# kvarq/kvarq

Measured on AMD Instinct MI355X. Metric: fastq_reads_per_sec_scanned, higher is better.
Workload: dtype u8

## Files before the change

include/kvarq_hip.h:

```cpp
#ifndef KVARQ_HIP_H
#define KVARQ_HIP_H

#include <stddef.h>
#include <stdint.h>

#ifdef __cplusplus
extern "C" {
#endif

#define KVQ_MAX_READLENGTH 1024
#define KVQ_SCANBUFSIZE    (1024*1024)
#define KVQ_MUT_CLASSES    6

enum {
    KVQ_OK          = 0,
    KVQ_ERR_FORMAT  = 1,
    KVQ_ERR_IO      = 2,
    KVQ_ERR_MEMORY  = 3,
    KVQ_ERR_RUNTIME = 4,
    KVQ_ERR_TYPE    = 5,
    KVQ_ERR_DEVICE  = 6,
    KVQ_ERR_RESCAN  = 7
};

typedef struct kvq_config {
    int32_t maxerrors;
    int32_t minoverlap;
    int32_t minreadlength;
    int32_t nthreads;
    int8_t  Amin;
    int8_t  Azero;
} kvq_config;

void kvq_config_set(const kvq_config *cfg);
void kvq_config_get(kvq_config *cfg);

int32_t kvq_last_error(char *msg, size_t cap);

typedef struct kvq_table kvq_table;

kvq_table *kvq_table_create(const uint8_t *const *seqs, const int32_t *seqlens, int32_t nseq,
                            const kvq_config *cfg);
void    kvq_table_destroy(kvq_table *t);
int32_t kvq_table_nseq(const kvq_table *t);
int64_t kvq_table_bases(const kvq_table *t);
int32_t kvq_table_seq_is_seeded(const kvq_table *t, int32_t s);
int32_t kvq_table_seed_k(const kvq_table *t);

enum { KVQ_CTR_RECORDS = 0, KVQ_CTR_LONGEST = 1, KVQ_CTR_HITS = 2, KVQ_CTR_READLENGTHS = 4 };
int64_t kvq_counters_len(const kvq_table *t);
int64_t kvq_counters_off_nseqhits(const kvq_table *t);
int64_t kvq_counters_off_nseqbasehits(const kvq_table *t);
int64_t kvq_counters_off_coverage(const kvq_table *t);
int64_t kvq_counters_off_mutations(const kvq_table *t);
int64_t kvq_table_seq_offset(const kvq_table *t, int32_t s);

typedef struct kvq_scan kvq_scan;

kvq_scan *kvq_scan_create(const kvq_table *t, void *d_counters);
void      kvq_scan_destroy(kvq_scan *s);

int64_t kvq_chunk_offsets(const uint8_t *data, int64_t nbytes, int64_t *offsets, int64_t cap);

int32_t kvq_scan_device(kvq_scan *s, const void *d_data, int64_t nbytes,
                        const int64_t *chunk_off, int64_t nchunks, int64_t fpos_base);

int32_t kvq_scan_host(kvq_scan *s, const void *h_data, int64_t nbytes,
                      const int64_t *chunk_off, int64_t nchunks, int64_t fpos_base);

int32_t kvq_scan_host_async(kvq_scan *s, const void *h_data, int64_t nbytes,
                            const int64_t *chunk_off, int64_t nchunks, int64_t fpos_base);
int32_t kvq_scan_host_copied(kvq_scan *s);
int32_t kvq_scan_host_drain(kvq_scan *s);

int32_t kvq_scan_finish(kvq_scan *s);
int32_t kvq_scan_finish_begin(kvq_scan *s);

int64_t        kvq_scan_n_hits(const kvq_scan *s);
const int32_t *kvq_scan_hit_seq_nr(const kvq_scan *s);
const int64_t *kvq_scan_hit_file_pos(const kvq_scan *s);
const int32_t *kvq_scan_hit_seq_pos(const kvq_scan *s);
const int32_t *kvq_scan_hit_length(const kvq_scan *s);
const int32_t *kvq_scan_hit_readlength(const kvq_scan *s);
const uint8_t *kvq_scan_hitseq_blob(const kvq_scan *s);
const int64_t *kvq_scan_hitseq_offsets(const kvq_scan *s);
const int64_t *kvq_scan_counters(const kvq_scan *s);
void          *kvq_scan_device_counters(const kvq_scan *s);
void          *kvq_scan_device_counters_own(const kvq_scan *s);
int64_t        kvq_scan_parsed(const kvq_scan *s);
int64_t        kvq_scan_total(const kvq_scan *s);

int32_t        kvq_scan_set_records(kvq_scan *s, int32_t on);
const uint8_t *kvq_scan_record_blob(const kvq_scan *s);
const int64_t *kvq_scan_hit_record_off(const kvq_scan *s);
const int32_t *kvq_scan_hit_record_len(const kvq_scan *s);
int64_t        kvq_scan_record_bytes(const kvq_scan *s);

double  kvq_scan_kernel_ms(const kvq_scan *s);
double  kvq_scan_main_kernel_ms(const kvq_scan *s);
double  kvq_scan_gap_ms(const kvq_scan *a, const kvq_scan *b);
int64_t kvq_scan_main_kernel_launches(const kvq_scan *s);
int32_t kvq_scan_reset(kvq_scan *s);
int32_t kvq_scan_path(const kvq_scan *s);
void    kvq_scan_force_exhaustive(kvq_scan *s, int32_t on);

#define KVQ_CELL_DENSE  0x1000
#define KVQ_CELL_DIAG   0x2000
#define KVQ_CELL_STAMPS 0x4000
int32_t kvq_scan_kernel_pick(int32_t k, int32_t stride, int32_t dense, uint32_t rec_bytes, uint32_t tile_bytes, uint32_t dbg);
int32_t kvq_scan_kernel(const kvq_scan *s);
uint32_t kvq_tile_for_text(const uint8_t *text, size_t n, uint32_t *rec_bytes_out);

typedef struct kvq_comm kvq_comm;
int32_t   kvq_comm_unique_id(void *id128);
kvq_comm *kvq_comm_create(int32_t nranks, int32_t rank, const void *id128);
void      kvq_comm_destroy(kvq_comm *c);
int32_t   kvq_comm_nranks(const kvq_comm *c);
int32_t   kvq_comm_rank(const kvq_comm *c);
int32_t   kvq_scan_set_comm(kvq_scan *s, kvq_comm *c);
int32_t   kvq_scan_gather_hits(kvq_scan *s, kvq_comm *c);
int32_t   kvq_comm_allreduce_counters(kvq_comm *c, void *d_counters, int64_t ctr_len, void *d_scratch16);
kvq_comm *kvq_comm_create_local(int32_t nranks, int32_t rank, uint64_t world_key);
int32_t   kvq_gather_plan(int32_t nranks, const uint64_t *counts, uint64_t *parts, uint64_t *blob_base, uint64_t *totals);
int32_t   kvq_gather_host(int32_t nranks, const uint64_t *counts, const uint8_t *const *rank_bufs, uint8_t *out);
void      kvq_result_layout_words(uint64_t n, uint64_t blob_bytes, uint64_t *out8);

kvq_scan *kvq_findseqs(const char *const *files, int32_t nfiles,
                       const uint8_t *const *seqs, const int32_t *seqlens, int32_t nseq);

#define KVQ_FIND_DEVICE_INFLATE 1u
#define KVQ_FIND_DEVICE_GZIP 2u
#define KVQ_FIND_RECORDS 4u
kvq_scan *kvq_findseqs_ex(const char *const *files, int32_t nfiles,
                          const uint8_t *const *seqs, const int32_t *seqlens, int32_t nseq, uint32_t flags);

void kvq_findseqs_free(kvq_scan *s);

int64_t kvq_host_chunk_plan(const char *const *files, int32_t nfiles, int64_t *chunk_fpos, int64_t *chunk_len,
                            int64_t cap, int64_t *parsed, int64_t *total, int64_t batch_bytes);

typedef struct kvq_live_stats {
    int64_t records_parsed;
    int64_t parsed;
    int64_t total;
    int64_t rls_longest;
    int32_t nseq;
    int32_t running;
    int32_t sigints;
    int32_t stop_requested;
} kvq_live_stats;

void kvq_poll_stats(kvq_live_stats *out, int64_t *readlengths ,
                    int64_t *nseqhits, int64_t *nseqbasehits, int32_t nseq_cap);
void kvq_request_stop(void);
void kvq_count_sigint(void);
int  kvq_sigint_counter_install(void);
void kvq_sigint_counter_remove(void);

int32_t kvq_device_count(void);
int32_t kvq_set_device(int32_t ordinal);
void   *kvq_device_alloc(int64_t nbytes);
void    kvq_device_free(void *p);
int32_t kvq_memcpy_h2d(void *d, const void *h, int64_t nbytes);
int32_t kvq_memcpy_d2h(void *h, const void *d, int64_t nbytes);
int32_t kvq_memset_d(void *d, int32_t value, int64_t nbytes);
int32_t kvq_device_synchronize(void);
void    kvq_release_cached(void);

int32_t kvq_synth_reads_device(void *d_out, int64_t first, int64_t n, int32_t L,
                               uint64_t seed, const void *d_genome, int64_t genome_size);
void    kvq_synth_reads_host(uint8_t *out, int64_t first, int64_t n, int32_t L,
                             uint64_t seed, const uint8_t *genome, int64_t genome_size);
void    kvq_synth_genome_host(uint8_t *out, int64_t size, uint64_t seed);

int32_t kvq_inflate_raw_host(const uint8_t *in, int64_t n, uint8_t *out, int64_t isize);

int64_t kvq_bgzf_index(const uint8_t *file_bytes, int64_t n, int64_t *block_off, uint32_t *csize, uint32_t *isize, int64_t cap);

typedef struct kvq_bgzf_block {
    int64_t  in_off;
    int64_t  out_off;
    uint32_t in_len;
    uint32_t isize;
} kvq_bgzf_block;

int32_t kvq_inflate_bgzf_device(const void *d_in, int64_t in_bytes, const kvq_bgzf_block *d_blocks, int64_t nblocks,
                                void *d_out, int64_t out_bytes, int32_t *d_status);

int64_t kvq_chunk_offsets_device(const void *d_data, int64_t nbytes, int64_t *offsets, int64_t cap);

typedef struct kvq_gzip_report {
    int64_t runs;
    int64_t chunks;
    int64_t candidates_tested;
    int64_t refuted;
    int64_t redecodes;
    int64_t slot_overflows;
    int64_t marker_symbols;
    int64_t input_retries;
    double  ms_find, ms_decode, ms_resolve, ms_replace;
} kvq_gzip_report;

int64_t kvq_inflate_gzip_host(const uint8_t *file, int64_t n, int64_t chunk_bytes, uint8_t *out, int64_t out_cap,
                              int32_t *status, int64_t *err_fpos, kvq_gzip_report *rep);
int64_t kvq_inflate_gzip_device(const void *d_file, int64_t n, int64_t chunk_bytes, void *d_out, int64_t out_cap,
                                int32_t *status, int64_t *err_fpos, kvq_gzip_report *rep);
void    kvq_gzip_last_report(kvq_gzip_report *rep);
int64_t kvq_gzip_slot_canaries(int32_t pad_symbols);
int64_t kvq_gzip_last_chunks(int64_t *cand, int64_t ncand_cap, int64_t *start_bit, int64_t *end_bit, int64_t *nsym, int64_t cap,
                             int64_t *ncand);

typedef struct kvq_bam_report {
    int64_t runs;
    int64_t segments;
    int64_t refuted;
    int64_t check_passes;
    int64_t records_seen;
    int64_t records_written;
    int64_t records_skipped;
    int64_t records_noqual;
    int64_t bam_bytes;
    int64_t text_bytes;
    double  ms_inflate, ms_find, ms_emit;
} kvq_bam_report;
void    kvq_bam_last_report(kvq_bam_report *rep);
int64_t kvq_bam_header_host(const uint8_t *inflated, int64_t n, int32_t *n_ref);
int64_t kvq_bam_to_fastq_host(const uint8_t *inflated, int64_t n, int32_t n_ref, int64_t first_record, uint8_t *out, int64_t cap,
                              int64_t *consumed);
int64_t kvq_bam_to_fastq_device(const void *d_in, int64_t n, int32_t n_ref, int64_t first_record, void *d_out, int64_t cap,
                                int64_t segment_bytes, kvq_bam_report *report);

const char *kvq_version(void);

#ifdef __cplusplus
}
#endif
#endif
```

kvarq_amd/_lib.py:

```python
import ctypes as C
import os

HERE = os.path.dirname(os.path.abspath(__file__))
PATH = os.path.join(HERE, 'libkvarq_hip.so')

MAX_READLENGTH = 1024
OK, ERR_FORMAT, ERR_IO, ERR_MEMORY, ERR_RUNTIME, ERR_TYPE, ERR_DEVICE, ERR_RESCAN = range(8)
CTR_RECORDS, CTR_LONGEST, CTR_HITS, CTR_READLENGTHS = 0, 1, 2, 4
CELL_DENSE, CELL_DIAG, CELL_STAMPS = 0x1000, 0x2000, 0x4000
FIND_RECORDS = 4


class Config(C.Structure):
    _fields_ = [('maxerrors', C.c_int32), ('minoverlap', C.c_int32), ('minreadlength', C.c_int32),
                ('nthreads', C.c_int32), ('Amin', C.c_int8), ('Azero', C.c_int8)]


class LiveStats(C.Structure):
    _fields_ = [('records_parsed', C.c_int64), ('parsed', C.c_int64), ('total', C.c_int64),
                ('rls_longest', C.c_int64), ('nseq', C.c_int32), ('running', C.c_int32),
                ('sigints', C.c_int32), ('stop_requested', C.c_int32)]


class GzipReport(C.Structure):
    _fields_ = [(n, C.c_int64) for n in ('runs', 'chunks', 'candidates_tested', 'refuted', 'redecodes',
                                         'slot_overflows', 'marker_symbols', 'input_retries')] + \
        [(n, C.c_double) for n in ('ms_find', 'ms_decode', 'ms_resolve', 'ms_replace')]

    def as_dict(self):
        return {n: getattr(self, n) for n, _ in self._fields_}


class BamReport(C.Structure):
    _fields_ = [(n, C.c_int64) for n in ('runs', 'segments', 'refuted', 'check_passes', 'records_seen', 'records_written',
                                         'records_skipped', 'records_noqual', 'bam_bytes', 'text_bytes')] + \
        [(n, C.c_double) for n in ('ms_inflate', 'ms_find', 'ms_emit')]

    def as_dict(self):
        return {n: getattr(self, n) for n, _ in self._fields_}


i32, i64, u64, vp, cp = C.c_int32, C.c_int64, C.c_uint64, C.c_void_p, C.c_char_p
P = C.POINTER

PROTOTYPES = {
    'kvq_config_set': (None, [P(Config)]),
    'kvq_config_get': (None, [P(Config)]),
    'kvq_last_error': (i32, [C.c_char_p, C.c_size_t]),
    'kvq_table_create': (vp, [P(cp), P(i32), i32, P(Config)]),
    'kvq_table_destroy': (None, [vp]),
    'kvq_table_nseq': (i32, [vp]),
    'kvq_table_bases': (i64, [vp]),
    'kvq_table_seq_is_seeded': (i32, [vp, i32]),
    'kvq_table_seed_k': (i32, [vp]),
    'kvq_counters_len': (i64, [vp]),
    'kvq_counters_off_nseqhits': (i64, [vp]),
    'kvq_counters_off_nseqbasehits': (i64, [vp]),
    'kvq_counters_off_coverage': (i64, [vp]),
    'kvq_counters_off_mutations': (i64, [vp]),
    'kvq_table_seq_offset': (i64, [vp, i32]),
    'kvq_scan_create': (vp, [vp, vp]),
    'kvq_scan_destroy': (None, [vp]),
    'kvq_chunk_offsets': (i64, [vp, i64, P(i64), i64]),
    'kvq_scan_device': (i32, [vp, vp, i64, P(i64), i64, i64]),
    'kvq_scan_host': (i32, [vp, vp, i64, P(i64), i64, i64]),
    'kvq_scan_host_async': (i32, [vp, vp, i64, P(i64), i64, i64]),
    'kvq_scan_host_copied': (i32, [vp]),
    'kvq_scan_host_drain': (i32, [vp]),
    'kvq_scan_finish': (i32, [vp]),
    'kvq_scan_finish_begin': (i32, [vp]),
    'kvq_scan_n_hits': (i64, [vp]),
    'kvq_scan_hit_seq_nr': (P(i32), [vp]),
    'kvq_scan_hit_file_pos': (P(i64), [vp]),
    'kvq_scan_hit_seq_pos': (P(i32), [vp]),
    'kvq_scan_hit_length': (P(i32), [vp]),
    'kvq_scan_hit_readlength': (P(i32), [vp]),
    'kvq_scan_hitseq_blob': (vp, [vp]),
    'kvq_scan_hitseq_offsets': (P(i64), [vp]),
    'kvq_scan_counters': (P(i64), [vp]),
    'kvq_scan_device_counters': (vp, [vp]),
    'kvq_scan_device_counters_own': (vp, [vp]),
    'kvq_scan_parsed': (i64, [vp]),
    'kvq_scan_total': (i64, [vp]),
    'kvq_scan_set_records': (i32, [vp, i32]),
    'kvq_scan_record_blob': (vp, [vp]),
    'kvq_scan_hit_record_off': (P(i64), [vp]),
    'kvq_scan_hit_record_len': (P(i32), [vp]),
    'kvq_scan_record_bytes': (i64, [vp]),
    'kvq_scan_kernel_ms': (C.c_double, [vp]),
    'kvq_scan_main_kernel_ms': (C.c_double, [vp]),
    'kvq_scan_gap_ms': (C.c_double, [vp, vp]),
    'kvq_scan_main_kernel_launches': (i64, [vp]),
    'kvq_scan_reset': (i32, [vp]),
    'kvq_scan_path': (i32, [vp]),
    'kvq_scan_force_exhaustive': (None, [vp, i32]),
    'kvq_scan_kernel_pick': (i32, [i32, i32, i32, C.c_uint32, C.c_uint32, C.c_uint32]),
    'kvq_scan_kernel': (i32, [vp]),
    'kvq_tile_for_text': (C.c_uint32, [vp, C.c_size_t, P(C.c_uint32)]),
    'kvq_comm_unique_id': (i32, [vp]),
    'kvq_comm_create': (vp, [i32, i32, vp]),
    'kvq_comm_destroy': (None, [vp]),
    'kvq_comm_nranks': (i32, [vp]),
    'kvq_comm_rank': (i32, [vp]),
    'kvq_scan_set_comm': (i32, [vp, vp]),
    'kvq_scan_gather_hits': (i32, [vp, vp]),
    'kvq_comm_allreduce_counters': (i32, [vp, vp, i64, vp]),
    'kvq_comm_create_local': (vp, [i32, i32, C.c_uint64]),
    'kvq_gather_plan': (i32, [i32, vp, vp, vp, vp]),
    'kvq_gather_host': (i32, [i32, vp, vp, vp]),
    'kvq_result_layout_words': (None, [C.c_uint64, C.c_uint64, vp]),
    'kvq_findseqs': (vp, [P(cp), i32, P(cp), P(i32), i32]),
    'kvq_findseqs_ex': (vp, [P(cp), i32, P(cp), P(i32), i32, C.c_uint32]),
    'kvq_findseqs_free': (None, [vp]),
    'kvq_host_chunk_plan': (i64, [P(cp), i32, P(i64), P(i64), i64, P(i64), P(i64), i64]),
    'kvq_poll_stats': (None, [P(LiveStats), P(i64), P(i64), P(i64), i32]),
    'kvq_request_stop': (None, []),
    'kvq_count_sigint': (None, []),
    'kvq_sigint_counter_install': (C.c_int, []),
    'kvq_sigint_counter_remove': (None, []),
    'kvq_device_count': (i32, []),
    'kvq_set_device': (i32, [i32]),
    'kvq_device_alloc': (vp, [i64]),
    'kvq_device_free': (None, [vp]),
    'kvq_memcpy_h2d': (i32, [vp, vp, i64]),
    'kvq_memcpy_d2h': (i32, [vp, vp, i64]),
    'kvq_memset_d': (i32, [vp, i32, i64]),
    'kvq_device_synchronize': (i32, []),
    'kvq_release_cached': (None, []),
    'kvq_synth_reads_device': (i32, [vp, i64, i64, i32, u64, vp, i64]),
    'kvq_synth_reads_host': (None, [vp, i64, i64, i32, u64, vp, i64]),
    'kvq_synth_genome_host': (None, [vp, i64, u64]),
    'kvq_inflate_raw_host': (i32, [vp, i64, vp, i64]),
    'kvq_bgzf_index': (i64, [vp, i64, P(i64), P(C.c_uint32), P(C.c_uint32), i64]),
    'kvq_chunk_offsets_device': (i64, [vp, i64, P(i64), i64]),
    'kvq_inflate_bgzf_device': (i32, [vp, i64, vp, i64, vp, i64, vp]),
    'kvq_inflate_gzip_host': (i64, [vp, i64, i64, vp, i64, P(i32), P(i64), P(GzipReport)]),
    'kvq_inflate_gzip_device': (i64, [vp, i64, i64, vp, i64, P(i32), P(i64), P(GzipReport)]),
    'kvq_gzip_last_report': (None, [P(GzipReport)]),
    'kvq_gzip_slot_canaries': (i64, [i32]),
    'kvq_gzip_last_chunks': (i64, [P(i64), i64, P(i64), P(i64), P(i64), i64, P(i64)]),
    'kvq_bam_last_report': (None, [P(BamReport)]),
    'kvq_bam_header_host': (i64, [vp, i64, P(i32)]),
    'kvq_bam_to_fastq_host': (i64, [vp, i64, i32, i64, vp, i64, P(i64)]),
    'kvq_bam_to_fastq_device': (i64, [vp, i64, i32, i64, vp, i64, i64, P(BamReport)]),
    'kvq_version': (cp, []),
}

_lib = None


def build():
    import subprocess
    subprocess.check_call(['make', '-s', '-C', os.path.join(HERE, 'csrc')])


def lib():
    global _lib
    if _lib is None:
        if not os.path.exists(PATH):
            raise ImportError('%s is missing: build it with `make -C kvarq_amd/csrc` '
                              '(there is no CPU fallback for the scan)' % PATH)
        L = C.CDLL(PATH)
        for name, (res, args) in PROTOTYPES.items():
            f = getattr(L, name)
            f.restype, f.argtypes = res, args
        _lib = L
    return _lib


def kernel_cell(cell):
    if cell <= 0:
        return None
    return {'k': cell & 15, 'stride': (cell >> 4) & 15, 'lg': ((cell >> 8) & 15) - 1, 'dense': bool(cell & CELL_DENSE)}


def last_error():
    buf = C.create_string_buffer(1024)
    code = lib().kvq_last_error(buf, 1024)
    return code, buf.value.decode('latin-1')
```

kvarq_amd/csrc/kernels_bp.hip:

```cpp
#include "kvq_host.h"

#ifndef KVQ_TEXT_AUX
#define KVQ_TEXT_AUX 0
#endif
#define KVQ_MARK(name) asm volatile("; KVQMARK " name)
#define BP_WIN (ST_BUF + ST_BLK)
#define BP_Q1_KIND 25
#define BP_QW 96
#define BP_Q2W 96
#define BP_NLCAP 1920
#define BP_P2_LATE 0xFFFEu
#define BP_HEAD 2048u
#define BP_QCAP (BP_QW * ST_WAVES)
#define BP_Q2CAP (BP_Q2W * ST_WAVES)

typedef unsigned int u32x4_t __attribute__((ext_vector_type(4)));

struct BpLds {
    uint32_t cdp[BP_WIN / 16 + 8];
    uint32_t gdp[BP_WIN / 32 + 8];
    uint16_t nl[BP_NLCAP];
    uint8_t  bmA[8192];
    uint32_t hist[KVQ_RL_BINS / 2];
    union {
// ... 98 lines not shown
                for (int jj = 0; jj <= me && !earlier; jj++) {
                    const int ph = jj * KK, pt = rl - (jj + 1) * KK;
                    if (ph + KK <= rl && (kind == 0u || ph < p)) earlier = seed_live_bp<KK>(P.tab2, roff, rl, ph, toff, seql, ph + d);
                    if (!earlier && pt >= 0 && (kind == 0u || pt < p)) earlier = seed_live_bp<KK>(P.tab2, roff, rl, pt, toff, seql, pt + d);
                }
                if (kind == 0u) {
                    for (int jj = 0; jj <= me && !earlier; jj++)
                        for (int sft = 0; sft < stride && !earlier; sft++) {
                            const int o = jj * P.pitch + sft;
                            if (o < q && ((o - d) & (stride - 1)) == 0) earlier = seed_live_bp<KK>(P.tab2, roff, rl, o - d, toff, seql, o);
                        }
                }
                if (!earlier) { hitAB = canAB; hitC = canC; }
            }
        }
    }
    emit_cold(P.cold, hitAB, fpos, s, sposAB, lenAB, rl, keyAB);
    emit_cold(P.cold, hitC, fpos, s, sposC, lenC, rl, keyC);
}

__device__ __forceinline__ void bp_vector(const uint4 v, uint32_t addk, uint32_t &nl16, uint32_t &g16, uint32_t &c32)
{
    const uint32_t x[4] = { v.x, v.y, v.z, v.w };
    uint32_t nf[4], gf[4], cc[4];
#pragma unroll
    for (int d = 0; d < 4; d++) {
        nf[d] = kvq_nl_flags(x[d]);
        gf[d] = good_flags(x[d], addk);
        cc[d] = __builtin_amdgcn_udot4(x[d] & 0x06060606u, 0x40100401u, 0u, false);
    }
#ifdef KVQ_ABL_JUNK
    {
        uint32_t junk = x[0];
#pragma unroll
        for (int i = 0; i < KVQ_ABL_JUNK; i++) {
#if KVQ_ABL_SLOW == 2
            { uint32_t sj = 0; asm volatile("s_add_u32 %0, %0, 1" : "+s"(sj)); asm volatile("" :: "s"(sj)); }
#elif KVQ_ABL_SLOW == 3
            { uint32_t lj; asm volatile("ds_read_b32 %0, %1" : "=v"(lj) : "v"(junk & 0x3FCu)); asm volatile("s_waitcnt lgkmcnt(0)" ::: "memory"); asm volatile("" :: "v"(lj)); }
#elif KVQ_ABL_SLOW
            asm volatile("v_lshl_or_b32 %0, %0, 1, %1" : "+v"(junk) : "v"(x[1]));
#else
            asm volatile("v_add_u32 %0, %0, %1" : "+v"(junk) : "v"(x[1]));
#endif
        }
        asm volatile("" :: "v"(junk));
    }
#endif
    nl16 = kvq_flags16(nf[0], nf[1], nf[2], nf[3]);
    g16 = kvq_flags16(gf[0], gf[1], gf[2], gf[3]);
    c32 = ((cc[0] | (cc[1] << 8)) >> 1) | ((cc[2] | (cc[3] << 8)) << 15);
}

struct BpArgs {
    KvqParams P;
    SeedTables X;
    const uint8_t *data; int64_t fpos_base;
    const uint4 *tiles; uint32_t *tile_report; unsigned int *tile_ctr;
    void *redo;
    unsigned int *fail;
    void *surv;
    uint32_t ntiles, tile_bytes, dbg, pad_, redo_cap;
    uint32_t surv_cap;
};
#define BP_SHARDS 64u
#define BP_SHARD_STRIDE 32u
__host__ __device__ static inline uint32_t bp_shard_begin(uint32_t sh, uint32_t ntiles) { return (uint32_t)(((uint64_t)sh * ntiles) / BP_SHARDS); }
__device__ __forceinline__ uint32_t bp_draw(unsigned int *ctr, uint32_t ntiles, uint32_t &sh, uint32_t &left)
{
    while (left) {
        const uint32_t t = atomicAdd(&ctr[sh * BP_SHARD_STRIDE], 1u);
        if (t < bp_shard_begin(sh + 1u, ntiles)) return t;
        sh = sh + 1u == BP_SHARDS ? 0u : sh + 1u; left--;
    }
    return ntiles;
}
static_assert(BP_SHARDS == 64u, "one counter per lane of the drawing wave");
__device__ __forceinline__ uint32_t bp_draw_wave(unsigned int *ctr, uint32_t ntiles, uint32_t &sh, uint32_t lane)
{
    const uint32_t m = (((uint32_t)blockIdx.x >> 6) * 2u + 37u) | 1u;
    for (;;) {
        const uint32_t mine = (sh + m * lane) & (BP_SHARDS - 1u);
        const uint32_t seen = __hip_atomic_load(&ctr[mine * BP_SHARD_STRIDE], __ATOMIC_RELAXED, __HIP_MEMORY_SCOPE_AGENT);
        const uint64_t open = __ballot(seen < bp_shard_begin(mine + 1u, ntiles));
        if (open == 0) return ntiles;
        const uint32_t pick = (sh + m * (uint32_t)(__ffsll((long long)open) - 1)) & (BP_SHARDS - 1u);
        uint32_t t = 0;
        if (lane == 0) t = atomicAdd(&ctr[pick * BP_SHARD_STRIDE], 1u);
        t = (uint32_t)__builtin_amdgcn_readfirstlane((int)t);
        sh = pick;
        if (t < bp_shard_begin(pick + 1u, ntiles)) return t;
    }
}
typedef const __attribute__((address_space(4))) BpArgs *BpArgsPtr;
__device__ __forceinline__ BpArgsPtr bp_args(const BpArgs *A)
{
    BpArgsPtr p = (BpArgsPtr)A;
    asm volatile("" : "+s"(p));
    return p;
}

#ifndef BP_OCC
#define BP_OCC 8
#endif

__device__ __forceinline__ void bp_runs64(uint64_t m, int n, uint32_t dbg, int &pre, int &suf, int &best, int &bstart)
{
    const uint64_t nmask = n < 64 ? (1ull << n) - 1ull : ~0ull;
    uint64_t zz = ~m & nmask;
    const int c = __popc((uint32_t)zz) + __popc((uint32_t)(zz >> 32));
    if (!__any(c > 3) && !(dbg & 4u)) {
        const uint32_t lo = (uint32_t)zz, hi = (uint32_t)(zz >> 32);
        auto ffbl = [](uint32_t x) -> uint32_t { uint32_t r; asm("v_ffbl_b32 %0, %1" : "=v"(r) : "v"(x)); return r; };
        auto ffbh = [](uint32_t x) -> uint32_t { uint32_t r; asm("v_ffbh_u32 %0, %1" : "=v"(r) : "v"(x)); return r; };
        auto ctz64 = [&](uint32_t l, uint32_t h) -> uint32_t {
            const uint32_t pl = ffbl(l), ph = ffbl(h) | 32u;
            const uint32_t r = pl < ph ? pl : ph; return r < (uint32_t)n ? r : (uint32_t)n;
        };
        const uint32_t p1 = ctz64(lo, hi);
        const uint64_t z2 = zz & (zz - 1ull);
        const uint32_t p2 = ctz64((uint32_t)z2, (uint32_t)(z2 >> 32));
        const uint32_t ch = ffbh(hi), cl = ffbh(lo) | 32u;
        uint32_t lz = ch < cl ? ch : cl; lz = lz < 64u ? lz : 64u;
        const uint32_t e = 64u - lz;
        const int g0 = (int)p1, g1 = (int)p2 - (int)p1 - 1, g2 = (int)e - (int)p2 - 2, g3 = n - (int)e;
        int bl = g0, bs = 0;
        if (g1 > bl) { bl = g1; bs = (int)p1 + 1; }
        if (g2 > bl) { bl = g2; bs = (int)p2 + 1; }
        if (g3 > bl) { bl = g3; bs = (int)e; }
        pre = g0; suf = g3; best = bl; bstart = bs;
    } else if (!__any(c > 8) && !(dbg & 4u)) {
        int prev = 0, first = n, p, bl = 0, bs = 0;
        do {
            const uint32_t plo = (uint32_t)(__ffs((int)(uint32_t)zz) - 1), ph = (uint32_t)(__ffs((int)(uint32_t)(zz >> 32)) - 1);
            const uint32_t phi = ph > 0xFFFFFFDFu ? 0xFFFFFFFFu : ph + 32u;
            uint32_t pm = plo < phi ? plo : phi; if (pm > (uint32_t)n) pm = (uint32_t)n;
            p = (int)pm;
            zz &= zz - 1ull;
            first = first < p ? first : p;
            const int gap = p - prev;
            if (gap > bl) { bl = gap; bs = prev; }
            prev = p < n ? p + 1 : prev;
        } while (__any(p < n));
        pre = first; suf = n - prev; best = bl; bstart = bs;
    } else {
        const uint64_t inv = ~m;
        pre = inv ? __ffsll((long long)inv) - 1 : 64; if (pre > n) pre = n;
        const uint64_t top = ~(m << (64 - n));
        suf = top ? __clzll((long long)top) : 64; if (suf > n) suf = n;
        longest_run64(m, n, best, bstart);
    }
}

template <int SS, int LG, bool STAMPS, bool DIAG = STAMPS, int KK = 8, bool DENSE = (KK < 8)>
__global__ void __launch_bounds__(ST_THREADS, DENSE ? 8 : BP_OCC)
kvq_scan_bp(const BpArgs *__restrict__ A_)
{
    __shared__ __align__(16) BpLds S;
    uint8_t *const lds_raw = reinterpret_cast<uint8_t *>(&S);
    int tid = threadIdx.x, lane = tid & 63;
    const uint32_t wave = rfl((uint32_t)tid >> 6);
    if ((uint32_t)(uintptr_t)((__attribute__((address_space(3))) uint8_t *)lds_raw) != 0u) __builtin_trap();
    unsigned long long stamp_acc[8] = { 0, 0, 0, 0, 0, 0, 0, 0 }, stamp_t = 0, wave_p34 = 0;
    unsigned long long rt_in = 0, rt_pro = 0, rt_first = 0;
    uint32_t tally[8] = { 0, 0, 0, 0, 0, 0, 0, 0 };
#ifdef KVQ_TALLY
#define BTALLY(i, cond) do { if constexpr (STAMPS) { if (cond) tally[i]++; } } while (0)
#else
#define BTALLY(i, cond) ((void)0)
#endif
    if constexpr (STAMPS) rt_in = __builtin_amdgcn_s_memrealtime();
#define BSTAMP(i) do { if constexpr (STAMPS) { const unsigned long long now_ = __builtin_amdgcn_s_memtime(); stamp_acc[i] += now_ - stamp_t; stamp_t = now_; } } while (0)

    uint32_t ntiles, tile_bytes, dbg, amin;
    {
        const BpArgsPtr A = bp_args(A_);
        ntiles = A->ntiles; tile_bytes = A->tile_bytes; dbg = DIAG ? A->dbg : 0u; amin = (uint32_t)A->P.amin;
        const GlbWords bm1 = (GlbWords)A->X.bm1;
        for (int i = tid; i < (1 << (2 * KK)) / 32; i += ST_THREADS) reinterpret_cast<uint32_t *>(S.bmA)[i] = bm1[i];
    }
    uint32_t my_shard = blockIdx.x % BP_SHARDS; bool no_more = false;
    if (wave == ST_WAVES - 1u) {
        unsigned int *const ctr = bp_args(A_)->tile_ctr;
        const uint32_t t0 = bp_draw_wave(ctr, ntiles, my_shard, (uint32_t)lane);
        const uint32_t t1 = t0 < ntiles ? bp_draw_wave(ctr, ntiles, my_shard, (uint32_t)lane) : ntiles;
        no_more = t1 >= ntiles;
        if (lane == 0) { S.first_tile = t0; S.next_tile = t1; }
    }
    for (int i = tid; i < KVQ_RL_BINS / 2; i += ST_THREADS) S.hist[i] = 0;
    if (tid == 0) { S.longest_p1 = 0; S.records = 0; S.fallback = 0; }
    if (tid < (int)ST_WAVES) { S.sv_at[tid] = 0; S.sv_end[tid] = 0; }
    if (tid < 8) { S.cdp[BP_WIN / 16 + tid] = 0; S.gdp[BP_WIN / 32 + tid] = 0; }

    static_assert(ST_ROUNDS * 16u == ST_BLK, "one scan block per thread");
    static_assert(ST_WAVES == 8, "eight wave totals");
    __syncthreads();

    if (const uint32_t stg = bp_args(A_)->pad_) { for (uint32_t i = 0; i < (blockIdx.x >> 8) * stg; i++) __builtin_amdgcn_s_sleep(127); }
    if constexpr (STAMPS) rt_pro = __builtin_amdgcn_s_memrealtime();
    unsigned long long *const ctr_stamps = bp_args(A_)->P.ctr + KVQ_CTR_RL_ + 924;
    const uint32_t addk = (0x80u - amin) * 0x01010101u;
    uint32_t tiles_done = 0;
    uint32_t g_done = 0xFFFFFFFFu;
    uint32_t my_longest = 0;
    for (uint32_t g = rfl(S.first_tile); ; ) {
        asm volatile("" : "+v"(tid));
        lane = tid & 63;
        const uint32_t blk = (uint32_t)tid * ST_BLK;
        const uint32_t wv = wave * (ST_BLK * 64u / 16u) + (uint32_t)lane;
        if constexpr (STAMPS) stamp_t = __builtin_amdgcn_s_memtime();
        uint32_t Ja = 0, Jb = 0, Jt = 0, g0 = 0; GlbBytes text = nullptr;
        uint4 pre[ST_ROUNDS];
#pragma unroll
        for (int r = 0; r < (int)ST_ROUNDS; r++) pre[r] = make_uint4(0, 0, 0, 0);
        if (g < ntiles) {
            const BpArgsPtr A = bp_args(A_);
            const u32x4_t q = ((const __attribute__((address_space(4))) u32x4_t *)A->tiles)[(dbg & 64u) ? (g & 63u) : g];
            Ja = q.x; Jb = q.y; Jt = q.z;
            g0 = (Ja & ~15u) + Jt * tile_bytes;
            const uint8_t *const data = A->data;
            text = (GlbBytes)data + g0 - ST_PRE;
            const uint32_t load_hi = g0 + ST_TILE + ST_OV < Jb ? g0 + ST_TILE + ST_OV : Jb;
            const uint32_t vo = 16u * wv - ST_PRE, vo0 = wv >= ST_PRE / 16u ? vo : ST_NO_BLOCK;
            const __amdgpu_buffer_rsrc_t rs = __builtin_amdgcn_make_buffer_rsrc((void *)(data + g0), 0, (int)(((load_hi + 15u) & ~15u) - g0), 0x00020000);
#pragma unroll
            for (int r = 0; r < (int)ST_ROUNDS; r++) {
                const u32x4_t v = __builtin_amdgcn_raw_buffer_load_b128(rs, (int)(r ? vo + 1024u * r : vo0), 0, KVQ_TEXT_AUX);
                pre[r] = make_uint4(v.x, v.y, v.z, v.w);
            }
        }
        __syncthreads();
        unsigned long long sub_t0 = 0, sub_t1 = 0;
        if constexpr (STAMPS) sub_t0 = __builtin_amdgcn_s_memtime();
        if (g_done != 0xFFFFFFFFu) {
            if (tid == 0 && S.fallback) { atomicOr(&bp_args(A_)->tile_report[g_done], TR_FLAG_FALLBACK); S.fallback = 0; }
        }
        if (g >= ntiles) break;
        const uint32_t gn = rfl(S.next_tile);
        const uint32_t own_end = g0 + tile_bytes < Jb ? g0 + tile_bytes : Jb;
        const uint32_t load_hi = g0 + ST_TILE + ST_OV < Jb ? g0 + ST_TILE + ST_OV : Jb;
        const uint32_t own_begin_l = (Jt == 0 ? Ja : g0) - g0 + ST_PRE;
        const uint32_t own_end_l = own_end - g0 + ST_PRE;
        const uint32_t end_l = load_hi - g0 + ST_PRE;

        {
            const uint32_t w_lo = wave * (ST_BLK * 64u), w_hi = w_lo + ST_BLK * 64u;
            const bool cut = ((own_begin_l & 15u) && own_begin_l > w_lo && own_begin_l < w_hi) || ((end_l & 15u) && end_l > w_lo && end_l < w_hi);
            if (cut) {
                uint32_t wv_ = wv;
                asm volatile("" : "+v"(wv_));
#pragma unroll
                for (int r = 0; r < (int)ST_ROUNDS; r++) {
                    const uint32_t o = 16u * (wv_ + 64u * r);
                    uint32_t x[4] = { pre[r].x, pre[r].y, pre[r].z, pre[r].w };
#pragma unroll
                    for (int d = 0; d < 4; d++) x[d] &= (kvq_range_flags(o + 4u * d, own_begin_l, end_l) >> 7) * 0xFFu;
                    pre[r] = make_uint4(x[0], x[1], x[2], x[3]);
                }
            }
        }
        if constexpr (STAMPS) { asm volatile("s_waitcnt vmcnt(0)" ::: "memory"); sub_t1 = __builtin_amdgcn_s_memtime(); }
        KVQ_MARK("P0 vectors");
        {
            const uint32_t pa = 2u * wv, ca = 4u * wv;
#pragma unroll
            for (int r = 0; r < (int)ST_ROUNDS; r++) {
                uint32_t n16, g16, c32;
                bp_vector(pre[r], addk, n16, g16, c32);
                *reinterpret_cast<__attribute__((address_space(3))) uint16_t *>((uintptr_t)(BP_LDS_NLP + pa + 128u * r)) = (uint16_t)n16;
                *reinterpret_cast<__attribute__((address_space(3))) uint16_t *>((uintptr_t)(BP_LDS_GDP + pa + 128u * r)) = (uint16_t)g16;
                *reinterpret_cast<__attribute__((address_space(3))) uint32_t *>((uintptr_t)(ca + 256u * r)) = c32;
            }
            if (wave == 0u) {
#pragma unroll
                for (int r = 0; r < (int)(BP_HEAD / 1024u); r++)
                    *reinterpret_cast<__attribute__((address_space(3))) u32x4_t *>((uintptr_t)(BP_LDS_HEAD + 16u * (uint32_t)lane + 1024u * r)) = u32x4_t{ pre[r].x, pre[r].y, pre[r].z, pre[r].w };
            }
        }
        KVQ_MARK("P0 vectors end");
        uint32_t m0, m1, m2;
        {
            const uint32_t a = BP_LDS_NLP + ((10u * (uint32_t)tid) & ~3u), sh = ((uint32_t)tid & 1u) * 16u;
            const uint32_t d0 = lds_u32_at(a), d1 = lds_u32_at(a + 4u), d2 = lds_u32_at(a + 8u);
            m0 = __builtin_amdgcn_alignbit(d1, d0, sh); m1 = __builtin_amdgcn_alignbit(d2, d1, sh); m2 = (d2 >> sh) & 0xFFFFu;
        }
        static_assert(ST_BLK == 80u, "five vectors per block");
        const uint32_t cnt = (uint32_t)(__popc(m0) + __popc(m1) + __popc(m2));
        const uint32_t incl = kvq_wave_incl_scan(cnt);
        if (lane == 63) S.wtot[wave] = incl;
        KVQ_MARK("P0 scan end");
        if constexpr (STAMPS) { if (tid == 0) { atomicAdd(&ctr_stamps[0], sub_t0 - stamp_t); atomicAdd(&ctr_stamps[1], sub_t1 - sub_t0); } }
        BSTAMP(0);
        __syncthreads();
        KVQ_MARK("P1b");
        BSTAMP(1);
        uint32_t n_all = 0;
        {
            uint32_t run = S.wtot[lane & 7];
            run += (uint32_t)__builtin_amdgcn_update_dpp(0, (int)run, 0x111, 0xf, 0xf, false);
            run += (uint32_t)__builtin_amdgcn_update_dpp(0, (int)run, 0x112, 0xf, 0xf, false);
            run += (uint32_t)__builtin_amdgcn_update_dpp(0, (int)run, 0x114, 0xf, 0xf, false);
            n_all = (uint32_t)__builtin_amdgcn_readlane((int)run, 7);
            const uint32_t upto = (uint32_t)__builtin_amdgcn_readlane((int)run, (int)wave);
            uint32_t n = upto - (uint32_t)__builtin_amdgcn_readlane((int)incl, 63) + incl - cnt;
            if (blk < own_end_l && blk + ST_BLK >= own_end_l) S.n_owned = n + cnt;
            if (__any(cnt != 0u)) {
                if (n_all <= BP_NLCAP && !__any(cnt > 2u)) {
// ... 264 lines not shown
                }
                }
        KVQ_MARK("filter end / P4a");
                BSTAMP(5);
                KVQ_SETPRIO(3);

                if constexpr (!DENSE) {
                const bool over = qn > BP_QW;
                const uint32_t qn_ok = (over || (dbg & 1u)) ? 0u : qn;
                if (over && step > 1u) { step >>= 1; continue; }
                if (over) {
                    if (mine && gl == 0) {
                        const BpArgsPtr A = bp_args(A_);
                        const KvqRedo Rd(A->redo);
                        const uint32_t boff = g0 - ST_PRE + roff;
                        bool put = false;
                        if (A->redo) {
                            if (rl >= KVQ_LONG_READ) {
                                const unsigned int i = atomicAdd(Rd.count + 1, 1u);
                                if (i < KVQ_LONG_CAP) { Rd.read_off[KVQ_REDO_CAP - 1u - i] = boff; Rd.read_len[KVQ_REDO_CAP - 1u - i] = rl; put = true; }
                            }
                            if (!put) {
                                const unsigned int i = atomicAdd(Rd.count, 1u);
                                if (i < A->redo_cap) { Rd.rec_start[i] = KVQ_REDO_TRIMMED; Rd.read_off[i] = boff; Rd.read_len[i] = rl; }
                                put = true;
                            }
                        }
                        if (!put) S.fallback = 1u;
                        else atomicOr(A->fail, 2u);
                    }
                }
#include "kernels_bp_p4.inc"
                } else {
                    uint32_t hA = 0, hpos = 0, tpos = 0; bool hh = false, th = false;
                    int ee = e0, xt = (int)G;
                    int ee_of_hA = e0;
                    bool done = false;
                    while (!done) {
                        bool full = false;
                        while (!full) {
                            if (!__any(hA != 0u || hh || th)) {
                                ee_of_hA = ee;
                                if (__any(ee < e1)) {
                                    const bool act = ee < e1;
                                    uint32_t hA_;
                                    {
#include "kernels_bp_lookup.inc"
                                        hA_ = hA;
                                    }
                                    const int nv = act ? (e1 - ee < NR ? e1 - ee : NR) : 0;
                                    hA = hA_ & ((1u << nv) - 1u);
                                    if (first) { hh = hhit; th = thit; hpos = gl * KK; tpos = (uint32_t)(rl - ((int)gl + 1) * KK); first = false; }
                                    ee += NR;
                                } else if (xt <= me_) {
                                    const int jj = xt + (int)gl;
                                    hpos = (uint32_t)(jj * KK); tpos = (uint32_t)(rl - (jj + 1) * KK);
                                    hh = fixed_block((int)hpos, head_ok(jj)); th = fixed_block((int)tpos, tail_ok(jj));
                                    xt += (int)G;
                                } else { done = true; break; }
                                continue;
                            }
                            const uint32_t c = (uint32_t)__popc(hA) + (hh ? 1u : 0u) + (th ? 1u : 0u);
                            const uint32_t inc = kvq_wave_incl_scan(c);
                            const uint32_t tot = (uint32_t)__builtin_amdgcn_readlane((int)inc, 63);
                            uint32_t idx = qn + inc - c;
                            while (hA && idx < BP_QW) {
                                const int j = __ffs((int)hA) - 1; hA &= hA - 1u;
                                q1[idx++] = k | ((uint32_t)(SS * (ee_of_hA + j)) << 9);
                            }
                            if (hh && idx < BP_QW) { q1[idx++] = k | (hpos << 9) | (1u << BP_Q1_KIND); hh = false; }
                            if (th && idx < BP_QW) { q1[idx++] = k | (tpos << 9) | (1u << BP_Q1_KIND); th = false; }
                            full = qn + tot >= BP_QW;
                            qn = qn + tot < BP_QW ? qn + tot : BP_QW;
                        }
                        {
                            const uint32_t qn_ok = (dbg & 1u) ? 0u : qn;
#include "kernels_bp_p4.inc"
                        }
                        qn = 0;
                    }
                }
                KVQ_SETPRIO(2);
                sub += step;
            }
            KVQ_SETPRIO(0);
            if (have && gl == 0 && (c0 != '@' || cp != '+')) {
                const BpArgsPtr A = bp_args(A_);
                const uint32_t m = jn + 4u * k;
                const uint32_t rstart = m == 0 ? ST_PRE + (Ja & 15u) : (uint32_t)S.nl[m - 1] + 1u, plus = (uint32_t)S.nl[m + 1] + 1u;
                const int64_t tf = A->fpos_base + (int64_t)g0;
                if (c0 != '@') atomicMin(A->P.err, ((unsigned long long)(tf + rstart - ST_PRE) << 16) | (0ull << 8) | c0);
                else atomicMin(A->P.err, ((unsigned long long)(tf + plus - ST_PRE) << 16) | (1ull << 8) | cp);
            }
        KVQ_MARK("P4 end");
            BSTAMP(6);
        }
        if constexpr (STAMPS) wave_p34 += __builtin_amdgcn_s_memtime() - wave_t3;
        if (wave == ST_WAVES - 1u) {
            uint32_t d = no_more ? ntiles : rfl(drawn);
            if (!no_more && d >= bp_shard_begin(my_shard + 1u, ntiles)) {
                d = bp_draw_wave(bp_args(A_)->tile_ctr, ntiles, my_shard, (uint32_t)tid & 63u);
                no_more = d >= ntiles;
            }
            if ((tid & 63) == 0) S.next_tile = d;
        }
        KVQ_MARK("tile end");
        BSTAMP(7);
        if constexpr (STAMPS) { if (rt_first == 0) rt_first = __builtin_amdgcn_s_memrealtime(); }
        g_done = g; g = gn;
    }

    unsigned long long rt_loop = 0;
    if constexpr (STAMPS) rt_loop = __builtin_amdgcn_s_memrealtime();
    {
        const uint32_t at = S.sv_at[wave], end = S.sv_end[wave];
        if (at + (uint32_t)lane < end) KvqSurvivors(bp_args(A_)->surv).item[at + (uint32_t)lane].rl = 0;
    }
    atomicMax(&S.longest_p1, my_longest);
    __syncthreads();
    unsigned long long *const ctr = (bp_args(A_)->P.ctr + (size_t)(blockIdx.x % KVQ_STAGE_COPIES) * KVQ_STAGE_SLOTS);
    if constexpr (STAMPS) {
        if (tid == 0) for (int i = 0; i < 8; i++) atomicAdd(&ctr[KVQ_CTR_RL_ + 900 + i], stamp_acc[i]);
        for (int i = 0; i < 8; i++) if (tally[i]) atomicAdd(&ctr[KVQ_CTR_RL_ + 930 + i], (unsigned long long)tally[i]);
        if (lane == 0) atomicAdd(&ctr[KVQ_CTR_RL_ + 908 + wave], wave_p34);
        if (tid == 0) {
            const unsigned long long rt_out = __builtin_amdgcn_s_memrealtime();
            atomicAdd(&ctr[KVQ_CTR_RL_ + 916], rt_pro - rt_in); atomicAdd(&ctr[KVQ_CTR_RL_ + 917], rt_first ? rt_first - rt_pro : 0ull);
            atomicAdd(&ctr[KVQ_CTR_RL_ + 918], rt_loop - rt_in); atomicAdd(&ctr[KVQ_CTR_RL_ + 919], 1ull);
            atomicMax(&ctr[KVQ_CTR_RL_ + 920], rt_out); atomicMax(&ctr[KVQ_CTR_RL_ + 921], rt_in);
            atomicMax(&ctr[KVQ_CTR_RL_ + 922], ~rt_in);
            atomicAdd(&ctr[KVQ_CTR_RL_ + 923], rt_out - rt_loop);
        }
    }
    for (int i = tid; i < KVQ_RL_BINS / 2; i += ST_THREADS) {
        const uint32_t w = S.hist[i];
        if (w & 0xFFFFu) atomicAdd(&ctr[KVQ_CTR_RL_ + 2 * i], (unsigned long long)(w & 0xFFFFu));
        if (w >> 16) atomicAdd(&ctr[KVQ_CTR_RL_ + 2 * i + 1], (unsigned long long)(w >> 16));
    }
    if (tid == 0) {
        if (S.longest_p1) atomicMax(&ctr[KVQ_CTR_LONGEST_], (unsigned long long)S.longest_p1);
        if (S.records) atomicAdd(&ctr[KVQ_CTR_RECORDS_], (unsigned long long)S.records);
    }
}

__device__ __forceinline__ bool seed_same_text(GlbBytes x, GlbBytes y, int K)
{
    const uint32_t x0 = glb_u32(x), y0 = glb_u32(y), x1 = glb_u32(x + 4), y1 = glb_u32(y + 4);
    const uint32_t m0 = K >= 4 ? 0x06060606u : (0x06060606u & ((1u << (8 * K)) - 1u));
    const uint32_t m1 = K >= 8 ? 0x06060606u : K > 4 ? (0x06060606u & ((1u << (8 * (K - 4))) - 1u)) : 0u;
    return (((x0 ^ y0) & m0) | ((x1 ^ y1) & m1)) == 0u;
}
extern "C" __global__ void __launch_bounds__(1024)
kvq_verify_survivors(KvqParams P, const uint8_t *__restrict__ data, int64_t fpos_base, const void *surv_, const unsigned int *__restrict__ fail,
                     int K, int stride, int pitch)
{
    const KvqSurvivors Sv(const_cast<void *>(surv_));
    if (fail && (*fail & 1u)) return;
    const uint32_t n = Sv.count[0] < Sv.count[1] ? Sv.count[0] : Sv.count[1];
    const int me = P.maxerrors, mo = P.minoverlap;
    const uint32_t step = gridDim.x * blockDim.x;
    __shared__ uint32_t n_round, arena_at;
    const uint32_t lane = threadIdx.x & 63u;
    for (uint32_t base = blockIdx.x * blockDim.x; base < n; base += step) {
        if (threadIdx.x == 0) n_round = 0;
        __syncthreads();
        const uint32_t i = base + threadIdx.x;
        bool hitAB = false, hitC = false;
        int s = 0, rl = 0, lenAB = 0, lenC = 0, sposAB = 0, sposC = 0; uint32_t keyAB = 0, keyC = 0; int64_t fpos = 0;
        if (i < n) {
            const KvqSurvivor v = Sv.item[i];
            rl = (int)v.rl; const int p = (int)v.p; const uint32_t kind = v.kind;
            fpos = fpos_base + (int64_t)v.boff;
            const int q = (int)(v.en & 4095u);
            s = (int)((v.en >> 12) & 0xFFFFFu);
            const uint32_t toff = (uint32_t)((v.en >> 32) & 0xFFFFFu);
            const int seql = (int)(v.en >> 52);
            const GlbBytes read = (GlbBytes)data + v.boff, seq = (GlbBytes)P.tab + toff;
            const int d = q - p;
            const int a = d < 0 ? -d : 0;
            const int L = (rl < seql - d ? rl : seql - d) - a;
            bool canAB = false, canC = false;
            const bool guard = rl > mo && seql > mo;
            if (d < 0) {
                const int ii = -d;
                if (ii <= rl - seql) { canC = true; lenC = seql; sposC = -ii; keyC = (2u << 30) | (uint32_t)ii; }
                else if (guard && ii <= rl - mo) { canAB = true; lenAB = rl - ii; sposAB = -ii; keyAB = (0u << 30) | (uint32_t)(rl - mo - ii); }
            } else if (d == 0) {
                canC = true; lenC = rl > seql ? seql : rl; sposC = 0; keyC = 2u << 30;
            } else {
                const int ii = d;
                if (guard && ii <= seql - mo && ii >= seql - rl) { canAB = true; lenAB = seql - ii; sposAB = ii; keyAB = (1u << 30) | (uint32_t)(seql - mo - ii); }
                if (rl <= seql && ii <= seql - rl) { canC = true; lenC = rl; sposC = ii; keyC = (2u << 30) | (uint32_t)ii; }
            }
            if ((canAB || canC) && L > 0 && rl > 0) {
                bool earlier = false;
                auto live = [&](bool want, int rp, int sq) -> bool {
                    const bool ok = want && rp >= 0 && rp + K <= rl && sq >= 0 && sq + K <= seql;
                    return seed_same_text(read + (ok ? rp : 0), seq + (ok ? sq : 0), K) && ok;
                };
                const int sft = d & (stride - 1);
                constexpr int JJ = 4;
#pragma unroll
                for (int jj = 0; jj < JJ; jj++) {
                    const int ph = jj * K, pt = rl - (jj + 1) * K, o = jj * pitch + sft;
                    const bool in = jj <= me;
                    const bool e0 = live(in && (kind == 0u || ph < p), ph, ph + d);
                    const bool e1 = live(in && (kind == 0u || pt < p), pt, pt + d);
                    const bool e2 = live(in && kind == 0u && o < q, o - d, o);
                    earlier = earlier || e0 || e1 || e2;
                }
                for (int jj = JJ; jj <= me && !earlier; jj++) {
                    const int ph = jj * K, pt = rl - (jj + 1) * K, o = jj * pitch + sft;
                    earlier = live(kind == 0u || ph < p, ph, ph + d) || live(kind == 0u || pt < p, pt, pt + d) || live(kind == 0u && o < q, o - d, o);
                }
                if (!earlier) {
                    int mism = 0, j = 0;
                    const GlbBytes x = read + a, y = seq + (a + d);
                    typedef u32x4_t __attribute__((aligned(1))) u32x4_any;
                    typedef const __attribute__((address_space(1))) u32x4_any *GlbVec;
                    auto diff16 = [](const u32x4_t xv, const u32x4_t yv) { return diff_bytes(xv.x, yv.x) + diff_bytes(xv.y, yv.y) + diff_bytes(xv.z, yv.z) + diff_bytes(xv.w, yv.w); };
                    for (; j + 128 <= L && mism <= me; j += 128) {
                        u32x4_t xv[8], yv[8];
#pragma unroll
                        for (int t = 0; t < 8; t++) { xv[t] = *(GlbVec)(x + j + 16 * t); yv[t] = *(GlbVec)(y + j + 16 * t); }
#pragma unroll
                        for (int t = 0; t < 8; t++) mism += diff16(xv[t], yv[t]);
                    }
                    if (j + 64 <= L && mism <= me) {
                        u32x4_t xv[4], yv[4];
#pragma unroll
                        for (int t = 0; t < 4; t++) { xv[t] = *(GlbVec)(x + j + 16 * t); yv[t] = *(GlbVec)(y + j + 16 * t); }
#pragma unroll
                        for (int t = 0; t < 4; t++) mism += diff16(xv[t], yv[t]);
                        j += 64;
                    }
                    for (; j + 16 <= L && mism <= me; j += 16) mism += diff16(*(GlbVec)(x + j), *(GlbVec)(y + j));
                    if (j < L && mism <= me) {
                        if (L >= 16) {
                            const u32x4_t xv = *(GlbVec)(x + L - 16), yv = *(GlbVec)(y + L - 16);
                            const int keep = L - j;
                            uint32_t dx[4] = { xv.x ^ yv.x, xv.y ^ yv.y, xv.z ^ yv.z, xv.w ^ yv.w };
#pragma unroll
                            for (int t = 0; t < 4; t++) {
                                const int first_new = 16 - keep - 4 * t;
                                const uint32_t m = first_new <= 0 ? 0xFFFFFFFFu : first_new >= 4 ? 0u : 0xFFFFFFFFu << (8 * first_new);
                                mism += diff_bytes(dx[t] & m, 0u);
                            }
                        } else {
                            for (; j + 4 <= L && mism <= me; j += 4) mism += diff_bytes(glb_u32(x + j), glb_u32(y + j));
                            for (; j < L && mism <= me; j++) mism += (x[j] != y[j]);
                        }
                    }
                    if (mism <= me) { hitAB = canAB; hitC = canC; }
                }
            }
        }
        const uint64_t mAB = __ballot(hitAB), mC = __ballot(hitC);
        const uint32_t nAB = (uint32_t)__popcll(mAB), nC = (uint32_t)__popcll(mC);
        uint32_t at = 0;
        if (nAB + nC) {
            if (lane == 0u) at = atomicAdd(&n_round, nAB + nC);
            at = (uint32_t)__builtin_amdgcn_readfirstlane((int)at);
        }
        __syncthreads();
        const uint32_t total = n_round;
        if (total) {
            if (threadIdx.x == 0) arena_at = atomicAdd(P.arena_n, total);
            __syncthreads();
            const uint32_t o = arena_at + at;
            KvqHit h;
            h.fpos = fpos; h.seq_nr = s; h.readlength = rl; h.blob_off = 0;
            if (hitAB) {
                const uint32_t idx = o + (uint32_t)__popcll(mAB & kvq_lanemask_lt());
                h.seq_pos = sposAB; h.length = lenAB; h.key = keyAB;
                if (idx < P.arena_cap) P.arena[idx] = h;
            }
            if (hitC) {
                const uint32_t idx = o + nAB + (uint32_t)__popcll(mC & kvq_lanemask_lt());
                h.seq_pos = sposC; h.length = lenC; h.key = keyC;
                if (idx < P.arena_cap) P.arena[idx] = h;
            }
        }
    }
}

__device__ void kvq_long_line_run(const uint8_t *line, uint32_t Q, int amin, int lane, int &best, uint32_t &best_start)
{
    Seg all; all.beg = 0; all.len = 0; all.pre = 0; all.suf = 0; all.best = 0; all.bstart = 0;
    for (uint32_t r0 = 0; r0 < Q; r0 += 4096u) {
        uint32_t w[4][4];
#pragma unroll
        for (int r = 0; r < 4; r++) {
            const uint32_t o = r0 + 1024u * (uint32_t)r + 16u * (uint32_t)lane;
            const uint32_t oo = o + 16u <= Q + 1u ? o : (Q + 1u >= 16u ? Q + 1u - 16u : 0u);
#pragma unroll
            for (int d = 0; d < 4; d++) __builtin_memcpy(&w[r][d], line + oo + 4u * d, 4);
        }
#pragma unroll
        for (int r = 0; r < 4; r++) {
            const uint32_t row = r0 + 1024u * (uint32_t)r;
            if (row >= Q) break;
            const uint32_t o = row + 16u * (uint32_t)lane;
            const uint32_t oo = o + 16u <= Q + 1u ? o : (Q + 1u >= 16u ? Q + 1u - 16u : 0u);
            const int n = o < Q ? (Q - o < 16u ? (int)(Q - o) : 16) : 0;
            uint32_t m = 0;
#pragma unroll
            for (int d = 0; d < 4; d++)
#pragma unroll
                for (int b = 0; b < 4; b++) m |= (uint32_t)((int)(int8_t)(w[r][d] >> (8 * b)) >= amin) << (4 * d + b);
            const uint32_t shift = o - oo;
// ... 21 lines not shown
```

kvarq_amd/csrc/kernels_bp_p4.inc:

```
                if (qn_ok) {
                    typedef const __attribute__((address_space(1))) u32x4_t *GlbEntries;
                    typedef unsigned int u32x2_t __attribute__((ext_vector_type(2)));
                    typedef const __attribute__((address_space(1))) u32x2_t __attribute__((aligned(4))) *GlbPairs;
                    GlbWords start; GlbEntries ent; int need;
                    {
                        const BpArgsPtr A = bp_args(A_);
                        start = (GlbWords)A->X.start; ent = (GlbEntries)A->X.ent;
                        need = (me_ + 1) * KK;
                    }
                    BTALLY(5, lane == 0);
                    for (uint32_t w0 = 0; ; w0 += BP_Q2W) {
                        uint32_t run = 0;
                        for (uint32_t q0 = 0; q0 < qn_ok; q0 += 64u) {
                            const uint32_t qi = q0 + lane;
                            uint32_t en0 = 0, ne = 0;
                            if (qi < qn_ok) {
                                const uint32_t cd = q1[qi];
                                BTALLY(0, w0 == 0u && (cd >> BP_Q1_KIND) == 0u); BTALLY(1, w0 == 0u && (cd >> BP_Q1_KIND) != 0u);
                                const uint32_t code = cdp_code<KK>((S.rinfo[cd & 511u] & 0xFFFFu) + ((cd >> 9) & 0xFFFFu));
                                const u32x2_t st = *(GlbPairs)(start + (code | ((cd >> BP_Q1_KIND) << (2 * KK))));
                                en0 = st.x; ne = st.y - st.x;
                            }
                            const uint32_t inc = kvq_wave_incl_scan(ne);
                            const uint32_t base = run + inc - ne - w0;
                            for (uint32_t j = 0; j < ne; j++)
                                if (base + j < BP_Q2W) q2[base + j] = (qi << 22) | (en0 + j);
                            run += (uint32_t)__builtin_amdgcn_readlane((int)inc, 63);
                        }
        KVQ_MARK("P4b");
                        const uint32_t n_items = run - w0 < BP_Q2W ? run - w0 : BP_Q2W;
                        for (uint32_t i0 = 0; i0 < n_items; i0 += 64u) {
                            BTALLY(4, lane == 0);
                            const uint32_t ii = i0 + lane;
                            bool alive = false;
                            uint32_t kind = 0, croff = 0, en_lo = 0, en_hi = 0; int p = 0, crl = 0;
                            BTALLY(2, ii < n_items);
                            if (ii < n_items) {
                                const uint32_t it = q2[ii];
                                const u32x4_t E = ent[it & 0x3FFFFFu];
                                const uint32_t cd = q1[it >> 22];
                                p = (int)((cd >> 9) & 0xFFFFu); kind = cd >> BP_Q1_KIND;
                                const uint32_t ri = S.rinfo[cd & 511u];
                                croff = ri & 0xFFFFu; crl = (int)(ri >> 16);
                                en_lo = E.x; en_hi = E.y;
                                const int q = (int)(E.x & 4095u), seql = (int)(E.y >> 20);
                                const int d = q - p;
                                const int a = d < 0 ? -d : 0;
                                const int L = (crl < seql - d ? crl : seql - d) - a;
                                if (L >= need) {
                                    const int wn = L < 16 ? L : 16;
                                    const int w = p < a + L - wn ? p : a + L - wn;
                                    const uint32_t sh = 2u * (uint32_t)(w - p + 16);
                                    const uint32_t seqw = (uint32_t)((((uint64_t)E.w << 32) | E.z) >> sh);
                                    const uint32_t v = cdp32(croff + (uint32_t)w) ^ seqw;
                                    uint32_t dm = (v | (v >> 1)) & 0x55555555u;
                                    if (wn < 16) dm &= (1u << (2 * wn)) - 1u;
                                    alive = __popc(dm) <= me_;
                                }
                            }
                            const bool any_alive = __any(alive);
                            BTALLY(3, alive); BTALLY(7, lane == 0 && any_alive);
                            if (any_alive) {
                                const KvqSurvivors Sv(bp_args(A_)->surv);
                                if (Sv.count) {
                                    const uint64_t am = __ballot(alive);
                                    const uint32_t na = (uint32_t)__popcll(am);
                                    uint32_t at = rfl(S.sv_at[wave]), end = rfl(S.sv_end[wave]);
                                    if (at + na > end) {
                                        if (at + lane < end) Sv.item[at + lane].rl = 0;
                                        const uint32_t want = na > KVQ_SURV_CHUNK ? na : KVQ_SURV_CHUNK;
                                        uint32_t base = 0;
                                        if (lane == 0) base = atomicAdd(Sv.count, want);
                                        base = rfl(base);
                                        const uint32_t cap = bp_args(A_)->surv_cap;
                                        if (base + want <= cap) { at = base; end = base + want; }
                                        else {
                                            if (lane < want && base + lane < cap) Sv.item[base + lane].rl = 0;
                                            at = end = 0;
                                        }
                                    }
                                    if (at + na <= end && end != 0u) {
                                        if (alive) {
                                            KvqSurvivor v;
                                            v.boff = g0 - ST_PRE + croff; v.rl = (uint16_t)crl; v.p = (uint16_t)p; v.en = ((uint64_t)en_hi << 32) | en_lo; v.kind = kind; v.pad = 0;
                                            Sv.item[at + (uint32_t)__popcll(am & kvq_lanemask_lt())] = v;
                                            alive = false;
                                        }
                                        at += na;
                                    }
                                    if (lane == 0) { S.sv_at[wave] = at; S.sv_end[wave] = end; }
                                }
                                if (__any(alive)) {
                                    BpHot H; int64_t tile_fpos;
                                    {
                                        const BpArgsPtr A = bp_args(A_);
                                        H.cold = &A_->P; H.tab = (GlbBytes)A->P.tab; H.tab2 = (GlbWords)A->X.tab2; H.maxerrors = me_; H.minoverlap = A->P.minoverlap; H.pitch = A->X.pitch;
                                        tile_fpos = A->fpos_base + (int64_t)g0;
                                    }
                                    bp_verify_rest<KK>(H, text, alive, croff, crl, p, kind, en_lo, en_hi, tile_fpos, SS);
                                }
                            }
                        }
                        if (run <= w0 + BP_Q2W) break;
                    }
                }
```

kvarq_amd/csrc/kvq_findseqs.hip:

```cpp
#include "kvq_host.h"

#include <atomic>
#include <condition_variable>
#include <deque>
#include <memory>
#include <mutex>
#include <signal.h>
#include <string.h>
#include <zlib.h>
#include <thread>
#include <sys/mman.h>
#include <unistd.h>

int64_t kvq_tail_record(const uint8_t *buf, int64_t n);
int kvq_scan_finish_internal(kvq_scan *s);


static std::atomic<int> g_running{0}, g_stop{0}, g_sigints{0};
static struct { kvq_table *t = nullptr; kvq_scan *s = nullptr; int dev = -1; } g_kept;
static std::mutex g_kept_lock;
void kvq_drop_kept_scan()
{
    std::lock_guard<std::mutex> l(g_kept_lock);
    if (g_kept.s) { kvq_table *kt = g_kept.t; kvq_scan_destroy(g_kept.s); kvq_table_destroy(kt); g_kept.t = nullptr; g_kept.s = nullptr; }
// ... 1139 lines not shown
            uint8_t *text = g_dev.d_text[tb].as<uint8_t>();
            const uint8_t *carry_at = g_dev.d_text[cb].as<uint8_t>() + carry_src;
            if (carry && carry_at != text) KVQ_HIP(hipMemcpyAsync(text, carry_at, (size_t)carry, hipMemcpyDeviceToDevice, st));
            KVQ_HIP(hipEventRecord(ev[2], st));
            if ((rc = bam_run_emit(bam, s0, seg_bytes, ro, text, carry, (int64_t)g_dev.d_text[tb].cap, st))) return rc;
            KVQ_HIP(hipEventRecord(ev[3], st));
            rep.text_bytes += ro.text;
            bcarry = n - ro.end; bcarry_src = ro.end; run_base += ro.end; bb ^= 1;
            int64_t *cut = (int64_t *)g_dev.pcut;
            int64_t *d_cut = g_dev.d_cut.as<int64_t>();
            std::vector<int64_t> off;
            int64_t cs = 0, cfill = fill;
            for (;;) {
                if ((rc = kvq_cut_chunks_launch(text, have, cs, cfill, d_cut + 8, KVQ_CUT_CAP, d_cut, st))) return rc;
                KVQ_HIP(hipMemcpyAsync(cut, d_cut, (8 + KVQ_CUT_CAP) * 8, hipMemcpyDeviceToHost, st));
                KVQ_HIP(hipStreamSynchronize(st));
                if (cut[3]) {
                    kvq_set_error(KVQ_ERR_RUNTIME, "could find beginning of record; read %ld bytes up to %ld", (long)cut[4], (long)(text_fpos + cut[5]));
                    return KVQ_ERR_RUNTIME;
                }
                off.insert(off.end(), cut + 8, cut + 8 + cut[0]);
                cs = cut[1]; cfill = cut[2];
                if (cut[0] < KVQ_CUT_CAP) break;
            }
            ms = 0; if (hipEventElapsedTime(&ms, ev[2], ev[3]) == hipSuccess) rep.ms_emit += ms;
            fill = cfill;
            fpos += ro.text;
            if (ftell0 + consumed > 0)
                total = (int64_t)(size_t)((float)size_all * fpos / (ftell0 + consumed));
            if (eof) { if (have > cs) off.push_back(cs); cs = have; }
            const bool handed = !off.empty();
            if (handed) {
                off.push_back(cs);
                if ((rc = sink.batch(text, cs, off.data(), (int64_t)off.size() - 1, text_fpos, fpos, total))) return rc;
            }
            if (eof) { ftell0 += consumed; }
            else { carry = have - cs; carry_src = cs; cb = tb; fill -= cs; text_fpos += cs; }
            if (handed) tb ^= 1;
        }
    }
    s->path_bits |= 64;
    *parsed = fpos; *total_out = total;
    return KVQ_OK;
}

static int findseqs_pass(kvq_scan *s, const char *const *files, int nfiles, uint8_t *pin, uint8_t *pin2, int64_t pin_cap,
                         const std::vector<BgzfFile> *bz = nullptr, const std::vector<GzFile> *gz = nullptr,
                         const std::vector<BamFile> *bam = nullptr)
{
    ScanSink sink; sink.s = s; sink.staged = bz != nullptr || gz != nullptr || bam != nullptr;
    int64_t parsed = 0, total = 0;
    const double tp0 = now_ms();
    int rc = bz ? stream_device(sink, s, *bz, &parsed, &total)
           : gz ? stream_gzip_device(sink, s, *gz, &parsed, &total)
           : bam ? stream_bam_device(sink, s, *bam, &parsed, &total)
                : stream_batches(sink, files, nfiles, pin, pin_cap, &parsed, &total, pin2);
    if (g_timing) fprintf(stderr, "findseqs pass: stream %.1f ms\n", now_ms() - tp0);
    if (rc) return rc;
    s->parsed = parsed; s->total = total;
    {
        std::lock_guard<std::mutex> l(g_live_lock);
        g_live.parsed = parsed; g_live.total = total;
    }
    rc = kvq_scan_finish_internal(s);
    if (rc == KVQ_OK) live_from_counters(s->t, s->h_ctr.data(), parsed, total);
    return rc;
}

struct PlanSink {
    int64_t *fpos, *len; int64_t cap, n = 0;
    void begin(int64_t) {}
    int batch(const uint8_t *, int64_t, const int64_t *off, int64_t nchunks, int64_t base, int64_t, int64_t)
    {
        for (int64_t c = 0; c < nchunks; c++, n++)
            if (n < cap) { fpos[n] = base + off[c]; len[n] = off[c + 1] - off[c]; }
        return KVQ_OK;
    }
};

extern "C" int64_t kvq_host_chunk_plan(const char *const *files, int32_t nfiles, int64_t *chunk_fpos, int64_t *chunk_len,
                                       int64_t cap, int64_t *parsed, int64_t *total, int64_t batch_bytes)
{
    kvq_clear_error();
    const int64_t pin_cap = (batch_bytes > 0 ? batch_bytes : BATCH_BYTES) + 2 * KVQ_SCANBUFSIZE;
    uint8_t *buf = (uint8_t *)malloc((size_t)pin_cap);
    if (!buf) { kvq_set_error(KVQ_ERR_MEMORY, "cannot allocate memory for scanning"); return -1; }
    PlanSink sink; sink.fpos = chunk_fpos; sink.len = chunk_len; sink.cap = cap;
    const int rc = stream_batches(sink, files, nfiles, buf, pin_cap, parsed, total);
    free(buf);
    return rc ? -1 : sink.n;
}

static kvq_scan *findseqs_impl(const char *const *files, int32_t nfiles,
                               const uint8_t *const *seqs, const int32_t *seqlens, int32_t nseq, uint32_t flags)
{
    kvq_clear_error();
    int expected = 0;
    if (!g_running.compare_exchange_strong(expected, 1)) {
        kvq_set_error(KVQ_ERR_RUNTIME, "findseqs() already running!");
        return nullptr;
    }
    g_stop = 0; g_sigints = 0;
    const double tf0 = now_ms();
    kvq_table *t = nullptr; kvq_scan *s = nullptr;
    {
        kvq_config cfg; kvq_config_get(&cfg);
        std::lock_guard<std::mutex> l(g_kept_lock);
        int dev_now = 0; (void)hipGetDevice(&dev_now);
        if (g_kept.s && g_kept.dev == dev_now && nseq == g_kept.t->nseq && memcmp(&cfg, &g_kept.t->cfg, sizeof(cfg)) == 0) {
            bool same = true;
            for (int32_t i = 0; i < nseq && same; i++) {
                const int32_t len = g_kept.t->h_off[i + 1] - g_kept.t->h_off[i];
                same = seqlens[i] == len && memcmp(seqs[i], g_kept.t->h_tab.data() + g_kept.t->h_off[i], (size_t)len) == 0;
            }
            if (same && kvq_scan_reset(g_kept.s) == KVQ_OK) {
                t = g_kept.t; s = g_kept.s; g_kept.t = nullptr; g_kept.s = nullptr;
                s->tile_bytes = 0; s->rec_bytes = 0;
            }
        }
        if (!s && g_kept.s) { kvq_table *kt = g_kept.t; kvq_scan_destroy(g_kept.s); kvq_table_destroy(kt); g_kept.t = nullptr; g_kept.s = nullptr; }
        kvq_clear_error();
    }
    if (!s) {
        t = kvq_table_create(seqs, seqlens, nseq, nullptr);
        s = t ? kvq_scan_create(t, nullptr) : nullptr;
    }
    if (s && kvq_scan_set_records(s, (flags & KVQ_FIND_RECORDS) ? 1 : 0)) { kvq_scan_destroy(s); kvq_table_destroy(t); s = nullptr; t = nullptr; }
    const double tf1 = now_ms();
    static uint8_t *g_pin = nullptr;
    const int64_t pin_cap = BATCH_BYTES + 2 * KVQ_SCANBUFSIZE;
    std::vector<BamFile> bamf;
    bool bam = false, bam_failed = false;
    if (s) {
        int nbam = 0; bool unreadable = false;
        for (int32_t i = 0; i < nfiles; i++) { const int v = bam_peek(files[i]); unreadable |= v < 0; nbam += v > 0; }
        if (!unreadable && nbam > 0 && nbam < nfiles) { kvq_set_error(KVQ_ERR_IO, "cannot scan BAM and FastQ files in one call"); bam_failed = true; }
        else if (!unreadable && nbam > 0) { bam = true; bam_failed = bam_files(files, nfiles, bamf) != KVQ_OK; }
    }
    std::vector<BgzfFile> bz;
    const bool dev = s && !bam && !bam_failed && (flags & (KVQ_FIND_DEVICE_INFLATE | KVQ_FIND_DEVICE_GZIP)) && bgzf_files(files, nfiles, bz);
    std::vector<GzFile> gzf;
    const bool dev_any = s && !bam && !bam_failed && !dev && (flags & KVQ_FIND_DEVICE_GZIP) && gz_files(files, nfiles, gzf);
    if (s && !bam && !bam_failed && !dev && !dev_any && !g_pin && hipHostMalloc((void **)&g_pin, (size_t)pin_cap * 2, hipHostMallocDefault) != hipSuccess) {
        kvq_set_error(KVQ_ERR_MEMORY, "cannot allocate memory for scanning"); g_pin = nullptr;
    }
    uint8_t *const pin = g_pin;
    int64_t use_cap = pin_cap;
    if (const char *mb = getenv("KVQ_BATCH_MB")) {
        const long v = atol(mb);
        if (v >= 2 && (v << 20) < BATCH_BYTES) use_cap = ((int64_t)v << 20) + 2 * KVQ_SCANBUFSIZE;
    }
    const double tf2 = now_ms();
    if (s && !bam_failed && (pin || dev || dev_any || bam)) {
        for (int attempt = 0; attempt < 4; attempt++) {
            const int rc = bam ? findseqs_pass(s, files, nfiles, nullptr, nullptr, 0, nullptr, nullptr, &bamf)
                         : dev ? findseqs_pass(s, files, nfiles, nullptr, nullptr, 0, &bz)
                         : dev_any ? findseqs_pass(s, files, nfiles, nullptr, nullptr, 0, nullptr, &gzf)
                               : findseqs_pass(s, files, nfiles, pin, pin + pin_cap, use_cap);
            if (rc != KVQ_NEED_RESCAN) break;
            if (kvq_scan_reset(s)) break;
            if (attempt == 3) kvq_set_error(KVQ_ERR_MEMORY, "cannot allocate memory for results");
        }
    }
    const double tf3 = now_ms();
    if (s && s->stream) (void)hipStreamSynchronize(s->stream);
    if (g_timing) fprintf(stderr, "findseqs: table+scan %.1f  pinned alloc %.1f  passes %.1f  free %.1f ms\n", tf1 - tf0, tf2 - tf1, tf3 - tf2, now_ms() - tf3);
    if (s && (dev || dev_any)) s->path_bits |= 16;
    g_running = 0;
    if (s) s->t = t;
    else if (t) kvq_table_destroy(t);
    return s;
}

extern "C" kvq_scan *kvq_findseqs(const char *const *files, int32_t nfiles,
                                  const uint8_t *const *seqs, const int32_t *seqlens, int32_t nseq)
{
    return findseqs_impl(files, nfiles, seqs, seqlens, nseq, 0);
}

extern "C" kvq_scan *kvq_findseqs_ex(const char *const *files, int32_t nfiles,
                                     const uint8_t *const *seqs, const int32_t *seqlens, int32_t nseq, uint32_t flags)
{
    return findseqs_impl(files, nfiles, seqs, seqlens, nseq, flags);
}

extern "C" void kvq_findseqs_free(kvq_scan *s)
{
    if (!s) return;
    kvq_table *t = const_cast<kvq_table *>(s->t);
    {
        static const bool keep = !(getenv("KVQ_KEEP_SCAN") && getenv("KVQ_KEEP_SCAN")[0] == '0');
        std::lock_guard<std::mutex> l(g_kept_lock);
        if (keep && t && !g_kept.s && s->finished) { g_kept.t = t; g_kept.s = s; (void)hipGetDevice(&g_kept.dev); return; }
    }
    kvq_scan_destroy(s);
    kvq_table_destroy(t);
}
```

kvarq_amd/csrc/kvq_host.h:

```cpp
#pragma once

#include <hip/hip_runtime.h>
#include <stdint.h>
#include <stdio.h>
#include <string>
#include <vector>

#include "../../include/kvarq_hip.h"
#include "kvq_device.h"

void kvq_set_error(int code, const char *fmt, ...);
void kvq_clear_error();
int  kvq_error_code();

#define KVQ_HIP(call)                                                                         \
    do {                                                                                      \
        hipError_t e_ = (call);                                                               \
        if (e_ != hipSuccess) {                                                               \
            kvq_set_error(KVQ_ERR_DEVICE, "%s failed: %s (%s:%d)", #call, hipGetErrorString(e_), __FILE__, __LINE__); \
            return KVQ_ERR_DEVICE;                                                            \
        }                                                                                     \
    } while (0)

struct DevBuf {
    void *p = nullptr; size_t cap = 0;
    int ensure(size_t n);
    void release();
    template <class T> T *as() const { return (T *)p; }
};

struct TablePool {
    uint8_t *h = nullptr, *d = nullptr; size_t cap = 0, used = 0, h_cap = 0, d_cap = 0;
    int reserve(size_t bytes, hipStream_t stream);
    size_t take(size_t bytes) { const size_t at = used; used += (bytes + 255) & ~(size_t)255; return at; }
    void release();
};

struct kvq_table {
    kvq_config cfg;
    int32_t nseq = 0;
    int64_t bases = 0;
    std::vector<uint8_t> h_tab;
    std::vector<int32_t> h_off;
    std::vector<int32_t> exhaustive;
    std::vector<int32_t> seeded;
    std::vector<uint8_t> is_seeded;
    int32_t seed_k = 0;
    int device = 0;
    DevBuf d_tab, d_off, d_exh, d_all, d_seeded;
    struct SeedIndex *index = nullptr;
    int64_t ctr_len, off_nseqhits, off_nseqbasehits, off_cov, off_mut;
};

struct KvqResultLayout {
    size_t file_pos = 0, hitseq_off = 0, seq_nr = 0, seq_pos = 0, length = 0, readlength = 0, blob = 0, total = 0;
};

struct Batch {
    const uint8_t *d_data; int64_t nbytes; int64_t fpos_base;
    std::vector<int64_t> chunk_off;
    bool redone = false;
    bool is_redo = false;
    bool skips_done = false;
    size_t skip_at = 0;
    uint32_t tile_bytes = 0;
    const uint8_t *staged = nullptr;
};

struct kvq_comm;
#define KVQ_REDO_CAP 16384u
struct KvqSurvivor { uint32_t boff; uint16_t rl, p; uint64_t en; uint32_t kind, pad; };
#define KVQ_SURV_CAP (1u << 22)
#define KVQ_SURV_CHUNK 16u
struct KvqSurvivors {
    unsigned int *count; KvqSurvivor *item;
    static size_t bytes() { return 256 + (size_t)KVQ_SURV_CAP * sizeof(KvqSurvivor); }
    __host__ __device__ explicit KvqSurvivors(void *p) { count = (unsigned int *)p; item = (KvqSurvivor *)((char *)p + 256); }
};
struct KvqRedo {
    unsigned int *count; uint32_t *nl4, *rec_start, *read_off; int32_t *read_len;
    static size_t bytes() { return 256 + (size_t)KVQ_REDO_CAP * (16 + 4 + 4 + 4); }
    __host__ __device__ explicit KvqRedo(void *p) { char *c = (char *)p; count = (unsigned int *)c; nl4 = (uint32_t *)(c + 256); rec_start = nl4 + 4 * (size_t)KVQ_REDO_CAP; read_off = rec_start + KVQ_REDO_CAP; read_len = (int32_t *)(read_off + KVQ_REDO_CAP); }
};
int kvq_live_scans();
int kvq_chain_wait(struct kvq_scan *s, bool *behind_a_running_scan = nullptr);
bool kvq_chain_busy(const struct kvq_scan *s);
int kvq_chain_publish(struct kvq_scan *s);
uint32_t kvq_device_cu_count();
int kvq_comm_reduce_counters(kvq_comm *c, const unsigned long long *d_in, unsigned long long *d_out, int64_t ctr_len, unsigned long long *d_scratch, hipStream_t stream);
int kvq_comm_max_status(kvq_comm *c, unsigned long long mine, unsigned long long *d_scratch, hipStream_t stream, unsigned long long *out);

struct kvq_scan {
    const kvq_table *t = nullptr;
    kvq_comm *comm = nullptr;
    hipStream_t stream = nullptr;
    bool force_exhaustive = false;
    unsigned long long *d_ctr = nullptr; bool own_ctr = false; DevBuf d_ctr_own;
    std::vector<int64_t> h_ctr;
    uint32_t cus = 0;
    bool seen_skips = false;
    bool tail_pending = false; size_t tail_nb0 = 0, tail_spec = 0;
    uint32_t surv_cap = 0;
    DevBuf d_surv;
    DevBuf d_redo;
    DevBuf d_skipped, d_chunk_off, d_seg_base, d_seg_cnt, d_chunk_nrec, d_rec_base, d_nl4, d_rec_start, d_read_off, d_read_len;
    DevBuf d_covdiff;
    uint32_t tile_bytes = 0;
    uint32_t rec_bytes = 0;
    DevBuf d_arena, d_blob, d_small;
    uint32_t arena_cap = 0; uint64_t blob_cap = 0;
    unsigned int *d_arena_n = nullptr, *d_range = nullptr, *d_fail = nullptr, *cur_fail = nullptr;
    unsigned long long *d_blob_n = nullptr, *d_err = nullptr, *d_err_stage = nullptr, *d_stage_ctr = nullptr;
    int path_bits = 0;
    int32_t kernel_cell = 0;
    std::vector<int64_t> cur_chunk_off;
    size_t cur_co_at = 0;
    size_t cur_skip_at = 0, cur_first_at = 0; uint32_t cur_ntiles = 0;
    TablePool pool;
    DevBuf d_stage, d_stage_b;
    int run_slot = 1;
    hipStream_t copy_stream = nullptr;
    hipEvent_t ev_copy[2] = { nullptr, nullptr };
    bool copied_pending = false; int copied_slot = 0; Batch copied;
    std::vector<Batch> batches;
    bool host_batches = false;
    int64_t host_pending = -1;
    hipEvent_t ev_chain = nullptr;
    int64_t records = 0;
    int64_t parsed = 0, total = 0;
    std::vector<std::pair<hipEvent_t, hipEvent_t>> ev_all, ev_main, ev_free;
    double ms_all = 0, ms_main = 0; int64_t main_launches = 0;
    DevBuf d_sort_tmp, d_sorted, d_result, d_order, d_finish;
    uint32_t order_nb_max = 0;
    uint8_t *pin_res = nullptr;
    size_t spec_bytes = 1u << 20;
    uint8_t *pin = nullptr; size_t pin_cap = 0;
    uint8_t *pin_small = nullptr; size_t pin_small_cap = 0;
    KvqResultLayout res;
    uint64_t n_hits = 0;
    bool finished = false;
    DevBuf d_ctr_all;
    DevBuf d_gather_cnt, d_gather_res;
    bool reduced = false, gathered = false;
    bool records_on = false;
    DevBuf d_rkey, d_roff, d_rlen, d_rdir, d_rstore, d_rsmall, d_rres;
    uint32_t rslots = 0;
    unsigned long long rstore_cap = 0;
    uint8_t *pin_rec = nullptr; size_t pin_rec_cap = 0;
    uint64_t rec_hcap = 0, rec_scap = 0;
    uint64_t rec_tail_n = 0, rec_tail_b = 0;
    uint64_t rec_spec_n = 4096, rec_spec_b = 1u << 20;
    int64_t rec_store_bytes = 0;
};

struct SeedIndex;
SeedIndex *kvq_seed_index_build(kvq_table *t);
void       kvq_seed_index_destroy(SeedIndex *ix);
int kvq_seeded_launch(kvq_scan *s, const KvqParams &P, const uint8_t *d_data, int64_t nbytes,
                      const uint32_t *d_chunk_off, int64_t nchunks, int64_t fpos_base, uint32_t max_chunk_bytes);

uint32_t kvq_choose_tile(uint32_t maxline, uint32_t rec_bytes);
uint32_t kvq_min_tile();
int32_t  kvq_scan_pick(int k, int stride, bool ix_dense, uint32_t rec_bytes, uint32_t tile_bytes, uint32_t dbg, int lg_env, int dense_env);


int kvq_scan_staged(kvq_scan *s, const uint8_t *d_text, int64_t nbytes, const int64_t *chunk_off, int64_t nchunks, int64_t fpos_base);

struct kvq_bgzf_entry_ { int64_t off; uint32_t size, hdr, isize; };
int kvq_inflate_bgzf_launch(const uint8_t *d_in, int64_t in_bytes, const kvq_bgzf_block *d_tab, int64_t nblocks,
                            uint8_t *d_out, int64_t out_bytes, int32_t *d_status, hipStream_t stream);
int kvq_cut_chunks_launch(const uint8_t *d_text, int64_t have, int64_t cs, int64_t fill, int64_t *d_offs, int64_t cap, int64_t *d_res, hipStream_t stream);
```

kvarq_amd/csrc/kvq_launch.hip:

```cpp
#include "kvq_host.h"


int32_t kvq_scan_pick(int k, int stride, bool ix_dense, uint32_t rec_bytes, uint32_t tile_bytes, uint32_t dbg, int lg_env, int dense_env)
{
    if (k < 5 || k > 8 || (stride != 2 && stride != 4 && stride != 8)) return -1;
    const bool st = (dbg & 16u) != 0;
    int lg = -1;
    if (rec_bytes >= 40u) {
        const uint32_t n_full = tile_bytes / rec_bytes + 1u;
        if (n_full <= 128u && n_full > 64u) lg = 2;
        else if (n_full <= 64u && n_full > 32u) lg = 3;
        else if (n_full <= 256u && n_full > 128u) lg = 1;
    }
    if (lg_env >= -1) lg = lg_env >= 1 && lg_env <= 3 ? lg_env : -1;
    if ((lg == 3 || lg == 1) && st) lg = -1;
    const bool dense = k == 8 && !st && (dense_env >= 0 ? dense_env != 0 : ix_dense);
    const bool diag = ((dbg & ~16u) && !st) || k != 8 || dense;
    if (diag && lg != 2) lg = -1;
    return (int32_t)k | (int32_t)stride << 4 | (int32_t)(lg + 1) << 8 | (k < 8 || dense ? KVQ_CELL_DENSE : 0) |
           (diag ? KVQ_CELL_DIAG : 0) | (st && !diag ? KVQ_CELL_STAMPS : 0);
}

extern "C" int32_t kvq_scan_kernel_pick(int32_t k, int32_t stride, int32_t dense, uint32_t rec_bytes, uint32_t tile_bytes, uint32_t dbg)
{
    return kvq_scan_pick(k, stride, dense != 0, rec_bytes, tile_bytes, dbg, -2, -1);
}

extern "C" int32_t kvq_scan_kernel(const kvq_scan *s) { return s->kernel_cell; }

int kvq_seeded_launch(kvq_scan *s, const KvqParams &P, const uint8_t *d_data, int64_t nbytes,
                      const uint32_t *d_chunk_off, int64_t nchunks, int64_t fpos_base, uint32_t max_chunk_bytes)
{
    (void)nbytes; (void)max_chunk_bytes;
    SeedIndex *ix = s->t->index;
    const std::vector<int64_t> &co = s->cur_chunk_off;
    if (s->tile_bytes == 0) {
        const size_t n = (size_t)std::min<int64_t>(nbytes, 128 << 10);
        std::vector<uint8_t> head(n);
        KVQ_HIP(hipStreamSynchronize(s->stream));
        KVQ_HIP(hipMemcpy(head.data(), d_data, n, hipMemcpyDeviceToHost));
        s->tile_bytes = kvq_tile_for_text(head.data(), n, &s->rec_bytes);
    }
    const uint32_t TILE = s->tile_bytes;
    uint64_t nt = 0;
    for (int64_t c = 0; c < nchunks; c++) {
        const uint32_t a = (uint32_t)co[c], b = (uint32_t)co[c + 1];
        nt += b > a ? (uint32_t)(((uint64_t)b - (a & ~15u) + TILE - 1) / TILE) : 0u;
    }
    s->cur_ntiles = 0;
    if (nt == 0) {
        if (!s->ev_main.empty()) { KVQ_HIP(hipEventRecord(s->ev_main.back().first, s->stream)); KVQ_HIP(hipEventRecord(s->ev_main.back().second, s->stream)); }
        return KVQ_OK;
    }
    static const uint32_t grid_env = (uint32_t)(getenv("KVQ_GRID") ? atoi(getenv("KVQ_GRID")) : 0);
    const uint32_t cus = s->cus ? s->cus : (s->cus = kvq_device_cu_count());
    const uint32_t per_cu = 4u;
    const uint32_t grid_full = cus * per_cu, grid_shared = grid_full - cus / 4u;
    const uint32_t grid_cap = grid_env ? grid_env : (kvq_live_scans() > 1 && kvq_chain_busy(s)) ? grid_shared : grid_full;
    if (s->pool.used + ((size_t)nchunks + 1) * 4 + (size_t)nt * 24 + 24576 + KVQ_SKIP_CAP * sizeof(KvqSkippedTile) > s->pool.cap) {
        kvq_set_error(KVQ_ERR_RUNTIME, "batch tables outgrew their reservation"); return KVQ_ERR_RUNTIME;
    }
    const size_t first_b = (((size_t)nchunks + 1) * 4 + 255) & ~(size_t)255;
    const size_t ctr_b = 256 + 4 * BP_SHARDS * BP_SHARD_STRIDE;
    const size_t first_at = s->pool.take(first_b + sizeof(BpArgs) + ctr_b);
    const size_t chunk_at = s->pool.take((size_t)nt * 16), report_at = s->pool.take((size_t)nt * 8), skip_at = s->pool.take(KVQ_SKIP_CAP * sizeof(KvqSkippedTile));
    s->cur_skip_at = skip_at; s->cur_first_at = first_at; s->cur_ntiles = (uint32_t)nt;
    uint32_t *first = reinterpret_cast<uint32_t *>(s->pool.h + first_at);
    uint64_t acc = 0;
    for (int64_t c = 0; c < nchunks; c++) {
        const uint32_t a = (uint32_t)co[c], b = (uint32_t)co[c + 1];
        first[c] = (uint32_t)acc;
        acc += b > a ? (uint32_t)(((uint64_t)b - (a & ~15u) + TILE - 1) / TILE) : 0u;
    }
    first[nchunks] = (uint32_t)acc;
    static const uint32_t dbg = (uint32_t)(getenv("KVQ_DBG") ? atoi(getenv("KVQ_DBG")) : 0);
    const uint32_t grid_seeded = (uint32_t)std::min<uint64_t>(nt, grid_cap);
    uint32_t *d_first = reinterpret_cast<uint32_t *>(s->pool.d + first_at);
    const BpArgs *d_args = reinterpret_cast<const BpArgs *>(s->pool.d + first_at + first_b);
    uint32_t *d_tchunk = reinterpret_cast<uint32_t *>(s->pool.d + chunk_at);
    uint32_t *d_report = reinterpret_cast<uint32_t *>(s->pool.d + report_at);
    const size_t ctr_at = first_at + first_b + ((sizeof(BpArgs) + 127) & ~(size_t)127);
    unsigned int *d_tile_ctr = reinterpret_cast<unsigned int *>(s->pool.d + ctr_at);
    {
        BpArgs a;
        memset(&a, 0, sizeof(a));
        a.P = P; a.X = ix->dev; a.data = d_data; a.fpos_base = fpos_base;
        a.tiles = reinterpret_cast<const uint4 *>(d_tchunk); a.tile_report = d_report; a.tile_ctr = d_tile_ctr;
        static const uint32_t stagger = (uint32_t)(getenv("KVQ_STAGGER") ? atoi(getenv("KVQ_STAGGER")) : 0);
        a.ntiles = (uint32_t)nt; a.tile_bytes = TILE; a.dbg = dbg; a.pad_ = stagger;
        a.redo = s->d_redo.p; a.redo_cap = KVQ_REDO_CAP - KVQ_LONG_CAP; a.fail = s->cur_fail;
        static const bool surv_off = getenv("KVQ_SURVIVORS") && getenv("KVQ_SURVIVORS")[0] == '0';
        a.surv = surv_off ? nullptr : s->d_surv.p; a.surv_cap = s->surv_cap;
        memcpy(s->pool.h + first_at + first_b, &a, sizeof(a));
    }
    {
        unsigned int *hc = reinterpret_cast<unsigned int *>(s->pool.h + ctr_at);
        memset(hc, 0, 4 * BP_SHARDS * BP_SHARD_STRIDE);
        for (uint32_t sh = 0; sh < BP_SHARDS; sh++) hc[sh * BP_SHARD_STRIDE] = bp_shard_begin(sh, (uint32_t)nt);
    }
    KVQ_HIP(hipMemcpyAsync(s->pool.d + s->cur_co_at, s->pool.h + s->cur_co_at, ctr_at + 4 * BP_SHARDS * BP_SHARD_STRIDE - s->cur_co_at,
                           hipMemcpyHostToDevice, s->stream));
    hipLaunchKernelGGL(kvq_expand_tiles, dim3((uint32_t)((nchunks + 255) / 256)), dim3(256), 0, s->stream, (uint32_t)nchunks, d_chunk_off, d_first, reinterpret_cast<uint4 *>(d_tchunk),
                       s->d_redo.p ? KvqRedo(s->d_redo.p).count : (unsigned int *)nullptr, s->d_surv.p ? KvqSurvivors(s->d_surv.p).count : (unsigned int *)nullptr);

    bool pipelined = false;
    { const int rcw = kvq_chain_wait(s, &pipelined); if (rcw) return rcw; }
    const bool timed = !s->ev_main.empty();
    if (timed) KVQ_HIP(hipEventRecord(s->ev_main.back().first, s->stream));
    typedef void (*BpKernel)(const BpArgs *);
    {
        static const BpKernel kernels_diag[6] = { kvq_scan_bp<2, -1, false, true>, kvq_scan_bp<4, -1, false, true>, kvq_scan_bp<8, -1, false, true>,
                                                  kvq_scan_bp<2, 2, false, true>, kvq_scan_bp<4, 2, false, true>, kvq_scan_bp<8, 2, false, true> };
        static const BpKernel kernels_bp[18] = { kvq_scan_bp<2, -1, false>, kvq_scan_bp<4, -1, false>, kvq_scan_bp<8, -1, false>,
                                                 kvq_scan_bp<2, -1, true>, kvq_scan_bp<4, -1, true>, kvq_scan_bp<8, -1, true>,
                                                 kvq_scan_bp<2, 2, false>, kvq_scan_bp<4, 2, false>, kvq_scan_bp<8, 2, false>,
                                                 kvq_scan_bp<2, 2, true>, kvq_scan_bp<4, 2, true>, kvq_scan_bp<8, 2, true>,
                                                 kvq_scan_bp<2, 3, false>, kvq_scan_bp<4, 3, false>, kvq_scan_bp<8, 3, false>,
                                                 kvq_scan_bp<2, 1, false>, kvq_scan_bp<4, 1, false>, kvq_scan_bp<8, 1, false> };
        static const BpKernel kernels_k5[6] = { kvq_scan_bp<2, -1, false, true, 5>, kvq_scan_bp<4, -1, false, true, 5>, kvq_scan_bp<8, -1, false, true, 5>,
                                                kvq_scan_bp<2, 2, false, true, 5>, kvq_scan_bp<4, 2, false, true, 5>, kvq_scan_bp<8, 2, false, true, 5> };
        static const BpKernel kernels_k6[6] = { kvq_scan_bp<2, -1, false, true, 6>, kvq_scan_bp<4, -1, false, true, 6>, kvq_scan_bp<8, -1, false, true, 6>,
                                                kvq_scan_bp<2, 2, false, true, 6>, kvq_scan_bp<4, 2, false, true, 6>, kvq_scan_bp<8, 2, false, true, 6> };
        static const BpKernel kernels_k7[6] = { kvq_scan_bp<2, -1, false, true, 7>, kvq_scan_bp<4, -1, false, true, 7>, kvq_scan_bp<8, -1, false, true, 7>,
                                                kvq_scan_bp<2, 2, false, true, 7>, kvq_scan_bp<4, 2, false, true, 7>, kvq_scan_bp<8, 2, false, true, 7> };
        static const BpKernel kernels_dense[6] = { kvq_scan_bp<2, -1, false, true, 8, true>, kvq_scan_bp<4, -1, false, true, 8, true>, kvq_scan_bp<8, -1, false, true, 8, true>,
                                                   kvq_scan_bp<2, 2, false, true, 8, true>, kvq_scan_bp<4, 2, false, true, 8, true>, kvq_scan_bp<8, 2, false, true, 8, true> };
        static const int lg_env = getenv("KVQ_LG") ? atoi(getenv("KVQ_LG")) : -2;
        static const int dense_env = getenv("KVQ_DENSE") ? atoi(getenv("KVQ_DENSE")) : -1;
        const int32_t cell = kvq_scan_pick(ix->k, ix->stride, ix->dense, s->rec_bytes, TILE, dbg, lg_env, dense_env);
        if (cell < 0) { kvq_set_error(KVQ_ERR_RUNTIME, "no scan kernel for seeds of %d bases at stride %d", ix->k, ix->stride); return KVQ_ERR_RUNTIME; }
        const int si = ix->stride == 8 ? 2 : ix->stride == 4 ? 1 : 0, lg = ((cell >> 8) & 15) - 1;
        const int k = cell & 15;
        const bool dense = (cell & KVQ_CELL_DENSE) != 0, diag = (cell & KVQ_CELL_DIAG) != 0, stamps = (cell & KVQ_CELL_STAMPS) != 0;
        const BpKernel *const dk = k == 5 ? kernels_k5 : k == 6 ? kernels_k6 : k == 7 ? kernels_k7 : dense ? kernels_dense : kernels_diag;
        const BpKernel kern = diag ? dk[(lg == 2 ? 3 : 0) + si] : kernels_bp[lg == 3 ? 12 + si : lg == 1 ? 15 + si : (lg == 2 ? 6 : 0) + si + (stamps ? 3 : 0)];
        s->kernel_cell = cell;
        hipLaunchKernelGGL(kern, dim3(grid_seeded), dim3(ST_THREADS), 0, s->stream, d_args);
    }
    if (timed) KVQ_HIP(hipEventRecord(s->ev_main.back().second, s->stream));
    static const int sv_env = getenv("KVQ_SV_MODE") ? atoi(getenv("KVQ_SV_MODE")) : -1;
    const bool beside = sv_env >= 0 ? sv_env != 0 : pipelined;
    if (beside) { const int rcp = kvq_chain_publish(s); if (rcp) return rcp; }
    static const int sv_grid = getenv("KVQ_SV_GRID") ? atoi(getenv("KVQ_SV_GRID")) : 64;
    if (s->d_surv.p)
        hipLaunchKernelGGL(kvq_verify_survivors, dim3(beside ? sv_grid : 256), dim3(beside ? 256 : 1024), 0, s->stream, P, d_data, fpos_base, (const void *)s->d_surv.p,
                           (const unsigned int *)s->cur_fail, ix->k, ix->stride, ix->pitch);
    if (!beside) { const int rcp = kvq_chain_publish(s); if (rcp) return rcp; }
    if (!(dbg & 64u))
    hipLaunchKernelGGL(kvq_validate_tiles, dim3((uint32_t)((nchunks + 255) / 256)), dim3(256), 0, s->stream, (uint32_t)nchunks,
                       d_first, d_report, s->cur_fail, reinterpret_cast<KvqSkippedTile *>(s->pool.d + skip_at), d_chunk_off, TILE);
    KVQ_HIP(hipGetLastError());
    if (getenv("KVQ_DBG_REPORT")) {
        KVQ_HIP(hipStreamSynchronize(s->stream));
        std::vector<uint32_t> rep((size_t)nt);
        KVQ_HIP(hipMemcpy(rep.data(), d_report, (size_t)nt * 4, hipMemcpyDeviceToHost));
        for (int64_t c = 0; c < nchunks; c++) {
            uint32_t seen = 0, total = 0;
            for (uint32_t g = first[c]; g < first[c + 1]; g++) total += rep[g] & 0xFFFFu;
            for (uint32_t g = first[c]; g < first[c + 1]; g++) {
                if (kvq_tile_report_bad(rep[g], g == first[c], seen, total))
                    fprintf(stderr, "tile %u (chunk %lld [%lld, %lld), tile %u of it): report %08x n_owned %u jn %u seen %u of %u\n",
                            g, (long long)c, (long long)co[c], (long long)co[c + 1], g - first[c], rep[g], rep[g] & 0xFFFFu, (rep[g] >> 16) & 0xFFu, seen, total);
                seen += rep[g] & 0xFFFFu;
            }
        }
    }
    return KVQ_OK;
}
```

kvarq_amd/csrc/kvq_runtime.hip:

```cpp
#include "kvq_host.h"

#include <algorithm>
#include <atomic>
#include <mutex>
#include <stdarg.h>
#include <string.h>
#include <chrono>

static double now_ms() { return std::chrono::duration<double, std::milli>(std::chrono::steady_clock::now().time_since_epoch()).count(); }
static const bool g_timing = getenv("KVQ_TIMING") != nullptr;

#define KVQ_NEED_RESCAN (-2)


static thread_local int  tl_err_code = 0;
static thread_local char tl_err_msg[1024] = "";

void kvq_set_error(int code, const char *fmt, ...)
{
    tl_err_code = code;
    va_list ap; va_start(ap, fmt);
    vsnprintf(tl_err_msg, sizeof(tl_err_msg), fmt, ap);
    va_end(ap);
}
// ... 166 lines not shown

    std::vector<int32_t> all((size_t)nseq);
    for (int i = 0; i < nseq; i++) all[i] = i;
    bool ok = t->d_tab.ensure(t->h_tab.size()) == KVQ_OK && t->d_off.ensure((size_t)(nseq + 1) * 4) == KVQ_OK &&
              t->d_exh.ensure((size_t)(nseq + 1) * 4) == KVQ_OK && t->d_all.ensure((size_t)(nseq + 1) * 4) == KVQ_OK &&
              t->d_seeded.ensure((size_t)(nseq + 1) * 4) == KVQ_OK;
    if (ok) {
        ok = hipMemcpy(t->d_tab.p, t->h_tab.data(), t->h_tab.size(), hipMemcpyHostToDevice) == hipSuccess &&
             hipMemcpy(t->d_off.p, t->h_off.data(), (size_t)(nseq + 1) * 4, hipMemcpyHostToDevice) == hipSuccess &&
             (t->exhaustive.empty() || hipMemcpy(t->d_exh.p, t->exhaustive.data(), t->exhaustive.size() * 4, hipMemcpyHostToDevice) == hipSuccess) &&
             (t->seeded.empty() || hipMemcpy(t->d_seeded.p, t->seeded.data(), t->seeded.size() * 4, hipMemcpyHostToDevice) == hipSuccess) &&
             (nseq == 0 || hipMemcpy(t->d_all.p, all.data(), (size_t)nseq * 4, hipMemcpyHostToDevice) == hipSuccess);
        if (!ok) kvq_set_error(KVQ_ERR_DEVICE, "uploading the sequence table failed");
    }
    if (!ok) { kvq_table_destroy(t); return nullptr; }
    return t;
}

extern "C" void kvq_table_destroy(kvq_table *t)
{
    if (!t) return;
    {
        int cur = 0; (void)hipGetDevice(&cur);
        if (t->device != cur) (void)hipSetDevice(t->device);
        (void)hipDeviceSynchronize();
        if (t->device != cur) (void)hipSetDevice(cur);
    }
    if (t->index) kvq_seed_index_destroy(t->index);
    t->d_tab.release(); t->d_off.release(); t->d_exh.release(); t->d_all.release(); t->d_seeded.release();
    delete t;
}
extern "C" int32_t kvq_table_nseq(const kvq_table *t) { return t->nseq; }
extern "C" int64_t kvq_table_bases(const kvq_table *t) { return t->bases; }
extern "C" int32_t kvq_table_seq_is_seeded(const kvq_table *t, int32_t s) { return (s >= 0 && s < t->nseq) ? t->is_seeded[s] : 0; }
extern "C" int32_t kvq_table_seed_k(const kvq_table *t) { return t->seed_k; }
extern "C" int64_t kvq_counters_len(const kvq_table *t) { return t->ctr_len; }
extern "C" int64_t kvq_counters_off_nseqhits(const kvq_table *t) { return t->off_nseqhits; }
extern "C" int64_t kvq_counters_off_nseqbasehits(const kvq_table *t) { return t->off_nseqbasehits; }
extern "C" int64_t kvq_counters_off_coverage(const kvq_table *t) { return t->off_cov; }
extern "C" int64_t kvq_counters_off_mutations(const kvq_table *t) { return t->off_mut; }
extern "C" int64_t kvq_table_seq_offset(const kvq_table *t, int32_t s) { return (s >= 0 && s <= t->nseq) ? t->h_off[s] : -1; }


#define KVQ_MAX_BATCHES 65536
static const size_t SMALL_RANGE = 64, SMALL_FAIL = SMALL_RANGE + 4 * (KVQ_MAX_BATCHES + 1),
                    SMALL_STAGE = (SMALL_FAIL + 4 * KVQ_MAX_BATCHES + 255) & ~(size_t)255,
                    SMALL_BYTES = SMALL_STAGE + 8 * KVQ_STAGE_SLOTS * KVQ_STAGE_COPIES;

extern "C" __global__ void __launch_bounds__(256)
kvq_commit_batch(unsigned long long *stage, unsigned long long *ctr, unsigned long long *err_stage, unsigned long long *err,
                 const unsigned int *fail, unsigned int *arena_n, unsigned int *range)
{
    KVQ_BESIDE_SCAN();
    const bool bad = (*fail & 1u) != 0u;
    for (int i = threadIdx.x; i < KVQ_STAGE_SLOTS; i += blockDim.x) {
        unsigned long long v = 0;
        for (int c = 0; c < KVQ_STAGE_COPIES; c++) {
            const unsigned long long w = stage[(size_t)c * KVQ_STAGE_SLOTS + i];
            v = i == KVQ_CTR_LONGEST_ ? (v > w ? v : w) : v + w;
            stage[(size_t)c * KVQ_STAGE_SLOTS + i] = 0;
        }
        if (v && !bad) { if (i == KVQ_CTR_LONGEST_) atomicMax(&ctr[i], v); else atomicAdd(&ctr[i], v); }
    }
    if (threadIdx.x == 0) {
        if (bad) *arena_n = range[0];
        else if (*err_stage != ~0ull) atomicMin(err, *err_stage);
        *err_stage = ~0ull;
        range[1] = *arena_n;
    }
}

extern "C" __global__ void __launch_bounds__(256)
kvq_reset_state(unsigned long long *small, size_t small_words, unsigned long long *ctr, size_t ctr_words,
                unsigned long long *cov, size_t cov_words)
{
    KVQ_BESIDE_SCAN();
    const size_t i0 = (size_t)blockIdx.x * blockDim.x + threadIdx.x, step = (size_t)gridDim.x * blockDim.x;
    for (size_t i = i0; i < small_words; i += step) small[i] = (i == 2 || i == 3) ? ~0ull : 0ull;
    for (size_t i = i0; i < ctr_words; i += step) ctr[i] = 0ull;
    for (size_t i = i0; i < cov_words; i += step) cov[i] = 0ull;
}

extern "C" __global__ void __launch_bounds__(256)
kvq_publish_small(const unsigned int *__restrict__ small, const unsigned int *__restrict__ fail, unsigned int nbatches,
                  const unsigned int *__restrict__ state, unsigned int state_words,
                  unsigned int *host_small, unsigned int *host_fail, unsigned int *host_state)
{
    KVQ_BESIDE_SCAN();
    if (threadIdx.x < 8) host_small[threadIdx.x] = small[threadIdx.x];
    for (unsigned int i = threadIdx.x; i < nbatches; i += blockDim.x) host_fail[i] = fail[i];
    for (unsigned int i = threadIdx.x; i < state_words; i += blockDim.x) host_state[i] = state[i];
    __threadfence_system();
}

static KvqRecTable rec_table(const kvq_scan *s)
{
    KvqRecTable T;
    T.key = s->d_rkey.as<unsigned long long>(); T.off = s->d_roff.as<unsigned long long>(); T.len = s->d_rlen.as<unsigned int>();
    T.dir = s->d_rdir.as<unsigned int>(); T.ctr = s->d_rsmall.as<unsigned long long>();
    T.store = s->d_rstore.as<uint8_t>(); T.store_cap = s->rstore_cap; T.mask = s->rslots - 1u;
    return T;
}

static int records_prepare(kvq_scan *s)
{
    int rc;
    uint64_t slots = 1024; while (slots < 2ull * s->arena_cap) slots <<= 1;
    if (s->rstore_cap == 0) {
        unsigned long long cap = 32ull << 20;
        if (const char *e = getenv("KVQ_RECORD_CAP")) { const long long v = atoll(e); if (v >= 0 && (unsigned long long)v < cap) cap = (unsigned long long)v; }
        if ((rc = s->d_rstore.ensure((size_t)std::max<unsigned long long>(cap, 256) + 64))) return rc;
        s->rstore_cap = cap;
    }
    if ((rc = s->d_rsmall.ensure(256))) return rc;
    if (slots > s->rslots) {
        if ((rc = s->d_rkey.ensure((size_t)slots * 8)) || (rc = s->d_roff.ensure((size_t)slots * 8)) ||
            (rc = s->d_rlen.ensure((size_t)slots * 4)) || (rc = s->d_rdir.ensure((size_t)slots * 4))) return rc;
        KVQ_HIP(hipMemsetAsync(s->d_rkey.p, 0, (size_t)slots * 8, s->stream));
        s->rslots = (uint32_t)slots;
    } else {
        hipLaunchKernelGGL(kvq_records_clear, dim3(256), dim3(256), 0, s->stream, rec_table(s));
    }
    KVQ_HIP(hipMemsetAsync(s->d_rsmall.p, 0, 256, s->stream));
    KVQ_HIP(hipGetLastError());
    return KVQ_OK;
}

static int reset_device_state(kvq_scan *s)
{
    static_assert(SMALL_BYTES % 8 == 0, "kvq_reset_state writes 8-byte words");
    hipLaunchKernelGGL(kvq_reset_state, dim3(256), dim3(256), 0, s->stream, (unsigned long long *)s->d_small.p, SMALL_BYTES / 8,
                       s->d_ctr, (size_t)s->t->ctr_len, s->d_covdiff.as<unsigned long long>(), (size_t)s->t->bases + (size_t)s->t->nseq + 1);
    KVQ_HIP(hipGetLastError());
    if (s->records_on) return records_prepare(s);
    return KVQ_OK;
}

static int ensure_arena(kvq_scan *s, uint64_t hits, uint64_t blob)
{
    if (hits > 0xFFFFFFF0ull) { kvq_set_error(KVQ_ERR_MEMORY, "cannot allocate memory for results"); return KVQ_ERR_MEMORY; }
    if (hits > s->arena_cap) {
        int rc = s->d_arena.ensure((size_t)hits * sizeof(KvqHit)); if (rc) return rc;
        s->arena_cap = (uint32_t)hits;
    }
    if (blob > s->blob_cap) {
        if (blob > 0xFFFFFFF0ull) { kvq_set_error(KVQ_ERR_MEMORY, "cannot allocate memory for results"); return KVQ_ERR_MEMORY; }
        int rc = s->d_blob.ensure((size_t)blob); if (rc) return rc;
        s->blob_cap = blob;
    }
    return KVQ_OK;
}

static std::atomic<int> g_live_scans{0};
int kvq_live_scans() { return g_live_scans.load(); }
uint32_t kvq_device_cu_count()
{
    int dev = 0; hipDeviceProp_t pr;
    if (hipGetDevice(&dev) != hipSuccess || hipGetDeviceProperties(&pr, dev) != hipSuccess || pr.multiProcessorCount <= 0) return 256u;
    return (uint32_t)pr.multiProcessorCount;
}

extern "C" kvq_scan *kvq_scan_create(const kvq_table *t, void *d_counters)
{
    kvq_clear_error();
    kvq_scan *s = new kvq_scan();
    g_live_scans++;
    s->t = t;
    if (hipStreamCreateWithFlags(&s->stream, hipStreamNonBlocking) != hipSuccess) {
        kvq_set_error(KVQ_ERR_DEVICE, "hipStreamCreate failed"); delete s; return nullptr;
    }
    if (d_counters) { s->d_ctr = (unsigned long long *)d_counters; s->own_ctr = false; }
    else {
        if (s->d_ctr_own.ensure((size_t)t->ctr_len * 8) != KVQ_OK) { kvq_scan_destroy(s); return nullptr; }
        s->d_ctr = s->d_ctr_own.as<unsigned long long>(); s->own_ctr = true;
    }
    if (s->d_small.ensure(SMALL_BYTES) != KVQ_OK) { kvq_scan_destroy(s); return nullptr; }
    if (s->d_covdiff.ensure(((size_t)t->bases + (size_t)t->nseq + 1) * 8) != KVQ_OK) { kvq_scan_destroy(s); return nullptr; }
    s->d_arena_n = (unsigned int *)s->d_small.p;
    s->d_blob_n = (unsigned long long *)((char *)s->d_small.p + 8);
    s->d_err = (unsigned long long *)((char *)s->d_small.p + 16);
    s->d_err_stage = (unsigned long long *)((char *)s->d_small.p + 24);
    s->d_range = (unsigned int *)((char *)s->d_small.p + SMALL_RANGE);
    s->d_fail = (unsigned int *)((char *)s->d_small.p + SMALL_FAIL);
    s->d_stage_ctr = (unsigned long long *)((char *)s->d_small.p + SMALL_STAGE);
    if (ensure_arena(s, 1u << 20, 64ull << 20) != KVQ_OK) { kvq_scan_destroy(s); return nullptr; }
    if (s->d_surv.ensure(KvqSurvivors::bytes()) != KVQ_OK) { kvq_scan_destroy(s); return nullptr; }
    {
        unsigned int hdr[64] = { 0 };
        hdr[1] = KVQ_SURV_CAP;
        if (const char *e = getenv("KVQ_SURV_CAP")) { const long v = atol(e); if (v >= 0 && v < (long)KVQ_SURV_CAP) hdr[1] = (unsigned int)v; }
        s->surv_cap = hdr[1];
        if (hipMemcpyAsync(s->d_surv.p, hdr, 256, hipMemcpyHostToDevice, s->stream) != hipSuccess || hipStreamSynchronize(s->stream) != hipSuccess) { kvq_scan_destroy(s); return nullptr; }
    }
    if (s->d_redo.ensure(KvqRedo::bytes()) != KVQ_OK) { kvq_scan_destroy(s); return nullptr; }
    if (hipMemsetAsync(s->d_redo.p, 0, 256, s->stream) != hipSuccess) { kvq_scan_destroy(s); return nullptr; }
    s->pin_cap = (size_t)t->ctr_len * 8 + (4u << 20);
    {
        const size_t small_b = 64 + 4 * (size_t)KVQ_MAX_BATCHES + 512;
        size_t c = 0;
        s->pin_small = (uint8_t *)pinned_take(small_b, &c); s->pin_small_cap = c;
        s->pin = (uint8_t *)pinned_take(s->pin_cap, &c);
        if (s->pin) s->pin_cap = c;
        if (!s->pin_small || !s->pin) { kvq_set_error(KVQ_ERR_MEMORY, "cannot allocate memory for results"); kvq_scan_destroy(s); return nullptr; }
        memset(s->pin_small, 0, small_b);
    }
    memset(s->pin, 0, s->pin_cap < (1u << 20) ? s->pin_cap : (1u << 20));
    s->res = kvq_result_layout(0, 0);
    s->pin_res = s->pin + ((((size_t)t->ctr_len * 8) + 255) & ~(size_t)255);
    if (reset_device_state(s) != KVQ_OK) { kvq_scan_destroy(s); return nullptr; }
    s->h_ctr.assign((size_t)t->ctr_len, 0);
    return s;
}

static std::mutex g_chain_lock;
static hipEvent_t g_chain_done = nullptr;
static const kvq_scan *g_chain_owner = nullptr;

bool kvq_chain_busy(const kvq_scan *s)
{
    std::lock_guard<std::mutex> l(g_chain_lock);
    if (!g_chain_done || g_chain_owner == s) return false;
    const bool busy = hipEventQuery(g_chain_done) == hipErrorNotReady;
    (void)hipGetLastError();
    return busy;
}
int kvq_chain_wait(kvq_scan *s, bool *behind_a_running_scan)
{
    std::lock_guard<std::mutex> l(g_chain_lock);
    if (behind_a_running_scan) *behind_a_running_scan = false;
    if (g_chain_done && g_chain_owner != s) {
        if (behind_a_running_scan) { *behind_a_running_scan = hipEventQuery(g_chain_done) == hipErrorNotReady; (void)hipGetLastError(); }
        KVQ_HIP(hipStreamWaitEvent(s->stream, g_chain_done, 0));
    }
    return KVQ_OK;
}
int kvq_chain_publish(kvq_scan *s)
{
    if (!s->ev_chain) KVQ_HIP(hipEventCreateWithFlags(&s->ev_chain, hipEventDisableTiming));
    KVQ_HIP(hipEventRecord(s->ev_chain, s->stream));
    std::lock_guard<std::mutex> l(g_chain_lock);
    g_chain_done = s->ev_chain; g_chain_owner = s;
    return KVQ_OK;
}
static void chain_forget(const kvq_scan *s)
{
    std::lock_guard<std::mutex> l(g_chain_lock);
    if (g_chain_owner == s) { g_chain_done = nullptr; g_chain_owner = nullptr; }
}

static void drop_events(kvq_scan *s, bool destroy = false)
{
    for (auto *v : { &s->ev_all, &s->ev_main }) { s->ev_free.insert(s->ev_free.end(), v->begin(), v->end()); v->clear(); }
    if (destroy) {
        chain_forget(s);
        for (auto &e : s->ev_free) { (void)hipEventDestroy(e.first); (void)hipEventDestroy(e.second); }
        s->ev_free.clear();
    }
}

extern "C" void kvq_scan_destroy(kvq_scan *s)
{
    if (!s) return;
    g_live_scans--;
    if (s->stream) (void)hipStreamSynchronize(s->stream);
    drop_events(s, true);
    s->d_ctr_own.release();
    if (s->copy_stream) (void)hipStreamSynchronize(s->copy_stream);
    if (s->pin) pinned_give(s->pin, s->pin_cap);
    if (s->pin_small) pinned_give(s->pin_small, s->pin_small_cap);
    for (int i = 0; i < 2; i++) if (s->ev_copy[i]) (void)hipEventDestroy(s->ev_copy[i]);
    if (s->copy_stream) (void)hipStreamDestroy(s->copy_stream);
    if (s->ev_chain) (void)hipEventDestroy(s->ev_chain);
    if (s->pin_rec) pinned_give(s->pin_rec, s->pin_rec_cap);
    DevBuf *bufs[] = { &s->d_rkey, &s->d_roff, &s->d_rlen, &s->d_rdir, &s->d_rstore, &s->d_rsmall, &s->d_rres, &s->d_surv, &s->d_redo, &s->d_ctr_all, &s->d_gather_cnt, &s->d_gather_res, &s->d_sort_tmp, &s->d_sorted, &s->d_result, &s->d_order, &s->d_finish, &s->d_covdiff, &s->d_skipped, &s->d_chunk_off, &s->d_seg_base, &s->d_seg_cnt, &s->d_chunk_nrec, &s->d_rec_base, &s->d_nl4,
                       &s->d_rec_start, &s->d_read_off, &s->d_read_len, &s->d_arena, &s->d_blob, &s->d_small, &s->d_stage, &s->d_stage_b };
    for (DevBuf *b : bufs) b->release();
    s->pool.release();
    if (s->stream) (void)hipStreamDestroy(s->stream);
    delete s;
}

extern "C" int32_t kvq_scan_path(const kvq_scan *s) { return s->path_bits; }
extern "C" void kvq_scan_force_exhaustive(kvq_scan *s, int32_t on) { s->force_exhaustive = on != 0; }

extern "C" int32_t kvq_scan_set_records(kvq_scan *s, int32_t on)
{
    kvq_clear_error();
    if (!s->batches.empty() || s->copied_pending || s->host_pending >= 0) {
        kvq_set_error(KVQ_ERR_RUNTIME, "kvq_scan_set_records: only before the first batch or after kvq_scan_reset");
        return KVQ_ERR_RUNTIME;
    }
    if (on && s->comm) {
        kvq_set_error(KVQ_ERR_RUNTIME, "records are not gathered across ranks: a scan with a communicator cannot keep them");
        return KVQ_ERR_RUNTIME;
    }
    const bool was = s->records_on;
    s->records_on = on != 0;
    s->rec_store_bytes = 0;
    return s->records_on && !was ? records_prepare(s) : KVQ_OK;
}
extern "C" const uint8_t *kvq_scan_record_blob(const kvq_scan *s)
{
    return s->records_on && s->finished ? s->pin_rec + 256 + ((s->rec_hcap * 8 + 255) & ~255ull) + ((s->rec_hcap * 4 + 255) & ~255ull) : nullptr;
}
extern "C" const int64_t *kvq_scan_hit_record_off(const kvq_scan *s) { return s->records_on && s->finished ? reinterpret_cast<const int64_t *>(s->pin_rec + 256) : nullptr; }
extern "C" const int32_t *kvq_scan_hit_record_len(const kvq_scan *s)
{
    return s->records_on && s->finished ? reinterpret_cast<const int32_t *>(s->pin_rec + 256 + ((s->rec_hcap * 8 + 255) & ~255ull)) : nullptr;
}
extern "C" int64_t kvq_scan_record_bytes(const kvq_scan *s) { return s->records_on && s->finished ? s->rec_store_bytes : 0; }

extern "C" int32_t kvq_scan_reset(kvq_scan *s)
{
    kvq_clear_error();
    const double tr0 = now_ms();
    KVQ_HIP(hipStreamSynchronize(s->stream));
    drop_events(s);
    if (s->copy_stream) (void)hipStreamSynchronize(s->copy_stream);
    s->batches.clear(); s->host_batches = false; s->host_pending = -1; s->copied_pending = false; s->records = 0; s->parsed = 0; s->total = 0;
    s->ms_all = s->ms_main = 0; s->main_launches = 0; s->finished = false; s->reduced = false; s->gathered = false; s->path_bits = 0; s->kernel_cell = 0; s->n_hits = 0;
    s->tail_pending = false;
    s->pool.used = 0;
    const int rr = reset_device_state(s);
    if (g_timing) fprintf(stderr, "reset host %.3f ms\n", now_ms() - tr0);
    return rr;
}

static KvqParams make_params(const kvq_scan *s)
{
    const kvq_table *t = s->t;
    KvqParams P;
    P.maxerrors = t->cfg.maxerrors; P.minoverlap = t->cfg.minoverlap; P.minreadlength = t->cfg.minreadlength;
    P.amin = (int32_t)t->cfg.Amin; P.nseq = t->nseq;
    P.tab = t->d_tab.as<uint8_t>(); P.tab_off = t->d_off.as<int32_t>();
    P.ctr = s->d_ctr; P.covdiff = s->d_covdiff.as<unsigned long long>();
    P.off_nseqhits = t->off_nseqhits; P.off_nseqbasehits = t->off_nseqbasehits; P.off_cov = t->off_cov; P.off_mut = t->off_mut;
    P.arena = s->d_arena.as<KvqHit>(); P.arena_cap = s->arena_cap; P.arena_n = s->d_arena_n;
    P.blob = s->d_blob.as<uint8_t>(); P.blob_cap = s->blob_cap; P.blob_n = s->d_blob_n;
    P.err = s->d_err;
    return P;
}

static int new_event_pair(kvq_scan *s, std::vector<std::pair<hipEvent_t, hipEvent_t>> &v)
{
    if (!s->ev_free.empty()) { v.push_back(s->ev_free.back()); s->ev_free.pop_back(); return KVQ_OK; }
    hipEvent_t a, b;
    KVQ_HIP(hipEventCreate(&a)); KVQ_HIP(hipEventCreate(&b));
    v.emplace_back(a, b);
    return KVQ_OK;
}

static int run_batch(kvq_scan *s, const uint8_t *d_data, int64_t nbytes, const int64_t *chunk_off, int64_t nchunks,
                     int64_t fpos_base, size_t batch_no, bool exhaustive_only)
{
    const kvq_table *t = s->t;
    const double tb0 = now_ms();
    if (nbytes <= 0 || nchunks <= 0) return KVQ_OK;
    if (nbytes > 0xFFF00000ll) { kvq_set_error(KVQ_ERR_RUNTIME, "batch of %lld bytes is too large (< 4 GiB - 1 MiB)", (long long)nbytes); return KVQ_ERR_RUNTIME; }
    if (batch_no >= KVQ_MAX_BATCHES) { kvq_set_error(KVQ_ERR_RUNTIME, "too many batches in one scan"); return KVQ_ERR_RUNTIME; }
    if (((uintptr_t)d_data & 15u) != 0) { kvq_set_error(KVQ_ERR_RUNTIME, "device buffer must be 16-byte aligned"); return KVQ_ERR_RUNTIME; }

    KvqParams P = make_params(s);
    const bool use_seeded = t->index && !t->seeded.empty() && !s->force_exhaustive && !exhaustive_only;
    s->cur_chunk_off.assign(chunk_off, chunk_off + nchunks + 1);
    const std::vector<int32_t> *exh = &t->exhaustive;
    const int32_t *d_exh = t->d_exh.as<int32_t>();
    std::vector<int32_t> all;
    if (!use_seeded) { d_exh = t->d_all.as<int32_t>(); }
    const int32_t n_exh = use_seeded ? (int32_t)exh->size() : t->nseq;

    int rc;
    const size_t tiles_bound = (size_t)(nbytes / kvq_min_tile()) + (size_t)nchunks + 2;
    if ((rc = s->pool.reserve(((size_t)nchunks + 1) * 8 + tiles_bound * 24 + 65536, s->stream))) return rc;
    const size_t co_at = s->pool.take(((size_t)nchunks + 1) * 4);
    s->cur_co_at = co_at;
    uint32_t *co = reinterpret_cast<uint32_t *>(s->pool.h + co_at);
    const uint32_t *d_co = reinterpret_cast<const uint32_t *>(s->pool.d + co_at);
    std::vector<uint32_t> sb((size_t)nchunks + 1);
    uint32_t maxseg = 0, maxchunk = 0; uint64_t segs = 0;
    for (int64_t c = 0; c <= nchunks; c++) {
        if (chunk_off[c] < 0 || chunk_off[c] > nbytes || (c && chunk_off[c] < chunk_off[c - 1])) {
            kvq_set_error(KVQ_ERR_RUNTIME, "bad chunk offsets"); return KVQ_ERR_RUNTIME;
        }
        co[c] = (uint32_t)chunk_off[c];
    }
    for (int64_t c = 0; c < nchunks; c++) {
        const uint32_t a = co[c], b = co[c + 1];
        const uint32_t n = b > a ? (uint32_t)(((uint64_t)b - (a & ~15u) + KVQ_SEG_BYTES - 1) / KVQ_SEG_BYTES) : 0u;
        sb[c] = (uint32_t)segs; segs += n;
        maxseg = std::max(maxseg, n); maxchunk = std::max(maxchunk, b - a);
    }
    sb[nchunks] = (uint32_t)segs;
    if (!use_seeded) KVQ_HIP(hipMemcpyAsync(s->pool.d + co_at, co, ((size_t)nchunks + 1) * 4, hipMemcpyHostToDevice, s->stream));

    if ((rc = new_event_pair(s, s->ev_all))) return rc;
    KVQ_HIP(hipEventRecord(s->ev_all.back().first, s->stream));

    bool hist_done = false;
    if (use_seeded) {
        if ((rc = new_event_pair(s, s->ev_main))) return rc;
        KvqParams PS = P;
        PS.ctr = s->d_stage_ctr; PS.err = s->d_err_stage;
        s->cur_fail = s->d_fail + batch_no;
        if ((rc = kvq_seeded_launch(s, PS, d_data, nbytes, d_co, nchunks, fpos_base, maxchunk))) return rc;
        s->batches[batch_no].skip_at = s->cur_skip_at; s->batches[batch_no].tile_bytes = s->tile_bytes;
        s->main_launches++; s->path_bits |= 1;
        hist_done = true;
    }

    if (!hist_done || n_exh > 0) {
        if (n_exh > 0) s->path_bits |= 2;
        if ((rc = s->d_seg_base.ensure(sb.size() * 4))) return rc;
        if ((rc = s->d_seg_cnt.ensure((size_t)(segs + 1) * 4))) return rc;
        if ((rc = s->d_chunk_nrec.ensure((size_t)(nchunks + 1) * 4))) return rc;
        if ((rc = s->d_rec_base.ensure((size_t)(nchunks + 1) * 4))) return rc;
        KVQ_HIP(hipMemcpyAsync(s->d_seg_base.p, sb.data(), sb.size() * 4, hipMemcpyHostToDevice, s->stream));
        const uint32_t gx = std::max(1u, std::min(65u, (maxseg + 3) / 4));
        for (int64_t c0 = 0; c0 < nchunks; c0 += 32768) {
            const uint32_t ny = (uint32_t)std::min<int64_t>(32768, nchunks - c0);
            hipLaunchKernelGGL(kvq_count_lines, dim3(gx, ny), dim3(256), 0, s->stream, d_data,
                               d_co + c0, s->d_seg_base.as<uint32_t>() + c0, s->d_seg_cnt.as<uint32_t>());
        }
        hipLaunchKernelGGL(kvq_scan_segments, dim3((uint32_t)((nchunks + 3) / 4)), dim3(256), 0, s->stream, (uint32_t)nchunks,
                           s->d_seg_base.as<uint32_t>(), s->d_seg_cnt.as<uint32_t>(), s->d_chunk_nrec.as<uint32_t>());
        std::vector<uint32_t> nrec((size_t)nchunks), rbase((size_t)nchunks + 1);
        KVQ_HIP(hipMemcpyAsync(nrec.data(), s->d_chunk_nrec.p, (size_t)nchunks * 4, hipMemcpyDeviceToHost, s->stream));
        KVQ_HIP(hipStreamSynchronize(s->stream));
        uint64_t R = 0;
        for (int64_t c = 0; c < nchunks; c++) { rbase[c] = (uint32_t)R; R += nrec[c]; }
        rbase[nchunks] = (uint32_t)R;
        if (R > 0) {
            if ((rc = s->d_nl4.ensure((size_t)R * 16))) return rc;
            if ((rc = s->d_rec_start.ensure((size_t)R * 4))) return rc;
            if ((rc = s->d_read_off.ensure((size_t)R * 4))) return rc;
            if ((rc = s->d_read_len.ensure((size_t)R * 4))) return rc;
            KVQ_HIP(hipMemcpyAsync(s->d_rec_base.p, rbase.data(), rbase.size() * 4, hipMemcpyHostToDevice, s->stream));
            KVQ_HIP(hipStreamSynchronize(s->stream));
            for (int64_t c0 = 0; c0 < nchunks; c0 += 32768) {
                const uint32_t ny = (uint32_t)std::min<int64_t>(32768, nchunks - c0);
                hipLaunchKernelGGL(kvq_index_records, dim3(gx, ny), dim3(256), 0, s->stream, d_data,
                                   d_co + c0, s->d_seg_base.as<uint32_t>() + c0, s->d_seg_cnt.as<uint32_t>(),
                                   s->d_chunk_nrec.as<uint32_t>() + c0, s->d_rec_base.as<uint32_t>() + c0,
                                   s->d_nl4.as<uint32_t>(), s->d_rec_start.as<uint32_t>());
            }
            const uint32_t per_block = 4 * 16;
            hipLaunchKernelGGL(kvq_trim_records, dim3((uint32_t)((R + per_block - 1) / per_block)), dim3(256), 0, s->stream, P, d_data,
                               fpos_base, (uint32_t)R, KvqDevCount{ nullptr, 0, 0, nullptr }, s->d_nl4.as<uint32_t>(), s->d_rec_start.as<uint32_t>(),
                               s->d_read_off.as<uint32_t>(), s->d_read_len.as<int32_t>(), hist_done ? 0 : 1, 16u, (unsigned int *)nullptr, 0u);
            if (n_exh > 0) {
                const bool main_here = !use_seeded;
                if (main_here) { if ((rc = new_event_pair(s, s->ev_main))) return rc; KVQ_HIP(hipEventRecord(s->ev_main.back().first, s->stream)); }
                hipLaunchKernelGGL(kvq_match_all, dim3((uint32_t)((R + 3) / 4)), dim3(256), 0, s->stream, P, d_data, fpos_base, (uint32_t)R, KvqDevCount{ nullptr, 0, 0, nullptr },
                                   s->d_read_off.as<uint32_t>(), s->d_read_len.as<int32_t>(), d_exh, n_exh);
                if (main_here) { KVQ_HIP(hipEventRecord(s->ev_main.back().second, s->stream)); s->main_launches++; }
            }
        }
    }
    if (use_seeded && s->cur_ntiles) {
        const KvqRedo Rd(s->d_redo.p);
        unsigned int *const failw = s->d_fail + batch_no;
        const KvqSkippedTile *tiles = reinterpret_cast<const KvqSkippedTile *>(s->pool.d + s->cur_skip_at);
        const KvqDevCount ntile{ failw, 8, KVQ_SKIP_CAP, failw }, nrec{ Rd.count, 0, KVQ_REDO_CAP - KVQ_LONG_CAP, failw }, nlong{ Rd.count + 1, 0, 0xFFFFFFFFu, failw };
        hipLaunchKernelGGL(kvq_collect_skipped, dim3(16), dim3(256), 0, s->stream, d_data, tiles, 0u, ntile, Rd.nl4, Rd.rec_start, Rd.count, KVQ_REDO_CAP - KVQ_LONG_CAP);
        hipLaunchKernelGGL(kvq_trim_records, dim3(32), dim3(256), 0, s->stream, P, d_data, fpos_base, 0u, nrec, Rd.nl4, Rd.rec_start, Rd.read_off, Rd.read_len, 1, 1u, Rd.count + 1, KVQ_REDO_CAP - 1u);
        static const char *mg = getenv("KVQ_MGRID");
        const uint32_t lgrid = mg && atoi(mg) > 0 ? (uint32_t)atoi(mg) : 1536u;
        const dim3 ogrid = s->seen_skips ? dim3(128, (uint32_t)std::min<size_t>(s->t->seeded.size(), 4), 1) : dim3(16, (uint32_t)std::min<size_t>(s->t->seeded.size(), 4), 1);
        if (!s->t->seeded.empty()) {
            hipLaunchKernelGGL(kvq_match_all, ogrid, dim3(256), 0, s->stream, P, d_data, fpos_base, 0u, nrec,
                               Rd.read_off, Rd.read_len, s->t->d_seeded.as<int32_t>(), (int32_t)s->t->seeded.size());
            hipLaunchKernelGGL(kvq_match_long, dim3(s->seen_skips ? lgrid : 256u), dim3(256), 0, s->stream, P, d_data, fpos_base, nlong,
                               Rd.read_off, Rd.read_len, s->t->d_seeded.as<int32_t>(), (int32_t)s->t->seeded.size(), KVQ_REDO_CAP - 1u);
        }
// ... 152 lines not shown
}

extern "C" int32_t kvq_scan_host(kvq_scan *s, const void *h_data, int64_t nbytes, const int64_t *chunk_off, int64_t nchunks, int64_t fpos_base)
{
    const int rc = kvq_scan_host_async(s, h_data, nbytes, chunk_off, nchunks, fpos_base);
    return rc ? rc : kvq_scan_host_copied(s);
}

static int records_tail(kvq_scan *s, const KvqFinishState *d_st)
{
    int rc;
    const size_t hoff = ((size_t)s->arena_cap * 8 + 255) & ~(size_t)255;
    if ((rc = s->d_rres.ensure(hoff + (size_t)s->arena_cap * 4 + 256))) return rc;
    long long *d_off = s->d_rres.as<long long>();
    int32_t *d_len = reinterpret_cast<int32_t *>(s->d_rres.as<uint8_t>() + hoff);
    hipLaunchKernelGGL(kvq_record_lookup, dim3(256), dim3(256), 0, s->stream, rec_table(s), d_st, (const uint8_t *)s->d_result.p, d_off, d_len);
    KVQ_HIP(hipGetLastError());
    s->rec_tail_n = s->rec_tail_b = 0;
    if (!s->pin_rec) return KVQ_OK;
    const uint64_t n = std::min<uint64_t>(std::min<uint64_t>(s->rec_spec_n, s->rec_hcap), s->arena_cap);
    const uint64_t b = std::min<uint64_t>(std::min<uint64_t>(s->rec_spec_b, s->rec_scap), s->rstore_cap);
    uint8_t *h_len = s->pin_rec + 256 + ((s->rec_hcap * 8 + 255) & ~255ull), *h_blob = h_len + ((s->rec_hcap * 4 + 255) & ~255ull);
    if (n) {
        KVQ_HIP(hipMemcpyAsync(s->pin_rec + 256, d_off, n * 8, hipMemcpyDeviceToHost, s->stream));
        KVQ_HIP(hipMemcpyAsync(h_len, d_len, n * 4, hipMemcpyDeviceToHost, s->stream));
    }
    if (b) KVQ_HIP(hipMemcpyAsync(h_blob, s->d_rstore.p, b, hipMemcpyDeviceToHost, s->stream));
    s->rec_tail_n = n; s->rec_tail_b = b;
    return KVQ_OK;
}

static int records_check(kvq_scan *s, uint64_t n_hits, unsigned long long *used, bool *grow)
{
    *grow = false;
    unsigned long long w[4] = { 0, 0, 0, 0 };
    KVQ_HIP(hipMemcpyAsync(w, s->d_rsmall.p, 32, hipMemcpyDeviceToHost, s->stream));
    KVQ_HIP(hipStreamSynchronize(s->stream));
    *used = w[0];
    if (w[0] <= s->rstore_cap && !w[2]) return KVQ_OK;
    unsigned long long want = w[0];
    if (n_hits > s->arena_cap && s->arena_cap) want = (unsigned long long)((double)w[0] * ((double)n_hits / s->arena_cap) * 1.25) + (1 << 20);
    want = std::max<unsigned long long>(want + want / 8, s->rstore_cap);
    if (want > 0xFFFFFFF0ull) { kvq_set_error(KVQ_ERR_MEMORY, "cannot allocate memory for results"); return KVQ_ERR_MEMORY; }
    int rc; if ((rc = s->d_rstore.ensure((size_t)want + 64))) return rc;
    s->rstore_cap = want;
    *grow = true;
    return KVQ_OK;
}

static int records_fetch(kvq_scan *s, uint64_t n_hits, unsigned long long used)
{
    const size_t hoff = ((size_t)s->arena_cap * 8 + 255) & ~(size_t)255;
    bool all = false;
    if (!s->pin_rec || n_hits > s->rec_hcap || used > s->rec_scap) {
        const uint64_t hc = std::max<uint64_t>(n_hits + n_hits / 4 + 4096, s->rec_hcap), sc = std::max<uint64_t>(used + used / 4 + (1 << 20), s->rec_scap);
        const size_t want = 256 + ((hc * 8 + 255) & ~255ull) + ((hc * 4 + 255) & ~255ull) + sc;
        size_t got = 0; uint8_t *np = (uint8_t *)pinned_take(want, &got);
        if (!np) { kvq_set_error(KVQ_ERR_MEMORY, "cannot allocate memory for results"); return KVQ_ERR_MEMORY; }
        if (s->pin_rec) pinned_give(s->pin_rec, s->pin_rec_cap);
        s->pin_rec = np; s->pin_rec_cap = got; s->rec_hcap = hc; s->rec_scap = sc;
        all = true;
    }
    uint8_t *h_len = s->pin_rec + 256 + ((s->rec_hcap * 8 + 255) & ~255ull), *h_blob = h_len + ((s->rec_hcap * 4 + 255) & ~255ull);
    bool copied = false;
    if (n_hits && (all || n_hits > s->rec_tail_n)) {
        KVQ_HIP(hipMemcpyAsync(s->pin_rec + 256, s->d_rres.p, n_hits * 8, hipMemcpyDeviceToHost, s->stream));
        KVQ_HIP(hipMemcpyAsync(h_len, s->d_rres.as<uint8_t>() + hoff, n_hits * 4, hipMemcpyDeviceToHost, s->stream));
        copied = true;
    }
    if (used && (all || used > s->rec_tail_b)) {
        KVQ_HIP(hipMemcpyAsync(h_blob, s->d_rstore.p, used, hipMemcpyDeviceToHost, s->stream));
        copied = true;
    }
    if (copied) KVQ_HIP(hipStreamSynchronize(s->stream));
    s->rec_store_bytes = (int64_t)used;
    s->rec_spec_n = n_hits + n_hits / 8 + 4096; s->rec_spec_b = used + used / 8 + 65536;
    return KVQ_OK;
}

static int enqueue_tail(kvq_scan *s)
{
    int rc;
    const kvq_table *t = s->t;
    const size_t ctr_b = ((size_t)t->ctr_len * 8 + 255) & ~(size_t)255;
    unsigned char *small = s->pin_small; unsigned int *fail = reinterpret_cast<unsigned int *>(s->pin_small + 64);
    static const bool no_buckets = getenv("KVQ_ORDER") && !strcmp(getenv("KVQ_ORDER"), "mergesort");
    uint32_t nb_max = 256; while ((uint64_t)nb_max < 4ull * s->arena_cap && nb_max < KVQ_BUCKETS_MAX) nb_max <<= 1;
    const size_t order_b = kvq_order_scratch_zero_bytes(nb_max) + (size_t)s->arena_cap * 4;
    if (order_b > s->d_order.cap || nb_max != s->order_nb_max) {
        if ((rc = s->d_order.ensure(order_b))) return rc;
        KVQ_HIP(hipMemsetAsync(s->d_order.p, 0, kvq_order_scratch_zero_bytes(nb_max), s->stream));
        s->order_nb_max = nb_max;
    }
    const KvqOrderScratch W = kvq_order_scratch(s->d_order.p, nb_max);
    if ((rc = s->d_finish.ensure(sizeof(KvqFinishState) + 256))) return rc;
    KvqFinishState *d_st = s->d_finish.as<KvqFinishState>();
    const size_t res_cap = kvq_result_layout(s->arena_cap, s->blob_cap).total + 256;
    if ((rc = s->d_result.ensure(res_cap))) return rc;
    int64_t lo = 0, hi = 1;
    for (size_t b = 0; b < s->batches.size(); b++) {
        const int64_t a = s->batches[b].fpos_base, e = a + s->batches[b].nbytes;
        if (b == 0 || a < lo) lo = a;
        if (b == 0 || e > hi) hi = e;
    }
    const size_t nb0 = s->batches.size();
    hipLaunchKernelGGL(kvq_finish_plan, dim3(1), dim3(64), 0, s->stream, (const unsigned int *)s->d_arena_n, s->arena_cap,
                       (const unsigned long long *)s->d_blob_n, (unsigned long long)s->blob_cap, (const unsigned long long *)s->d_err,
                       (long long)lo, (long long)hi, nb_max, d_st);
    if (t->nseq > 0)
        hipLaunchKernelGGL(kvq_cov_apply, dim3((uint32_t)((t->nseq + 3) / 4)), dim3(256), 0, s->stream, make_params(s));
    if (!no_buckets &&
        (rc = kvq_order_by_buckets(s->stream, s->d_arena.as<KvqHit>(), s->d_blob.as<uint8_t>(), s->blob_cap, d_st, W, s->d_result.as<uint8_t>()))) return rc;
    if (s->records_on && (rc = records_tail(s, d_st))) return rc;
    hipLaunchKernelGGL(kvq_publish_small, dim3(1), dim3(256), 0, s->stream, (const unsigned int *)s->d_small.p,
                       (const unsigned int *)s->d_fail, (unsigned int)nb0, (const unsigned int *)d_st, (unsigned int)(sizeof(KvqFinishState) / 4),
                       (unsigned int *)small, fail, (unsigned int *)(s->pin_small + 64 + 4 * (size_t)KVQ_MAX_BATCHES));
    KVQ_HIP(hipGetLastError());
    size_t spec = std::min(s->spec_bytes, res_cap);
    if (ctr_b + spec > s->pin_cap) spec = s->pin_cap > ctr_b ? s->pin_cap - ctr_b : 0;
    KVQ_HIP(hipMemcpyAsync(s->pin, s->d_ctr, (size_t)t->ctr_len * 8, hipMemcpyDeviceToHost, s->stream));
    if (spec) KVQ_HIP(hipMemcpyAsync(s->pin + ctr_b, s->d_result.p, spec, hipMemcpyDeviceToHost, s->stream));
    s->tail_nb0 = nb0; s->tail_spec = spec; s->tail_pending = true;
    return KVQ_OK;
}

extern "C" int32_t kvq_scan_finish_begin(kvq_scan *s)
{
    kvq_clear_error();
    if (!s || s->finished) return KVQ_OK;
    if (s->host_pending >= 0 || s->copied_pending) { const int rc0 = kvq_scan_host_drain(s); if (rc0) return rc0; }
    return enqueue_tail(s);
}

static int finish_once(kvq_scan *s)
{
    const double t0 = now_ms();
    { const int rc0 = kvq_scan_host_drain(s); if (rc0) return rc0; }
    int rc;
    const kvq_table *t = s->t;
    const size_t ctr_b = ((size_t)t->ctr_len * 8 + 255) & ~(size_t)255;
    unsigned int *fail = reinterpret_cast<unsigned int *>(s->pin_small + 64);
    const KvqFinishState *h_st = reinterpret_cast<const KvqFinishState *>(s->pin_small + 64 + 4 * (size_t)KVQ_MAX_BATCHES);
    static const bool no_buckets = getenv("KVQ_ORDER") && !strcmp(getenv("KVQ_ORDER"), "mergesort");

    for (int round = 0; round < 3; round++) {
        if (!(s->tail_pending && s->tail_nb0 == s->batches.size()) && (rc = enqueue_tail(s))) return rc;
        s->tail_pending = false;
        const size_t nb0 = s->tail_nb0;
        size_t spec = s->tail_spec;
        KvqFinishState *d_st = s->d_finish.as<KvqFinishState>();
        KVQ_HIP(hipStreamSynchronize(s->stream));
        const double t1 = now_ms();

        if (nb0 && (s->path_bits & 1)) {
            bool any = false;
            for (size_t b = 0; b < nb0; b++) {
                if (!fail[b] || s->batches[b].redone || s->batches[b].is_redo || !s->batches[b].d_data) continue;
                if (!(fail[b] & 1u)) { s->path_bits |= 8 | 2; s->seen_skips = true; continue; }
                s->batches[b].redone = true;
                s->tile_bytes = kvq_choose_tile(1u << 20, 0); s->rec_bytes = 0;
                Batch again = s->batches[b]; again.is_redo = true;
                s->batches.push_back(again);
                s->path_bits |= 4; any = true;
                rc = run_batch(s, again.d_data, again.nbytes, again.chunk_off.data(), (int64_t)again.chunk_off.size() - 1,
                               again.fpos_base, s->batches.size() - 1, true);
                if (rc) return rc;
            }
            if (any) continue;
        }
        const KvqFinishState st = *h_st;
        const uint32_t n_hits = st.n_raw; const unsigned long long blob_n = st.blob_n, err = st.err;
        if (err != ~0ull) {
            const long fpos = (long)(err >> 16); const int kind = (int)((err >> 8) & 0xFF); const int ch = (int)(err & 0xFF);
            if (kind == 0) kvq_set_error(KVQ_ERR_FORMAT, "record must start with '@' (and not '%c') fpos=%ld", ch, fpos);
            else kvq_set_error(KVQ_ERR_FORMAT, "3rd line of record must start with '+' fpos=%ld", fpos);
            return KVQ_ERR_FORMAT;
        }
        unsigned long long rec_used = 0; bool rec_grow = false;
        if (s->records_on && (rc = records_check(s, n_hits, &rec_used, &rec_grow))) return rc;
        if (n_hits > s->arena_cap || blob_n > s->blob_cap) {
            const uint64_t want_hits = std::max<uint64_t>(n_hits + n_hits / 8 + 1024, s->arena_cap);
            uint64_t want_blob = blob_n;
            if (n_hits > s->arena_cap && s->arena_cap) want_blob = (uint64_t)((double)blob_n * ((double)n_hits / s->arena_cap) * 1.25) + (1 << 20);
            want_blob = std::max<uint64_t>(want_blob + want_blob / 8, s->blob_cap);
            rc = ensure_arena(s, want_hits, want_blob); if (rc) return rc;
            return KVQ_NEED_RESCAN;
        }
        if (rec_grow) return KVQ_NEED_RESCAN;
        const KvqResultLayout L = st.L;
        if (ctr_b + L.total > s->pin_cap) {
            const size_t want = (ctr_b + L.total) * 5 / 4 + (1 << 20);
            size_t got = 0; uint8_t *np = (uint8_t *)pinned_take(want, &got);
            if (!np) { kvq_set_error(KVQ_ERR_MEMORY, "cannot allocate memory for results"); return KVQ_ERR_MEMORY; }
            memcpy(np, s->pin, ctr_b);
            pinned_give(s->pin, s->pin_cap);
            s->pin = np; s->pin_cap = got; spec = 0;
        }
        bool refetch = L.total > spec;
        if (n_hits && (no_buckets || st.crowded)) {
            if ((rc = kvq_order_by_mergesort(s->stream, s->d_arena.as<KvqHit>(), n_hits, s->d_blob.as<uint8_t>(), s->blob_cap, d_st,
                                             s->d_sort_tmp, s->d_sorted, s->d_result.as<uint8_t>()))) return rc;
            refetch = true;
            if (s->records_on && (rc = records_tail(s, d_st))) return rc;
            s->rec_tail_n = 0;
        }
        if (n_hits && refetch) {
            KVQ_HIP(hipMemcpyAsync(s->pin + ctr_b, s->d_result.p, L.total, hipMemcpyDeviceToHost, s->stream));
            KVQ_HIP(hipStreamSynchronize(s->stream));
        }
        if (s->records_on && (rc = records_fetch(s, n_hits, rec_used))) return rc;
        memcpy(s->h_ctr.data(), s->pin, (size_t)t->ctr_len * 8);
        s->pin_res = s->pin + ctr_b;
        if (!n_hits) memset(s->pin_res + L.hitseq_off, 0, 8);
        s->res = L; s->n_hits = n_hits;
        s->spec_bytes = L.total + L.total / 8 + 65536;

        s->ms_all = s->ms_main = 0;
        for (auto &e : s->ev_all) { float ms = 0; if (hipEventElapsedTime(&ms, e.first, e.second) == hipSuccess) s->ms_all += ms; }
        for (auto &e : s->ev_main) { float ms = 0; if (hipEventElapsedTime(&ms, e.first, e.second) == hipSuccess) s->ms_main += ms; }
        (void)hipGetLastError();
        s->finished = true;
        if (g_timing) {
            unsigned int rc2[2] = { 0, 0 };
            if (s->d_redo.p) (void)hipMemcpy(rc2, s->d_redo.p, 8, hipMemcpyDeviceToHost);
            fprintf(stderr, "finish: enqueue + wait %.3f  rest %.3f ms (%u hits; the last launch's skipped tiles left %u records, %u of them long)\n", t1 - t0, now_ms() - t1, n_hits, rc2[0], rc2[1]);
        }
        return KVQ_OK;
    }
    kvq_set_error(KVQ_ERR_RUNTIME, "a redone batch failed validation again");
    return KVQ_ERR_RUNTIME;
}

int kvq_scan_finish_internal(kvq_scan *s)
{
    for (int attempt = 0; attempt < 4; attempt++) {
        int rc = finish_once(s);
        if (rc != KVQ_NEED_RESCAN) return rc;
        if (s->host_batches) return KVQ_NEED_RESCAN;
        std::vector<Batch> again; again.swap(s->batches);
        drop_events(s); s->main_launches = 0; s->path_bits = 0; s->tail_pending = false;
        if ((rc = reset_device_state(s))) return rc;
        s->pool.used = 0;
        for (size_t b = 0; b < again.size(); b++) {
            if (again[b].is_redo) continue;
            Batch nb = again[b]; nb.redone = false; nb.skips_done = false;
            s->batches.push_back(nb);
            rc = run_batch(s, nb.d_data, nb.nbytes, nb.chunk_off.data(), (int64_t)nb.chunk_off.size() - 1, nb.fpos_base, s->batches.size() - 1, false);
            if (rc) return rc;
        }
    }
    kvq_set_error(KVQ_ERR_MEMORY, "cannot allocate memory for results");
    return KVQ_ERR_MEMORY;
}

static int finish_over_ranks(kvq_scan *s, int rc_own)
{
    int rc;
    if ((rc = s->d_finish.ensure(sizeof(KvqFinishState) + 256))) return rc;
    unsigned long long *scratch = (unsigned long long *)((char *)s->d_finish.p + ((sizeof(KvqFinishState) + 15) & ~(size_t)15));
    unsigned long long worst = 0;
    const unsigned long long mine = rc_own == KVQ_OK ? 0ull : rc_own == KVQ_ERR_RESCAN ? 1ull : 2ull;
    if ((rc = kvq_comm_max_status(s->comm, mine, scratch, s->stream, &worst))) return rc;
    if (worst == 2) {
        if (rc_own != KVQ_OK && rc_own != KVQ_ERR_RESCAN) return rc_own;
        kvq_set_error(KVQ_ERR_RUNTIME, "the scan of another rank has failed");
        return KVQ_ERR_RUNTIME;
    }
    if (worst == 1) {
        if (rc_own != KVQ_ERR_RESCAN) kvq_set_error(KVQ_ERR_RESCAN, "the hit arena of another rank overflowed on host batches: every rank resets its scan and feeds its batches again");
        s->finished = false;
        return KVQ_ERR_RESCAN;
    }
    if ((rc = s->d_ctr_all.ensure((size_t)s->t->ctr_len * 8))) return rc;
    if ((rc = kvq_comm_reduce_counters(s->comm, s->d_ctr, s->d_ctr_all.as<unsigned long long>(), s->t->ctr_len, scratch, s->stream))) return rc;
    KVQ_HIP(hipMemcpyAsync(s->pin, s->d_ctr_all.p, (size_t)s->t->ctr_len * 8, hipMemcpyDeviceToHost, s->stream));
    KVQ_HIP(hipStreamSynchronize(s->stream));
    memcpy(s->h_ctr.data(), s->pin, (size_t)s->t->ctr_len * 8);
    s->reduced = true;
    return KVQ_OK;
}

extern "C" int32_t kvq_scan_finish(kvq_scan *s)
{
    kvq_clear_error();
    int rc = kvq_scan_finish_internal(s);
    if (rc == KVQ_NEED_RESCAN) { kvq_set_error(KVQ_ERR_RESCAN, "hit arena overflow on host batches: the arena has been enlarged, reset the scan and feed the batches again"); rc = KVQ_ERR_RESCAN; }
    if (s->comm) {
        const int saved = kvq_error_code(); char msg[1024]; kvq_last_error(msg, sizeof(msg));
        const int rc2 = finish_over_ranks(s, rc);
        if (rc && rc2 == rc) kvq_set_error(saved, "%s", msg);
        rc = rc2;
    }
    return rc;
}

extern "C" int64_t kvq_scan_n_hits(const kvq_scan *s) { return (int64_t)s->n_hits; }
extern "C" const int32_t *kvq_scan_hit_seq_nr(const kvq_scan *s) { return reinterpret_cast<const int32_t *>(s->pin_res + s->res.seq_nr); }
extern "C" const int64_t *kvq_scan_hit_file_pos(const kvq_scan *s) { return reinterpret_cast<const int64_t *>(s->pin_res + s->res.file_pos); }
extern "C" const int32_t *kvq_scan_hit_seq_pos(const kvq_scan *s) { return reinterpret_cast<const int32_t *>(s->pin_res + s->res.seq_pos); }
extern "C" const int32_t *kvq_scan_hit_length(const kvq_scan *s) { return reinterpret_cast<const int32_t *>(s->pin_res + s->res.length); }
extern "C" const int32_t *kvq_scan_hit_readlength(const kvq_scan *s) { return reinterpret_cast<const int32_t *>(s->pin_res + s->res.readlength); }
extern "C" const uint8_t *kvq_scan_hitseq_blob(const kvq_scan *s) { return s->pin_res + s->res.blob; }
extern "C" const int64_t *kvq_scan_hitseq_offsets(const kvq_scan *s) { return reinterpret_cast<const int64_t *>(s->pin_res + s->res.hitseq_off); }
extern "C" const int64_t *kvq_scan_counters(const kvq_scan *s) { return s->h_ctr.data(); }
extern "C" void *kvq_scan_device_counters(const kvq_scan *s) { return s->reduced ? s->d_ctr_all.p : (void *)s->d_ctr; }
extern "C" void *kvq_scan_device_counters_own(const kvq_scan *s) { return s->d_ctr; }
extern "C" int64_t kvq_scan_parsed(const kvq_scan *s) { return s->parsed; }
extern "C" int64_t kvq_scan_total(const kvq_scan *s) { return s->total; }
extern "C" double kvq_scan_kernel_ms(const kvq_scan *s) { return s->ms_all; }
extern "C" double kvq_scan_main_kernel_ms(const kvq_scan *s) { return s->ms_main; }
extern "C" double kvq_scan_gap_ms(const kvq_scan *a, const kvq_scan *b)
{
    if (!a || !b || a->ev_main.empty() || b->ev_main.empty()) return -1.0;
    float ms = 0;
    if (hipEventElapsedTime(&ms, a->ev_main.back().second, b->ev_main.front().first) != hipSuccess) { (void)hipGetLastError(); return -1.0; }
    return (double)ms;
}
extern "C" int64_t kvq_scan_main_kernel_launches(const kvq_scan *s) { return s->main_launches; }


int64_t kvq_tail_record(const uint8_t *buf, int64_t n)
{
    bool plus_seen = false;
    for (int64_t k = n - 1; k >= 2; k--) {
        const uint8_t prev = buf[k - 1];
        if (prev != '\n' && prev != '\r') continue;
        if (buf[k] == '+') plus_seen = true;
        else if (buf[k] == '@' && plus_seen) return n - k;
    }
    return -1;
}

extern "C" int64_t kvq_chunk_offsets(const uint8_t *data, int64_t nbytes, int64_t *offsets, int64_t cap)
{
    int64_t n = 0, cs = 0, fill = 0;
    for (;;) {
        const int64_t want = KVQ_SCANBUFSIZE - (fill - cs);
        const int64_t have = nbytes - fill;
        if (have >= want) {
            const int64_t end = fill + want;
            const int64_t keep = kvq_tail_record(data + cs, end - cs);
            if (keep < 0) return -1;
            if (n < cap) offsets[n] = cs;
            n++;
            cs = end - keep; fill = end;
        } else {
            if (nbytes > cs) { if (n < cap) offsets[n] = cs; n++; }
            break;
        }
    }
    if (n < cap + 1) offsets[n] = nbytes;
    return n;
}
```

kvarq_amd/engine.py:

```python
import collections
import itertools
import numpy as np
import ctypes as C

from . import _lib
from .fastq import FastqFileFormatException
from .log import lo

Hit = collections.namedtuple('Hit', 'seq_nr file_pos seq_pos length readlength')
Hit.__doc__ = (
    "seq_nr : refers to the list of sequences in call to engine.findseqs\n"
    "file_pos : beginning of read (within decompressed data)\n"
    "seq_pos : places the beginning of the read relative to the beginning of the sequence\n"
    "length : gives the number of overlapping basepairs\n"
    "readlength : length of the (quality trimmed) read containing the hit\n")

_KEYS = ('maxerrors', 'minoverlap', 'minreadlength', 'nthreads', 'Amin', 'Azero')


def _char(x, name):
    if isinstance(x, str):
        x = x.encode('latin-1')
    if not isinstance(x, (bytes, bytearray)) or len(x) != 1:
        raise TypeError('%s must be a single character' % name)
    v = x[0]
    return v - 256 if v > 127 else v


def config(**kw):
    for k in kw:
        if k not in _KEYS:
            raise TypeError("'%s' is an invalid keyword argument for this function" % k)
    L = _lib.lib()
    c = _lib.Config()
    L.kvq_config_get(C.byref(c))
    for k in _KEYS[:4]:
        if k in kw:
            if isinstance(kw[k], bool) or not isinstance(kw[k], int):
                raise TypeError('an integer is required')
            setattr(c, k, kw[k])
    for k in _KEYS[4:]:
        if k in kw:
            setattr(c, k, _char(kw[k], k))
    L.kvq_config_set(C.byref(c))


def get_config():
    L = _lib.lib()
    c = _lib.Config()
    L.kvq_config_get(C.byref(c))
    return {'maxerrors': c.maxerrors, 'minoverlap': c.minoverlap, 'minreadlength': c.minreadlength,
            'nthreads': c.nthreads, 'Amin': chr(c.Amin & 0xFF), 'Azero': chr(c.Azero & 0xFF)}


class RescanRequired(MemoryError):
    """kvq_scan_finish after host batches: the hit arena was too small; it has been enlarged, and the same
    batches have to be fed again after a reset (``scan.Scanner`` does that itself)"""


def _raise_last():
    code, msg = _lib.last_error()
    if code == _lib.ERR_FORMAT:
        raise FastqFileFormatException(msg)
    if code == _lib.ERR_IO:
        raise IOError(msg)
    if code == _lib.ERR_RESCAN:
        raise RescanRequired(msg)
    if code == _lib.ERR_MEMORY:
        raise MemoryError(msg)
    if code == _lib.ERR_TYPE:
        raise TypeError(msg)
    raise RuntimeError(msg)


def _stats_dict(readlengths, longest, nseqbasehits, nseqhits, parsed, total, sigints, records):
    progress = 0.0
    if total > 0:
        progress = C.c_float(C.c_float(min(parsed, total)).value / C.c_float(total).value).value
    return {
        'readlengths': tuple(readlengths[i] if i < _lib.MAX_READLENGTH else 0 for i in range(longest + 1)),
        'progress': progress,
        'nseqbasehits': tuple(nseqbasehits),
        'nseqhits': tuple(nseqhits),
        'parsed': parsed, 'total': total, 'sigints': sigints, 'records_parsed': records,
    }


_last_inflate = None
INFLATE_FLAGS = {'host': 0, 'device': 1, 'device_any': 2}
PATH_DEVICE_INFLATE = 0x10
PATH_DEVICE_GZIP = 0x20
PATH_DEVICE_BAM = 0x40


def findseqs(fname, sequences, *, inflate='host', records=False):
    import os, time
    global _last_inflate
    if inflate not in INFLATE_FLAGS:
        raise ValueError("inflate must be 'host', 'device' or 'device_any'")
    _last_inflate = None
    t_in = time.perf_counter()
    L = _lib.lib()
    if isinstance(fname, (str, bytes)):
        fnames = [fname]
    else:
        try:
            fnames = list(fname)
        except TypeError:
            raise TypeError('fname must be [sequence of] string[s]')
    for f in fnames:
        if not isinstance(f, (str, bytes)):
            raise TypeError('fname must be [sequence of] string[s]')
    try:
        seqs = list(sequences)
    except TypeError:
        raise TypeError('seqlist must be sequence of strings')
    as_str = any(isinstance(s, str) for s in seqs) or not seqs and isinstance(fnames[0] if fnames else '', str)
    bseqs = []
    for s in seqs:
        if isinstance(s, str):
            s = s.encode('latin-1')
        elif not isinstance(s, (bytes, bytearray)):
            raise TypeError('seqlist must be list of strings')
        bseqs.append(bytes(s))
    bfiles = [f.encode() if isinstance(f, str) else f for f in fnames]

    n = len(bseqs)
    farr = (C.c_char_p * max(1, len(bfiles)))(*bfiles)
    bufs = [C.create_string_buffer(s, len(s) + 1) for s in bseqs]
    sarr = (C.c_char_p * max(1, n))(*[C.cast(b, C.c_char_p) for b in bufs])
    lens = (C.c_int32 * max(1, n))(*[len(s) for s in bseqs])

    t_0 = time.perf_counter()
    if inflate == 'host' and not records:
        h = L.kvq_findseqs(farr, len(bfiles), sarr, lens, n)
    else:
        h = L.kvq_findseqs_ex(farr, len(bfiles), sarr, lens, n, INFLATE_FLAGS[inflate] | (_lib.FIND_RECORDS if records else 0))
    t_1 = time.perf_counter()
    try:
        if h:
            path = L.kvq_scan_path(h)
            _last_inflate = ('device_bam' if path & PATH_DEVICE_BAM else 'device_gzip' if path & PATH_DEVICE_GZIP
                             else 'device' if path & PATH_DEVICE_INFLATE else 'host')
        code, _ = _lib.last_error()
        if not h or code:
            _raise_last()
        nh = L.kvq_scan_n_hits(h)
        def col(ptr, count):
            return np.ctypeslib.as_array(ptr, shape=(count,)).tolist() if count else []
        hits = tuple(map(tuple.__new__, itertools.repeat(Hit),
                         zip(col(L.kvq_scan_hit_seq_nr(h), nh), col(L.kvq_scan_hit_file_pos(h), nh), col(L.kvq_scan_hit_seq_pos(h), nh),
                             col(L.kvq_scan_hit_length(h), nh), col(L.kvq_scan_hit_readlength(h), nh))))
        off = col(L.kvq_scan_hitseq_offsets(h), nh + 1)
        blob = C.string_at(L.kvq_scan_hitseq_blob(h), off[nh]) if nh else b''
        if as_str:
            blob = blob.decode('latin-1')
        hitseqs = [blob[a:b] for a, b in zip(off, off[1:])]
        o_hits = _lib.CTR_READLENGTHS + _lib.MAX_READLENGTH
        ctr = col(L.kvq_scan_counters(h), o_hits + 2 * n)
        st = _stats_dict(
            ctr[_lib.CTR_READLENGTHS:o_hits], ctr[_lib.CTR_LONGEST] - 1,
            ctr[o_hits + n:o_hits + 2 * n], ctr[o_hits:o_hits + n],
            L.kvq_scan_parsed(h), L.kvq_scan_total(h), _sigints(), ctr[_lib.CTR_RECORDS])
        if os.environ.get('KVQ_TIMING'):
            import sys
            sys.stderr.write('engine.findseqs: arguments %.1f ms, library %.1f ms, results as Python objects %.1f ms\n' % ((t_0 - t_in) * 1e3, (t_1 - t_0) * 1e3, (time.perf_counter() - t_1) * 1e3))
        out = {'hits': hits, 'stats': st, 'hitseqs': hitseqs}
        if _last_inflate == 'device_bam':
            noqual = last_bam_report()['records_noqual']
            if noqual:
                lo.warning('%d BAM records without qualities were written with Phred 1 (\'"\'): at the default Amin '
                           'they are trimmed to nothing' % noqual)
        if records:
            out['records'] = _records(L, h, nh, as_str)
        return out
    finally:
        if h:
            t_f = time.perf_counter()
            L.kvq_findseqs_free(h)
            if os.environ.get('KVQ_TIMING'):
                import sys
                sys.stderr.write('engine.findseqs: free %.1f ms\n' % ((time.perf_counter() - t_f) * 1e3))


def _records(L, h, nh, as_str):
    if not nh:
        return []
    off = np.ctypeslib.as_array(L.kvq_scan_hit_record_off(h), shape=(nh,)).tolist()
    ln = np.ctypeslib.as_array(L.kvq_scan_hit_record_len(h), shape=(nh,)).tolist()
    blob = C.string_at(L.kvq_scan_record_blob(h), L.kvq_scan_record_bytes(h))
    if as_str:
        blob = blob.decode('latin-1')
    return [blob[a:a + b] for a, b in zip(off, ln)]


def last_inflate():
    return _last_inflate


def last_bam_report():
    rep = _lib.BamReport()
    _lib.lib().kvq_bam_last_report(C.byref(rep))
    return rep.as_dict()


def last_inflate_report():
    rep = _lib.GzipReport()
    _lib.lib().kvq_gzip_last_report(C.byref(rep))
    return rep.as_dict()
# ... 39 lines not shown
```

kvarq_amd/scan.py:

```python
import ctypes as C

import numpy as np

from . import _lib
from .engine import Hit, _raise_last


def _check(rc):
    if rc:
        _raise_last()


class Table(object):

    def __init__(self, seqs, **config):
        L = _lib.lib()
        self.seqs = [s.encode('latin-1') if isinstance(s, str) else bytes(s) for s in seqs]
        n = len(self.seqs)
        cfg = _lib.Config()
        L.kvq_config_get(C.byref(cfg))
        for k, v in config.items():
            if k in ('Amin', 'Azero'):
                v = (v.encode('latin-1') if isinstance(v, str) else v)[0]
                v = v - 256 if v > 127 else v
            setattr(cfg, k, v)
        self.config = cfg
        bufs = [C.create_string_buffer(s, len(s) + 1) for s in self.seqs]
        arr = (C.c_char_p * max(1, n))(*[C.cast(b, C.c_char_p) for b in bufs])
        lens = (C.c_int32 * max(1, n))(*[len(s) for s in self.seqs])
        self.h = L.kvq_table_create(arr, lens, n, C.byref(cfg))
        if not self.h:
            _raise_last()
        self.nseq = n
        self.bases = L.kvq_table_bases(self.h)
        self.counters_len = L.kvq_counters_len(self.h)
        self.off_nseqhits = L.kvq_counters_off_nseqhits(self.h)
        self.off_nseqbasehits = L.kvq_counters_off_nseqbasehits(self.h)
        self.off_coverage = L.kvq_counters_off_coverage(self.h)
        self.off_mutations = L.kvq_counters_off_mutations(self.h)
        self.seq_offset = [L.kvq_table_seq_offset(self.h, i) for i in range(n + 1)]
        self.seeded = [bool(L.kvq_table_seq_is_seeded(self.h, i)) for i in range(n)]
        self.seed_k = L.kvq_table_seed_k(self.h)

    def close(self):
        if self.h:
            _lib.lib().kvq_table_destroy(self.h)
            self.h = None

    def __del__(self):
        try:
            self.close()
        except Exception:
            pass


def chunk_offsets(data):
    L = _lib.lib()
    arr = np.frombuffer(data, dtype=np.uint8) if not isinstance(data, np.ndarray) else data
    cap = arr.nbytes // (512 * 1024) + 4
    out = (C.c_int64 * (cap + 1))()
    n = L.kvq_chunk_offsets(arr.ctypes.data if arr.nbytes else None, arr.nbytes, out, cap)
    if n < 0:
        raise RuntimeError('could find beginning of record')
    return np.array(list(out)[:n + 1], dtype=np.int64)


def _view(ptr, n, ctype, dtype):
    addr = C.cast(ptr, C.c_void_p).value
    if not addr or n <= 0:
        return np.zeros(0, dtype=dtype)
    return np.frombuffer((ctype * n).from_address(addr), dtype=dtype)


class RescanRequired(RuntimeError):
    """the hit arena overflowed on host batches that the Scanner no longer holds: reset() and feed them again"""


class Scanner(object):

    def __init__(self, table, counters_ptr=None, retain_limit=1 << 30, replay=None, records=False):
        self.table = table
        self.h = _lib.lib().kvq_scan_create(table.h, counters_ptr)
        if not self.h:
            _raise_last()
        self.records = bool(records)
        if self.records:
            _check(_lib.lib().kvq_scan_set_records(self.h, 1))
        self._host_batches = []
        self._device_batches = []
        self._retained, self._retain_limit, self._replay = 0, (0 if replay is not None else retain_limit), replay
        self._comm = None

    def set_comm(self, comm):
        self._comm = comm
        _check(_lib.lib().kvq_scan_set_comm(self.h, comm.h if comm is not None else None))

    def gather_hits(self):
        _check(_lib.lib().kvq_scan_gather_hits(self.h, self._comm.h if self._comm is not None else None))
        return self._hits_dict()

    def force_exhaustive(self, on=True):
        _lib.lib().kvq_scan_force_exhaustive(self.h, 1 if on else 0)

    def scan_device(self, d_ptr, nbytes, chunk_off, fpos_base=0):
        co = np.ascontiguousarray(chunk_off, dtype=np.int64)
        self._device_batches.append((d_ptr, nbytes, co, fpos_base))
        _check(_lib.lib().kvq_scan_device(self.h, d_ptr, nbytes, co.ctypes.data_as(C.POINTER(C.c_int64)), len(co) - 1, fpos_base))

    def _feed_host(self, arr, co, fpos_base):
        _check(_lib.lib().kvq_scan_host(self.h, arr.ctypes.data if arr.nbytes else None, arr.nbytes,
                                        co.ctypes.data_as(C.POINTER(C.c_int64)), len(co) - 1, fpos_base))

    def scan_host(self, data, chunk_off=None, fpos_base=0):
        arr = np.frombuffer(data, dtype=np.uint8) if not isinstance(data, np.ndarray) else data
        co = chunk_offsets(arr) if chunk_off is None else np.ascontiguousarray(chunk_off, dtype=np.int64)
        if self._host_batches is not None:
            if self._retained + arr.nbytes <= self._retain_limit:
                self._host_batches.append((arr.copy(), co.copy(), fpos_base)); self._retained += arr.nbytes
            else:
                self._host_batches = None
        self._feed_host(arr, co, fpos_base)

    def finish_begin(self):
        _check(_lib.lib().kvq_scan_finish_begin(self.h))

    def finish(self, hits=True, stats=True):
        L = _lib.lib()
        for attempt in range(4):
            if L.kvq_scan_finish(self.h) == 0:
                break
            if _lib.last_error()[0] != _lib.ERR_RESCAN or attempt == 3:
                _raise_last()
            again, device, replay = self._host_batches, self._device_batches, self._replay
            if again is None and replay is None:
                raise RescanRequired(_lib.last_error()[1])
            if replay is None and not again and not device:
                raise RescanRequired('nothing to feed again: ' + str(_lib.last_error()[1]))
            retained = self._retained
            self.reset()
            if replay is not None:
                replay(self)
            else:
                self._host_batches, self._retained = again, retained
                for arr, co, fpos_base in again:
                    self._feed_host(arr, co, fpos_base)
                for d_ptr, nbytes, co, fpos_base in device:
                    self.scan_device(d_ptr, nbytes, co, fpos_base)
        t = self.table
        ctr = _view(L.kvq_scan_counters(self.h), t.counters_len, C.c_int64, np.int64)
        if stats:
            ctr = ctr.copy()
        out = {'counters': ctr}
        out['n_hits'] = L.kvq_scan_n_hits(self.h)
        if hits:
            out.update(self._hits_dict())
            if self.records:
                out['records'] = self._records()
        out['kernel_ms'] = L.kvq_scan_kernel_ms(self.h)
        out['main_kernel_ms'] = L.kvq_scan_main_kernel_ms(self.h)
        out['main_kernel_launches'] = L.kvq_scan_main_kernel_launches(self.h)
        if not stats:
            return out
        longest = int(ctr[_lib.CTR_LONGEST]) - 1
        parsed, total = L.kvq_scan_parsed(self.h), L.kvq_scan_total(self.h)
        rls = ctr[_lib.CTR_READLENGTHS:_lib.CTR_READLENGTHS + _lib.MAX_READLENGTH]
        out['stats'] = {
            'readlengths': tuple(int(rls[i]) if i < _lib.MAX_READLENGTH else 0 for i in range(longest + 1)),
            'progress': (C.c_float(C.c_float(min(parsed, total)).value / C.c_float(total).value).value if total > 0 else 0.0),
            'nseqbasehits': tuple(int(x) for x in ctr[t.off_nseqbasehits:t.off_nseqbasehits + t.nseq]),
            'nseqhits': tuple(int(x) for x in ctr[t.off_nseqhits:t.off_nseqhits + t.nseq]),
            'parsed': parsed, 'total': total, 'sigints': 0, 'records_parsed': int(ctr[_lib.CTR_RECORDS]),
        }
        out['coverage'] = ctr[t.off_coverage:t.off_coverage + t.bases]
        out['mutations'] = ctr[t.off_mutations:t.off_mutations + 6 * t.bases]
        path = L.kvq_scan_path(self.h)
        out['path'] = {'seeded': bool(path & 1), 'exhaustive': bool(path & 2), 'rescanned': bool(path & 4), 'tiles_rescanned': bool(path & 8)}
        out['kernel'] = _lib.kernel_cell(L.kvq_scan_kernel(self.h))
        return out

    def hit_arrays(self):
        L = _lib.lib()
        nh = L.kvq_scan_n_hits(self.h)
        a = [_view(f(self.h), nh, ct, dt).copy()
             for f, ct, dt in ((L.kvq_scan_hit_seq_nr, C.c_int32, np.int32), (L.kvq_scan_hit_file_pos, C.c_int64, np.int64),
                               (L.kvq_scan_hit_seq_pos, C.c_int32, np.int32), (L.kvq_scan_hit_length, C.c_int32, np.int32),
                               (L.kvq_scan_hit_readlength, C.c_int32, np.int32))]
        off = _view(L.kvq_scan_hitseq_offsets(self.h), nh + 1, C.c_int64, np.int64).copy()
        blob = np.frombuffer(C.string_at(L.kvq_scan_hitseq_blob(self.h), int(off[nh])) if nh else b'', dtype=np.uint8)
        out = dict(seq_nr=a[0], file_pos=a[1], seq_pos=a[2], length=a[3], readlength=a[4], offsets=off, blob=blob)
        if self.records:
            out['record_off'] = _view(L.kvq_scan_hit_record_off(self.h), nh, C.c_int64, np.int64).copy()
            out['record_len'] = _view(L.kvq_scan_hit_record_len(self.h), nh, C.c_int32, np.int32).copy()
            nb = L.kvq_scan_record_bytes(self.h)
            out['record_blob'] = np.frombuffer(C.string_at(L.kvq_scan_record_blob(self.h), nb) if nb else b'', dtype=np.uint8)
        return out

    def _records(self):
        L = _lib.lib()
        nh = L.kvq_scan_n_hits(self.h)
        if not nh:
            return []
        off = _view(L.kvq_scan_hit_record_off(self.h), nh, C.c_int64, np.int64).tolist()
        ln = _view(L.kvq_scan_hit_record_len(self.h), nh, C.c_int32, np.int32).tolist()
        blob = C.string_at(L.kvq_scan_record_blob(self.h), L.kvq_scan_record_bytes(self.h))
        return [blob[a:a + b] for a, b in zip(off, ln)]

    def _hits_dict(self):
        L = _lib.lib()
        nh = L.kvq_scan_n_hits(self.h)
        a = [_view(f(self.h), nh, ct, dt).copy()
             for f, ct, dt in ((L.kvq_scan_hit_seq_nr, C.c_int32, np.int32), (L.kvq_scan_hit_file_pos, C.c_int64, np.int64),
                               (L.kvq_scan_hit_seq_pos, C.c_int32, np.int32), (L.kvq_scan_hit_length, C.c_int32, np.int32),
                               (L.kvq_scan_hit_readlength, C.c_int32, np.int32))]
        hits = tuple(Hit(int(a[0][i]), int(a[1][i]), int(a[2][i]), int(a[3][i]), int(a[4][i])) for i in range(nh))
        off = L.kvq_scan_hitseq_offsets(self.h)
        blob = C.string_at(L.kvq_scan_hitseq_blob(self.h), off[nh]) if nh else b''
        return {'n_hits': nh, 'hits': hits, 'hitseqs': [blob[off[i]:off[i + 1]] for i in range(nh)]}

    def reset(self):
        self._host_batches, self._device_batches, self._retained = [], [], 0
        _check(_lib.lib().kvq_scan_reset(self.h))

    def close(self):
        if self.h:
            _lib.lib().kvq_scan_destroy(self.h)
            self.h = None

    def __del__(self):
        try:
            self.close()
        except Exception:
            pass


class DeviceBuffer(object):

    def __init__(self, nbytes):
        self.nbytes = nbytes
        self.ptr = _lib.lib().kvq_device_alloc(nbytes + 64)
        if not self.ptr:
            _raise_last()

    def upload(self, arr):
        arr = np.ascontiguousarray(arr)
        _check(_lib.lib().kvq_memcpy_h2d(self.ptr, arr.ctypes.data, arr.nbytes))

    def download(self, nbytes=None, offset=0):
        n = self.nbytes - offset if nbytes is None else nbytes
        out = np.empty(n, dtype=np.uint8)
        _check(_lib.lib().kvq_memcpy_d2h(out.ctypes.data, self.ptr + offset, n))
        return out

    def free(self):
        if self.ptr:
            _lib.lib().kvq_device_free(self.ptr)
            self.ptr = None

    def __del__(self):
        try:
            self.free()
        except Exception:
            pass


def inflate_bgzf_device(d_in, in_bytes, d_blocks, nblocks, d_out, out_bytes, d_status):
    _check(_lib.lib().kvq_inflate_bgzf_device(C.c_void_p(d_in), in_bytes, C.c_void_p(d_blocks), nblocks,
                                               C.c_void_p(d_out), out_bytes, C.c_void_p(d_status)))


def inflate_gzip_device(d_file, n, chunk_bytes, d_out, out_cap):
    from . import gzip_spec
    return gzip_spec._call(_lib.lib().kvq_inflate_gzip_device, C.c_void_p(d_file), n, chunk_bytes, out_cap, C.c_void_p(d_out))
```

Baseline: 9.478 billion.

## Add lean kernel variant that defers survivor verification to list, rescanning on overflow

Adds a template flag that compiles the seeded scan kernel without its in-place survivor verification block, and launches this lean twin by default when a survivors list exists. The verify kernel now flags when the survivors list overflowed. On overflow the host forces a full rescan and makes the scan object stick to the in-place kernels. This cuts register pressure and divergent work in the main kernel, at the cost of rescans when the list is too small. Retry budgets are raised by one to make room for the extra rescan.

Result: faster. 9.903 billion, median of 6 (+4.5%).

```diff
diff --git a/include/kvarq_hip.h b/include/kvarq_hip.h
--- a/include/kvarq_hip.h
+++ b/include/kvarq_hip.h
@@ -109,6 +109,11 @@
 #define KVQ_CELL_STAMPS 0x4000
 int32_t kvq_scan_kernel_pick(int32_t k, int32_t stride, int32_t dense, uint32_t rec_bytes, uint32_t tile_bytes, uint32_t dbg);
 int32_t kvq_scan_kernel(const kvq_scan *s);
+#define KVQ_TWIN_LEAN    1
+#define KVQ_TWIN_INPLACE 2
+#define KVQ_TWIN_STICKY  4
+int32_t kvq_scan_kernel_twin(const kvq_scan *s);
+int64_t kvq_list_rescans(void);
 uint32_t kvq_tile_for_text(const uint8_t *text, size_t n, uint32_t *rec_bytes_out);
 
 typedef struct kvq_comm kvq_comm;
diff --git a/kvarq_amd/_lib.py b/kvarq_amd/_lib.py
--- a/kvarq_amd/_lib.py
+++ b/kvarq_amd/_lib.py
@@ -96,6 +96,8 @@
     'kvq_scan_force_exhaustive': (None, [vp, i32]),
     'kvq_scan_kernel_pick': (i32, [i32, i32, i32, C.c_uint32, C.c_uint32, C.c_uint32]),
     'kvq_scan_kernel': (i32, [vp]),
+    'kvq_scan_kernel_twin': (i32, [vp]),
+    'kvq_list_rescans': (i64, []),
     'kvq_tile_for_text': (C.c_uint32, [vp, C.c_size_t, P(C.c_uint32)]),
     'kvq_comm_unique_id': (i32, [vp]),
     'kvq_comm_create': (vp, [i32, i32, vp]),
@@ -174,6 +176,10 @@
     return {'k': cell & 15, 'stride': (cell >> 4) & 15, 'lg': ((cell >> 8) & 15) - 1, 'dense': bool(cell & CELL_DENSE)}
 
 
+def kernel_twin(word):
+    return {'name': {1: 'lean', 2: 'inplace'}.get(word & 3), 'list_rescans': word >> 8}
+
+
 def last_error():
     buf = C.create_string_buffer(1024)
     code = lib().kvq_last_error(buf, 1024)
diff --git a/kvarq_amd/csrc/kernels_bp.hip b/kvarq_amd/csrc/kernels_bp.hip
--- a/kvarq_amd/csrc/kernels_bp.hip
+++ b/kvarq_amd/csrc/kernels_bp.hip
@@ -274,7 +274,7 @@
     }
 }
 
-template <int SS, int LG, bool STAMPS, bool DIAG = STAMPS, int KK = 8, bool DENSE = (KK < 8)>
+template <int SS, int LG, bool STAMPS, bool DIAG = STAMPS, int KK = 8, bool DENSE = (KK < 8), bool INPLACE = true>
 __global__ void __launch_bounds__(ST_THREADS, DENSE ? 8 : BP_OCC)
 kvq_scan_bp(const BpArgs *__restrict__ A_)
 {
@@ -845,10 +845,11 @@
 }
 extern "C" __global__ void __launch_bounds__(1024)
 kvq_verify_survivors(KvqParams P, const uint8_t *__restrict__ data, int64_t fpos_base, const void *surv_, const unsigned int *__restrict__ fail,
-                     int K, int stride, int pitch)
+                     int K, int stride, int pitch, unsigned int *__restrict__ list_full)
 {
     const KvqSurvivors Sv(const_cast<void *>(surv_));
     if (fail && (*fail & 1u)) return;
+    if (list_full && blockIdx.x == 0 && threadIdx.x == 0 && Sv.count[0] > Sv.count[1]) *list_full = 1u;
     const uint32_t n = Sv.count[0] < Sv.count[1] ? Sv.count[0] : Sv.count[1];
     const int me = P.maxerrors, mo = P.minoverlap;
     const uint32_t step = gridDim.x * blockDim.x;
diff --git a/kvarq_amd/csrc/kernels_bp_p4.inc b/kvarq_amd/csrc/kernels_bp_p4.inc
--- a/kvarq_amd/csrc/kernels_bp_p4.inc
+++ b/kvarq_amd/csrc/kernels_bp_p4.inc
@@ -90,7 +90,7 @@
                                     }
                                     if (lane == 0) { S.sv_at[wave] = at; S.sv_end[wave] = end; }
                                 }
-                                if (__any(alive)) {
+                                if constexpr (INPLACE) if (__any(alive)) {
                                     BpHot H; int64_t tile_fpos;
                                     {
                                         const BpArgsPtr A = bp_args(A_);
diff --git a/kvarq_amd/csrc/kvq_findseqs.hip b/kvarq_amd/csrc/kvq_findseqs.hip
--- a/kvarq_amd/csrc/kvq_findseqs.hip
+++ b/kvarq_amd/csrc/kvq_findseqs.hip
@@ -1315,14 +1315,14 @@
     }
     const double tf2 = now_ms();
     if (s && !bam_failed && (pin || dev || dev_any || bam)) {
-        for (int attempt = 0; attempt < 4; attempt++) {
+        for (int attempt = 0; attempt < 5; attempt++) {
             const int rc = bam ? findseqs_pass(s, files, nfiles, nullptr, nullptr, 0, nullptr, nullptr, &bamf)
                          : dev ? findseqs_pass(s, files, nfiles, nullptr, nullptr, 0, &bz)
                          : dev_any ? findseqs_pass(s, files, nfiles, nullptr, nullptr, 0, nullptr, &gzf)
                                : findseqs_pass(s, files, nfiles, pin, pin + pin_cap, use_cap);
             if (rc != KVQ_NEED_RESCAN) break;
             if (kvq_scan_reset(s)) break;
-            if (attempt == 3) kvq_set_error(KVQ_ERR_MEMORY, "cannot allocate memory for results");
+            if (attempt == 4) kvq_set_error(KVQ_ERR_MEMORY, "cannot allocate memory for results");
         }
     }
     const double tf3 = now_ms();
diff --git a/kvarq_amd/csrc/kvq_host.h b/kvarq_amd/csrc/kvq_host.h
--- a/kvarq_amd/csrc/kvq_host.h
+++ b/kvarq_amd/csrc/kvq_host.h
@@ -113,6 +113,10 @@
     unsigned long long *d_blob_n = nullptr, *d_err = nullptr, *d_err_stage = nullptr, *d_stage_ctr = nullptr;
     int path_bits = 0;
     int32_t kernel_cell = 0;
+    int32_t kernel_twin = 0;
+    bool inplace = false;
+    int32_t list_rescans = 0;
+    unsigned int *d_list_full = nullptr;
     std::vector<int64_t> cur_chunk_off;
     size_t cur_co_at = 0;
     size_t cur_skip_at = 0, cur_first_at = 0; uint32_t cur_ntiles = 0;
diff --git a/kvarq_amd/csrc/kvq_launch.hip b/kvarq_amd/csrc/kvq_launch.hip
--- a/kvarq_amd/csrc/kvq_launch.hip
+++ b/kvarq_amd/csrc/kvq_launch.hip
@@ -27,6 +27,7 @@
 }
 
 extern "C" int32_t kvq_scan_kernel(const kvq_scan *s) { return s->kernel_cell; }
+extern "C" int32_t kvq_scan_kernel_twin(const kvq_scan *s) { return s->kernel_twin | (s->inplace ? KVQ_TWIN_STICKY : 0) | s->list_rescans << 8; }
 
 int kvq_seeded_launch(kvq_scan *s, const KvqParams &P, const uint8_t *d_data, int64_t nbytes,
                       const uint32_t *d_chunk_off, int64_t nchunks, int64_t fpos_base, uint32_t max_chunk_bytes)
@@ -81,6 +82,7 @@
     uint32_t *d_report = reinterpret_cast<uint32_t *>(s->pool.d + report_at);
     const size_t ctr_at = first_at + first_b + ((sizeof(BpArgs) + 127) & ~(size_t)127);
     unsigned int *d_tile_ctr = reinterpret_cast<unsigned int *>(s->pool.d + ctr_at);
+    bool no_list = false;
     {
         BpArgs a;
         memset(&a, 0, sizeof(a));
@@ -92,6 +94,7 @@
         static const bool surv_off = getenv("KVQ_SURVIVORS") && getenv("KVQ_SURVIVORS")[0] == '0';
         a.surv = surv_off ? nullptr : s->d_surv.p; a.surv_cap = s->surv_cap;
         memcpy(s->pool.h + first_at + first_b, &a, sizeof(a));
+        no_list = a.surv == nullptr;
     }
     {
         unsigned int *hc = reinterpret_cast<unsigned int *>(s->pool.h + ctr_at);
@@ -108,6 +111,7 @@
     const bool timed = !s->ev_main.empty();
     if (timed) KVQ_HIP(hipEventRecord(s->ev_main.back().first, s->stream));
     typedef void (*BpKernel)(const BpArgs *);
+    bool lean = false;
     {
         static const BpKernel kernels_diag[6] = { kvq_scan_bp<2, -1, false, true>, kvq_scan_bp<4, -1, false, true>, kvq_scan_bp<8, -1, false, true>,
                                                   kvq_scan_bp<2, 2, false, true>, kvq_scan_bp<4, 2, false, true>, kvq_scan_bp<8, 2, false, true> };
@@ -117,6 +121,11 @@
                                                  kvq_scan_bp<2, 2, true>, kvq_scan_bp<4, 2, true>, kvq_scan_bp<8, 2, true>,
                                                  kvq_scan_bp<2, 3, false>, kvq_scan_bp<4, 3, false>, kvq_scan_bp<8, 3, false>,
                                                  kvq_scan_bp<2, 1, false>, kvq_scan_bp<4, 1, false>, kvq_scan_bp<8, 1, false> };
+#define KVQ_LEAN(ss, lg) kvq_scan_bp<ss, lg, false, false, 8, false, false>
+        static const BpKernel kernels_lean[18] = { KVQ_LEAN(2, -1), KVQ_LEAN(4, -1), KVQ_LEAN(8, -1), nullptr, nullptr, nullptr,
+                                                   KVQ_LEAN(2, 2), KVQ_LEAN(4, 2), KVQ_LEAN(8, 2), nullptr, nullptr, nullptr,
+                                                   KVQ_LEAN(2, 3), KVQ_LEAN(4, 3), KVQ_LEAN(8, 3), KVQ_LEAN(2, 1), KVQ_LEAN(4, 1), KVQ_LEAN(8, 1) };
+#undef KVQ_LEAN
         static const BpKernel kernels_k5[6] = { kvq_scan_bp<2, -1, false, true, 5>, kvq_scan_bp<4, -1, false, true, 5>, kvq_scan_bp<8, -1, false, true, 5>,
                                                 kvq_scan_bp<2, 2, false, true, 5>, kvq_scan_bp<4, 2, false, true, 5>, kvq_scan_bp<8, 2, false, true, 5> };
         static const BpKernel kernels_k6[6] = { kvq_scan_bp<2, -1, false, true, 6>, kvq_scan_bp<4, -1, false, true, 6>, kvq_scan_bp<8, -1, false, true, 6>,
@@ -133,8 +142,10 @@
         const int k = cell & 15;
         const bool dense = (cell & KVQ_CELL_DENSE) != 0, diag = (cell & KVQ_CELL_DIAG) != 0, stamps = (cell & KVQ_CELL_STAMPS) != 0;
         const BpKernel *const dk = k == 5 ? kernels_k5 : k == 6 ? kernels_k6 : k == 7 ? kernels_k7 : dense ? kernels_dense : kernels_diag;
-        const BpKernel kern = diag ? dk[(lg == 2 ? 3 : 0) + si] : kernels_bp[lg == 3 ? 12 + si : lg == 1 ? 15 + si : (lg == 2 ? 6 : 0) + si + (stamps ? 3 : 0)];
-        s->kernel_cell = cell;
+        const int bi = lg == 3 ? 12 + si : lg == 1 ? 15 + si : (lg == 2 ? 6 : 0) + si + (stamps ? 3 : 0);
+        lean = !diag && !no_list && !s->inplace && kernels_lean[bi] != nullptr;
+        const BpKernel kern = diag ? dk[(lg == 2 ? 3 : 0) + si] : lean ? kernels_lean[bi] : kernels_bp[bi];
+        s->kernel_cell = cell; s->kernel_twin = lean ? KVQ_TWIN_LEAN : KVQ_TWIN_INPLACE;
         hipLaunchKernelGGL(kern, dim3(grid_seeded), dim3(ST_THREADS), 0, s->stream, d_args);
     }
     if (timed) KVQ_HIP(hipEventRecord(s->ev_main.back().second, s->stream));
@@ -144,7 +155,7 @@
     static const int sv_grid = getenv("KVQ_SV_GRID") ? atoi(getenv("KVQ_SV_GRID")) : 64;
     if (s->d_surv.p)
         hipLaunchKernelGGL(kvq_verify_survivors, dim3(beside ? sv_grid : 256), dim3(beside ? 256 : 1024), 0, s->stream, P, d_data, fpos_base, (const void *)s->d_surv.p,
-                           (const unsigned int *)s->cur_fail, ix->k, ix->stride, ix->pitch);
+                           (const unsigned int *)s->cur_fail, ix->k, ix->stride, ix->pitch, lean ? s->d_list_full : (unsigned int *)nullptr);
     if (!beside) { const int rcp = kvq_chain_publish(s); if (rcp) return rcp; }
     if (!(dbg & 64u))
     hipLaunchKernelGGL(kvq_validate_tiles, dim3((uint32_t)((nchunks + 255) / 256)), dim3(256), 0, s->stream, (uint32_t)nchunks,
diff --git a/kvarq_amd/csrc/kvq_runtime.hip b/kvarq_amd/csrc/kvq_runtime.hip
--- a/kvarq_amd/csrc/kvq_runtime.hip
+++ b/kvarq_amd/csrc/kvq_runtime.hip
@@ -342,6 +342,8 @@
 }
 
 static std::atomic<int> g_live_scans{0};
+static std::atomic<long long> g_list_rescans{0};
+extern "C" int64_t kvq_list_rescans() { return (int64_t)g_list_rescans.load(); }
 int kvq_live_scans() { return g_live_scans.load(); }
 uint32_t kvq_device_cu_count()
 {
@@ -367,13 +369,16 @@
     if (s->d_small.ensure(SMALL_BYTES) != KVQ_OK) { kvq_scan_destroy(s); return nullptr; }
     if (s->d_covdiff.ensure(((size_t)t->bases + (size_t)t->nseq + 1) * 8) != KVQ_OK) { kvq_scan_destroy(s); return nullptr; }
     s->d_arena_n = (unsigned int *)s->d_small.p;
+    s->d_list_full = (unsigned int *)s->d_small.p + 1;
     s->d_blob_n = (unsigned long long *)((char *)s->d_small.p + 8);
     s->d_err = (unsigned long long *)((char *)s->d_small.p + 16);
     s->d_err_stage = (unsigned long long *)((char *)s->d_small.p + 24);
     s->d_range = (unsigned int *)((char *)s->d_small.p + SMALL_RANGE);
     s->d_fail = (unsigned int *)((char *)s->d_small.p + SMALL_FAIL);
     s->d_stage_ctr = (unsigned long long *)((char *)s->d_small.p + SMALL_STAGE);
-    if (ensure_arena(s, 1u << 20, 64ull << 20) != KVQ_OK) { kvq_scan_destroy(s); return nullptr; }
+    uint64_t hits0 = 1u << 20;
+    if (const char *e = getenv("KVQ_ARENA_CAP")) { const long v = atol(e); if (v > 0 && v < (1l << 20)) hits0 = (uint64_t)v; }
+    if (ensure_arena(s, hits0, 64ull << 20) != KVQ_OK) { kvq_scan_destroy(s); return nullptr; }
     if (s->d_surv.ensure(KvqSurvivors::bytes()) != KVQ_OK) { kvq_scan_destroy(s); return nullptr; }
     {
         unsigned int hdr[64] = { 0 };
@@ -508,7 +513,7 @@
     drop_events(s);
     if (s->copy_stream) (void)hipStreamSynchronize(s->copy_stream);
     s->batches.clear(); s->host_batches = false; s->host_pending = -1; s->copied_pending = false; s->records = 0; s->parsed = 0; s->total = 0;
-    s->ms_all = s->ms_main = 0; s->main_launches = 0; s->finished = false; s->reduced = false; s->gathered = false; s->path_bits = 0; s->kernel_cell = 0; s->n_hits = 0;
+    s->ms_all = s->ms_main = 0; s->main_launches = 0; s->finished = false; s->reduced = false; s->gathered = false; s->path_bits = 0; s->kernel_cell = 0; s->kernel_twin = 0; s->n_hits = 0;
     s->tail_pending = false;
     s->pool.used = 0;
     const int rr = reset_device_state(s);
@@ -967,7 +972,10 @@
         KVQ_HIP(hipStreamSynchronize(s->stream));
         const double t1 = now_ms();
 
-        if (nb0 && (s->path_bits & 1)) {
+        const bool list_full = reinterpret_cast<const unsigned int *>(s->pin_small)[1] && !s->inplace;
+        if (list_full) { s->inplace = true; s->list_rescans++; g_list_rescans++; }
+
+        if (nb0 && (s->path_bits & 1) && !list_full) {
             bool any = false;
             for (size_t b = 0; b < nb0; b++) {
                 if (!fail[b] || s->batches[b].redone || s->batches[b].is_redo || !s->batches[b].d_data) continue;
@@ -1001,7 +1009,7 @@
             rc = ensure_arena(s, want_hits, want_blob); if (rc) return rc;
             return KVQ_NEED_RESCAN;
         }
-        if (rec_grow) return KVQ_NEED_RESCAN;
+        if (rec_grow || list_full) return KVQ_NEED_RESCAN;
         const KvqResultLayout L = st.L;
         if (ctr_b + L.total > s->pin_cap) {
             const size_t want = (ctr_b + L.total) * 5 / 4 + (1 << 20);
@@ -1048,7 +1056,7 @@
 
 int kvq_scan_finish_internal(kvq_scan *s)
 {
-    for (int attempt = 0; attempt < 4; attempt++) {
+    for (int attempt = 0; attempt < 5; attempt++) {
         int rc = finish_once(s);
         if (rc != KVQ_NEED_RESCAN) return rc;
         if (s->host_batches) return KVQ_NEED_RESCAN;
@@ -1082,7 +1090,7 @@
         return KVQ_ERR_RUNTIME;
     }
     if (worst == 1) {
-        if (rc_own != KVQ_ERR_RESCAN) kvq_set_error(KVQ_ERR_RESCAN, "the hit arena of another rank overflowed on host batches: every rank resets its scan and feeds its batches again");
+        if (rc_own != KVQ_ERR_RESCAN) kvq_set_error(KVQ_ERR_RESCAN, "a device-side table of another rank overflowed on host batches: every rank resets its scan and feeds its batches again");
         s->finished = false;
         return KVQ_ERR_RESCAN;
     }
@@ -1099,7 +1107,7 @@
 {
     kvq_clear_error();
     int rc = kvq_scan_finish_internal(s);
-    if (rc == KVQ_NEED_RESCAN) { kvq_set_error(KVQ_ERR_RESCAN, "hit arena overflow on host batches: the arena has been enlarged, reset the scan and feed the batches again"); rc = KVQ_ERR_RESCAN; }
+    if (rc == KVQ_NEED_RESCAN) { kvq_set_error(KVQ_ERR_RESCAN, "a device-side table overflowed on host batches (hit arena or record store: enlarged; survivors' list: the in-place kernels from now on): reset the scan and feed the batches again"); rc = KVQ_ERR_RESCAN; }
     if (s->comm) {
         const int saved = kvq_error_code(); char msg[1024]; kvq_last_error(msg, sizeof(msg));
         const int rc2 = finish_over_ranks(s, rc);
diff --git a/kvarq_amd/engine.py b/kvarq_amd/engine.py
--- a/kvarq_amd/engine.py
+++ b/kvarq_amd/engine.py
@@ -54,7 +54,8 @@
 
 
 class RescanRequired(MemoryError):
-    """kvq_scan_finish after host batches: the hit arena was too small; it has been enlarged, and the same
+    """kvq_scan_finish after host batches: the hit arena (or the record store) was too small and has been enlarged, or the
+    survivors' list was full and the scan object now takes the in-place kernels; the same
     batches have to be fed again after a reset (``scan.Scanner`` does that itself)"""
 
 
diff --git a/kvarq_amd/scan.py b/kvarq_amd/scan.py
--- a/kvarq_amd/scan.py
+++ b/kvarq_amd/scan.py
@@ -73,7 +73,7 @@
 
 
 class RescanRequired(RuntimeError):
-    """the hit arena overflowed on host batches that the Scanner no longer holds: reset() and feed them again"""
+    """a device-side table (hit arena, record store, survivors' list) overflowed on host batches that the Scanner no longer holds: reset() and feed them again"""
 
 
 class Scanner(object):
@@ -126,10 +126,10 @@
 
     def finish(self, hits=True, stats=True):
         L = _lib.lib()
-        for attempt in range(4):
+        for attempt in range(5):
             if L.kvq_scan_finish(self.h) == 0:
                 break
-            if _lib.last_error()[0] != _lib.ERR_RESCAN or attempt == 3:
+            if _lib.last_error()[0] != _lib.ERR_RESCAN or attempt == 4:
                 _raise_last()
             again, device, replay = self._host_batches, self._device_batches, self._replay
             if again is None and replay is None:
@@ -176,6 +176,7 @@
         path = L.kvq_scan_path(self.h)
         out['path'] = {'seeded': bool(path & 1), 'exhaustive': bool(path & 2), 'rescanned': bool(path & 4), 'tiles_rescanned': bool(path & 8)}
         out['kernel'] = _lib.kernel_cell(L.kvq_scan_kernel(self.h))
+        out['twin'] = _lib.kernel_twin(L.kvq_scan_kernel_twin(self.h))
         return out
 
     def hit_arrays(self):
```
